# yusanshi/news-recommendation

Measured on NVIDIA H100. Metric: impressions/sec (fwd+bwd), higher is better.
Workload: dtype bf16

## Files before the change

### include/newsrec_b200.h

```cpp
#ifndef NEWSREC_B200_H
#define NEWSREC_B200_H

#include <stdint.h>

#ifdef __cplusplus
extern "C" {
#endif

int nr_version(void);
const char* nr_last_error(void);
int nr_device_error(int out4[4]);
long long nr_launch_count(void);
int nr_num_sms(void);
void nr_debug_set_simt_gemm(int on);
int nr_has_triage_backends(void);
void nr_debug_set_gru_stepwise(int on);
typedef struct {
    const void* A;
    int M, lda;
    const void* W;
    int N, ldw, K, taps, w_tap_rows, tap_origin;
    void* out;
    int ld_out, out_bf16, relu, tanh;
    const void* dtanh_src;
// ... 97 lines not shown
int nr_topk_dot_ranged(const float* users, long long n_users, int ld_users, const float* news, long long n_news, int ld_news, int D,
                       int k, const long long* excl_offsets, const long long* excl_rows, const int* categories, int max_per_category,
                       const long long* row_lo, const long long* row_hi, long long* idx, float* score, int* bad_row_flag,
                       int* bad_score_flag, void* workspace, long long workspace_bytes, void* stream);

int nr_mmr_rerank(const float* news, long long n_news, int ld_news, int D, const long long* shortlist_idx, const float* shortlist_score,
                  long long n_users, int depth, int k, float lambda, long long* idx, float* score, int* bad_row_flag, void* stream);

int nr_list_stats(const float* news, long long n_news, int ld_news, int D, const long long* idx, long long n_rows, int k,
                  const int* categories, const int* ks, int n_ks, double* pair_sum, int* distinct, int* bad_row_flag, void* stream);

long long nr_pool_ranks_workspace(long long n_rows, long long n_news, int D);
int nr_pool_ranks(const float* queries, long long n_rows, int ld_queries, const float* news, long long n_news, int ld_news, int D,
                  const long long* tgt_offsets, const long long* tgt_rows, const long long* excl_offsets, const long long* excl_rows,
                  long long* rank, float* score, int* bad_row_flag, int* bad_score_flag, int* target_flag, void* workspace,
                  long long workspace_bytes, void* stream);

int nr_pool_ranks_ranged(const float* queries, long long n_rows, int ld_queries, const float* news, long long n_news, int ld_news,
                         int D, const long long* tgt_offsets, const long long* tgt_rows, const long long* excl_offsets,
                         const long long* excl_rows, const long long* row_lo, const long long* row_hi, long long* rank, float* score,
                         int* bad_row_flag, int* bad_score_flag, int* target_flag, void* workspace, long long workspace_bytes,
                         void* stream);

long long nr_topk_archive_workspace(long long n_users, int P, long long n_news, int F, int hidden, int k);
int nr_topk_archive(const float* archive, long long n_users, int P, const float* news, long long n_news, int F, const float* W1,
                    const float* b1, int hidden, const float* w2, const float* b2, int k, const long long* excl_offsets,
                    const long long* excl_rows, const int* categories, int max_per_category, long long* idx, float* score,
                    int* bad_row_flag, int* bad_score_flag, void* workspace, long long workspace_bytes, void* stream);

int nr_topk_archive_ranged(const float* archive, long long n_users, int P, const float* news, long long n_news, int F,
                           const float* W1, const float* b1, int hidden, const float* w2, const float* b2, int k,
                           const long long* excl_offsets, const long long* excl_rows, const int* categories, int max_per_category,
                           const long long* row_lo, const long long* row_hi, long long* idx, float* score, int* bad_row_flag,
                           int* bad_score_flag, void* workspace, long long workspace_bytes, void* stream);

long long nr_pool_ranks_archive_workspace(long long n_rows, int P, long long n_news, int F, int hidden);
int nr_pool_ranks_archive(const float* archive, long long n_rows, int P, const float* news, long long n_news, int F, const float* W1,
                          const float* b1, int hidden, const float* w2, const float* b2, const long long* tgt_offsets,
                          const long long* tgt_rows, const long long* excl_offsets, const long long* excl_rows, long long* rank,
                          float* score, int* bad_row_flag, int* bad_score_flag, int* target_flag, void* workspace,
                          long long workspace_bytes, void* stream);

int nr_pool_ranks_archive_ranged(const float* archive, long long n_rows, int P, const float* news, long long n_news, int F,
                                 const float* W1, const float* b1, int hidden, const float* w2, const float* b2,
                                 const long long* tgt_offsets, const long long* tgt_rows, const long long* excl_offsets,
                                 const long long* excl_rows, const long long* row_lo, const long long* row_hi, long long* rank,
                                 float* score, int* bad_row_flag, int* bad_score_flag, int* target_flag, void* workspace,
                                 long long workspace_bytes, void* stream);

int nr_accumulate_ext_grad(float* ext, int rows, int ld, int D, float* dW, float* db, void* stream);

typedef struct {
    long long n_seq;
    int T;
    int d;
    int heads;
    int q;
    int ldx;
    int ld3;
    const long long* ids;
    const void* table_bf16;
    int V;
    const float* dense;
    long long dense_s_seq, dense_s_tok, dense_s_col;
    const void* wqkv_bf16;
    const float* bqkv;
    const void* wa_bf16;
    const float* ba;
    const float* qv;
    float p_drop;
    unsigned long long seed;
    void* X_bf16;
    void* QKV_bf16;
    void* C_bf16;
    float* w;
    float* out;
    int* bad_id_flag;
    void* C_lo_bf16;
    const void* wqkv_kcat_bf16;
    void* X_kcat_bf16;
    float* QKV_f32;
    void* V_lo_bf16;
    const float* dense_pos;
} nr_mhsa_encoder_fwd_args;
int nr_mhsa_accurate_supported(int T, int d, int heads);
int nr_mhsa_encoder_fwd(const nr_mhsa_encoder_fwd_args* a, void* stream);

typedef struct {
    long long n_seq;
    int T, d, heads, q, ldx, ld3, ldq;
    const long long* ids;
    int V;
    const void* wqkvT_bf16;
    const void* wa_bf16;
    const void* waT_bf16;
    const float* ba;
    const float* qv;
    float p_drop;
    unsigned long long seed;
    const void* X_bf16;
    const void* QKV_bf16;
    const void* C_bf16;
    const float* w;
    const float* dout;
    float* dWqkv_ext;
    float* dWa_ext;
    float* dqv;
    float* demb;
    float* ddense;
    void* workspace;
    long long workspace_bytes;
    const void* wqkv_bf16;
    const float* bqkv;
    void* emb_grad_ready_event;
    float* dpos;
    const void* table_bf16;
} nr_mhsa_encoder_bwd_args;
long long nr_mhsa_encoder_bwd_workspace(long long n_seq, int T, int d, int q);
int nr_mhsa_encoder_bwd(const nr_mhsa_encoder_bwd_args* a, void* stream);

typedef struct {
    long long n_seq;
    int T, d, F, q, ldx, ldf;
    const long long* ids;
    const void* table_bf16;
    int V;
    const void* wconv_bf16;
    const float* bconv;
    const void* wa_bf16;
    const float* ba;
    const float* qv;
    float p_drop;
    unsigned long long seed;
    void* Xp_bf16;
    void* Y_bf16;
    float* w;
    float* out;
    int* bad_id_flag;
    void* Y_lo_bf16;
    int window;
} nr_cnn_encoder_fwd_args;
int nr_cnn_encoder_fwd(const nr_cnn_encoder_fwd_args* a, void* stream);

typedef struct {
    long long n_seq;
    int T, d, F, q, ldx, ldf, ldq;
    const long long* ids;
    int V;
    const void* wconvT_bf16;
    const void* wa_bf16;
    const void* waT_bf16;
    const float* ba;
    const float* qv;
    float p_drop;
    unsigned long long seed;
    const void* Xp_bf16;
    const void* Y_bf16;
    const float* w;
    const float* dout;
    float* dWconv_ext;
    float* dWa_ext;
    float* dqv;
    float* demb;
    void* workspace;
    long long workspace_bytes;
    int window;
} nr_cnn_encoder_bwd_args;
long long nr_cnn_encoder_bwd_workspace(long long n_seq, int T, int F, int q);
int nr_cnn_encoder_bwd(const nr_cnn_encoder_bwd_args* a, void* stream);

typedef struct {
    long long n_seq;
    int T, d, de, F, q, n_win;
    int win[4];
    int ldx, lde, ldf, ldo;
    const long long* word_ids;
    const long long* entity_ids;
    const void* word_table_bf16;
    int V;
    const void* entity_table_bf16;
    int Ve;
    const void* mT_bf16;
    const float* mb;
    const void* wconv_bf16;
    const float* bconv;
    const void* wa_bf16;
    const float* ba;
    const float* qv;
    void* X2_bf16;
    void* E_bf16;
    void* Y_bf16;
    float* w;
    float* out;
    int* bad_id_flag;
} nr_kcnn_encoder_fwd_args;
int nr_kcnn_encoder_fwd(const nr_kcnn_encoder_fwd_args* a, void* stream);

typedef struct {
    long long n_seq;
// ... 115 lines not shown
```

### news-recommendation_b200/csrc/abi.cu

```cuda
#include <cstring>
#include <utility>

#include "../../include/newsrec_b200.h"
#include "nr_common.cuh"
#include "nr_ops.h"

namespace nr {
const char* last_error();
int read_device_error(int* out4);
void set_debug_simt_gemm(int on);
int has_triage_backends();
void set_debug_gemm_timing(void* dev_buf, int slots);
void set_comm_reserved_sms(int n);
}

using namespace nr;

extern "C" {

int nr_version(void) { return 1; }
const char* nr_last_error(void) { return last_error(); }
int nr_device_error(int out4[4]) { return read_device_error(out4); }
long long nr_launch_count(void) { return g_launches; }
int nr_num_sms(void) { return num_sms(); }
void nr_debug_set_simt_gemm(int on) { set_debug_simt_gemm(on); }
void nr_debug_set_gru_stepwise(int on) { set_gru_stepwise(on); }
int nr_debug_gemm_store(const nr_gemm_store_args* a, void* stream) {
    NR_REQUIRE(a && a->A && a->W && a->out, "nr_debug_gemm_store: null operand");
    const auto misaligned = [](const void* p, uintptr_t bytes) { return (reinterpret_cast<uintptr_t>(p) & (bytes - 1)) != 0; };
    NR_REQUIRE(!misaligned(a->out, 16) && !misaligned(a->lo_out, 16) && !misaligned(a->dtanh_src, 4),
               "nr_debug_gemm_store: out and lo_out need 16-byte, dtanh_src 4-byte aligned bases");
    return gemm_store({.A = a->A, .M = a->M, .lda = a->lda, .W = a->W, .N = a->N, .ldw = a->ldw, .K = a->K, .taps = a->taps,
                       .w_tap_rows = a->w_tap_rows, .tap_origin = a->tap_origin},
                      {.out = a->out, .ld_out = a->ld_out, .out_bf16 = a->out_bf16, .relu = a->relu, .tanh = a->tanh,
                       .dtanh_src = a->dtanh_src, .dtanh_ld = a->dtanh_ld, .bias = a->bias,
                       .rm = {a->rm_seg_in, a->rm_in_off, a->rm_seg_len, a->rm_seg_out, a->rm_out_off},
                       .drop = {a->p_drop, a->seed}, .ones_col = a->ones_col, .ones_zero_upto = a->ones_zero_upto, .lo_out = a->lo_out,
                       .ld_lo = a->ld_lo, .lo_col0 = a->lo_col0, .accumulate = a->accumulate, .rows_per_tile = a->rows_per_tile},
                      as_stream(stream));
}
int nr_debug_live_tokens(const long long* ids, long long n_seq, int T, int d, const void* table, int V, const void* X, int ldx,
                         const float* bqkv, unsigned* mask, unsigned char* pad, int* offset, int* index, int* tiles, void* Xc,
                         void* dqkv_c, void* stream) {
    NR_REQUIRE(ids && X && bqkv && mask && pad && offset && index && tiles && Xc && dqkv_c && n_seq >= 0 && d >= 2,
               "nr_debug_live_tokens: null operand or n_seq=%lld d=%d", n_seq, d);
    const cudaStream_t st = as_stream(stream);
    const int sec = (d + 7) & ~7, ld3 = (3 * sec + 15) & ~15;
    const long long bytes = live_tokens_bytes(n_seq, T, ld3);
    char* buf = nullptr;
    NR_CHECK_CUDA(cudaMallocAsync(reinterpret_cast<void**>(&buf), bytes, st));
    LiveTokens lt;
    int rc = live_tokens(ids, n_seq, T, d, table, ldx, V, bqkv, sec, ld3, X, ldx, Xc, dqkv_c, buf, bytes, &lt, st);
    const size_t n = static_cast<size_t>(n_seq), M = n * T;
    const std::pair<void*, const void*> copies[] = {{mask, lt.mask}, {pad, lt.pad}, {offset, lt.offset}, {index, lt.index}, {tiles, lt.tiles}};
    const size_t sizes[] = {4 * n, n, 4 * (n + 1), 4 * M, 4 * (1 + (M + 63) / 64)};
    for (int i = 0; i < 5 && rc == 0 && n > 0; ++i)
        if (cudaMemcpyAsync(copies[i].first, copies[i].second, sizes[i], cudaMemcpyDeviceToDevice, st) != cudaSuccess) rc = -1;
    NR_CHECK_CUDA(cudaFreeAsync(buf, st));
    NR_REQUIRE(rc != -1, "nr_debug_live_tokens: copy-out failed");
    return rc;
}
int nr_has_triage_backends(void) { return has_triage_backends(); }
void nr_reserve_sms_for_comm(int n) { set_comm_reserved_sms(n); }
void nr_debug_set_gemm_timing(void* dev_buf, int slots) { set_debug_gemm_timing(dev_buf, slots); }
void nr_profile_enable(int on) { prof_enable(on); }
void nr_profile_context(const char* ctx) { prof_context(ctx ? ctx : ""); }
int nr_profile_report(char* buf, int cap) { return prof_report(buf, cap); }

static Bf16Rows cast_pad_job(const float* src, int R, int C, int lds, void* dst, int ld, int transpose) {
    if (transpose) return {.src = src, .n_rows = C, .D = R, .s_seq = 1, .s_col = lds, .width = ld, .hi = dst, .ld_hi = ld};
    return {.src = src, .n_rows = R, .D = C, .s_seq = lds, .width = ld, .hi = dst, .ld_hi = ld};
}
int nr_cast_pad_bf16_many(int n, const float* const* src, const int* R, const int* C, const int* lds, void* const* dst, const int* ld,
                          const int* transpose, void* stream) {
    NR_REQUIRE(src && R && C && lds && dst && ld && transpose, "nr_cast_pad_bf16_many: null argument array");
    NR_REQUIRE(n >= 0 && n <= kBf16RowsJobs, "nr_cast_pad_bf16_many: %d matrices (at most %d per call)", n, kBf16RowsJobs);
    Bf16Rows jobs[kBf16RowsJobs];
    for (int i = 0; i < n; ++i) {
        NR_REQUIRE(R[i] >= 1 && C[i] >= 1, "nr_cast_pad_bf16_many: bad matrix %d", i);
        jobs[i] = cast_pad_job(src[i], R[i], C[i], lds[i], dst[i], ld[i], transpose[i]);
    }
    return rows_to_bf16(jobs, n, kCastPadMany, as_stream(stream));
}
int nr_cast_pad_bf16(const float* src, int R, int C, int lds, void* dst, int ld, int transpose, void* stream) {
    NR_REQUIRE(src && dst && R >= 0 && C >= 0 && ld % 8 == 0 && ld >= (transpose ? R : C),
               "nr_cast_pad_bf16: R=%d C=%d ld=%d transpose=%d", R, C, ld, transpose);
    return rows_to_bf16(cast_pad_job(src, R, C, lds, dst, ld, transpose), kCastPad, as_stream(stream));
}
int nr_rows_to_bf16(const float* src, long long n, int D, long long s_row, long long s_col, void* dst, int ld,
                    void* stream) {
    NR_REQUIRE(src && dst && n >= 0 && ld % 8 == 0, "nr_rows_to_bf16: n=%lld ld=%d", n, ld);
    return rows_to_bf16({.src = src, .n_rows = n, .D = D, .s_seq = s_row, .s_col = s_col, .width = ld, .hi = dst, .ld_hi = ld, .ones_col = 1},
                        kRowsToBf16, as_stream(stream));
}
int nr_rows_to_bf16_hilo(const float* src, long long n, int D, long long s_row, long long s_col, void* hi, void* lo, int ld,
                         void* stream) {
    NR_REQUIRE(src && hi && lo && n >= 0 && D >= 1 && ld % 8 == 0, "nr_rows_to_bf16_hilo: n=%lld D=%d ld=%d", n, D, ld);
    return rows_to_bf16({.src = src, .n_rows = n, .D = D, .s_seq = s_row, .s_col = s_col, .width = ld, .hi = hi, .ld_hi = ld, .ones_col = 1,
                         .lo = lo, .ld_lo = ld},
                        kRowsToBf16Planes, as_stream(stream));
}
int nr_gather_rows(const long long* ids, long long n_tok, int T, const void* table, int V, int D, int ld, void* X,
                   int padded, float p_drop, unsigned long long seed, int* bad_id_flag, void* stream) {
    NR_REQUIRE(ids && table && X && bad_id_flag && T >= 1 && n_tok % T == 0 && p_drop >= 0.f && p_drop < 1.f,
               "nr_gather_rows: n_tok=%lld T=%d p=%f", n_tok, T, p_drop);
    return gather_rows(ids, n_tok, T, table, V, D, ld, X, ld, padded, DropoutCfg{p_drop, seed}, bad_id_flag, as_stream(stream));
}
int nr_linear(const void* A, int M, int lda, const void* W, int N, int ldw, int K, int taps, int w_tap_rows,
              int rows_per_tile, const float* bias, int relu, void* out, int ld_out, int out_is_bf16, void* stream) {
    NR_REQUIRE(A && W && out && (taps == 1 || taps == 3), "nr_linear: null operand or taps=%d", taps);
    return gemm_store({.A = A, .M = M, .lda = lda, .W = W, .N = N, .ldw = ldw, .K = K, .taps = taps, .w_tap_rows = w_tap_rows},
                      {.out = out, .ld_out = ld_out, .out_bf16 = out_is_bf16, .relu = relu, .bias = bias, .rows_per_tile = rows_per_tile},
                      as_stream(stream));
}
int nr_gemm_tn(const void* A, int Kr, int Ma, int lda, const void* B, int b_rows, int b_cols, int ldb, int b_col0,
               int Nb, int b_row_shift, float* D, int ldd, void* stream) {
    NR_REQUIRE(A && B && D, "nr_gemm_tn: null operand");
    return gemm_tn_accumulate(A, Kr, Ma, lda, B, b_rows, b_cols, ldb, b_col0, Nb, b_row_shift, D, ldd, as_stream(stream));
}
int nr_mhsa_core_fwd(const void* qkv, int ld_qkv, int sec, long long n_seq, int T, int heads, int dk, void* ctx, int ld_ctx,
                     float p_drop, unsigned long long seed, void* stream) {
    NR_REQUIRE(qkv && ctx, "nr_mhsa_core_fwd: null operand");
    return mhsa_core_fwd(qkv, ld_qkv, sec, n_seq, T, heads, dk, ctx, ld_ctx, DropoutCfg{p_drop, seed}, as_stream(stream));
}
int nr_mhsa_core_bwd(const void* qkv, int ld_qkv, int sec, const void* dctx, int ld_dctx, long long n_seq, int T, int heads,
                     int dk, void* dqkv, int ld_dqkv, void* stream) {
    NR_REQUIRE(qkv && dctx && dqkv, "nr_mhsa_core_bwd: null operand");
    return mhsa_core_bwd(qkv, ld_qkv, sec, dctx, ld_dctx, n_seq, T, heads, dk, dqkv, ld_dqkv, as_stream(stream));
}

int nr_additive_attention_fwd(const void* X, long long n_seg, int seg_len, int D, int ldx, const void* Wa, int q, int ldw,
// ... 183 lines not shown
                                 float* score, int* bad_row_flag, int* bad_score_flag, int* target_flag, void* workspace,
                                 long long workspace_bytes, void* stream) {
    NR_REQUIRE(archive && news && W1 && b1 && w2 && b2 && tgt_offsets && tgt_rows && row_lo && row_hi && rank && score &&
                   bad_row_flag && bad_score_flag && target_flag,
               "nr_pool_ranks_archive_ranged: null operand");
    return pool_ranks_archive(archive, n_rows, P, news, n_news, F, W1, b1, hidden, w2, b2, tgt_offsets, tgt_rows, excl_offsets,
                              excl_rows, row_lo, row_hi, rank, score, bad_row_flag, bad_score_flag, target_flag, workspace,
                              workspace_bytes, as_stream(stream));
}
long long nr_prediction_line_offsets_workspace(long long n_seg) {
    NR_REQUIRE(n_seg >= 0, "nr_prediction_line_offsets_workspace: n_seg=%lld", n_seg);
    return prediction_scan_bytes(n_seg);
}
int nr_prediction_line_offsets(const long long* impression_ids, const int* ranks, const long long* seg_offsets, long long n_seg,
                               long long* line_offsets, void* workspace, long long workspace_bytes, void* stream) {
    NR_REQUIRE(impression_ids && ranks && seg_offsets && line_offsets && workspace && n_seg >= 0,
               "nr_prediction_line_offsets: null operand or n_seg=%lld", n_seg);
    return prediction_line_offsets(impression_ids, ranks, seg_offsets, n_seg, line_offsets, workspace, workspace_bytes, as_stream(stream));
}
int nr_prediction_text(const long long* impression_ids, const int* ranks, const long long* seg_offsets, long long n_seg,
                       const long long* line_offsets, char* text, void* stream) {
    NR_REQUIRE(impression_ids && ranks && seg_offsets && line_offsets && text && n_seg >= 0,
               "nr_prediction_text: null operand or n_seg=%lld", n_seg);
    return prediction_text(impression_ids, ranks, seg_offsets, n_seg, line_offsets, text, as_stream(stream));
}

int nr_accumulate_ext_grad(float* ext, int rows, int ld, int D, float* dW, float* db, void* stream) {
    NR_REQUIRE(ext && dW && rows >= 0 && D >= 1, "nr_accumulate_ext_grad: null operand");
    return accumulate_ext_grad(ext, rows, ld, D, dW, db, as_stream(stream));
}

int nr_slots_device_readable(const void* const* slots, int n) {
    if (slots == nullptr || n <= 0) return 0;
    return slots_device_readable(slots, n);
}
int nr_pack_slots(const void* const* slots, int n_clicked, int n_candidates, int B, int L, long long* out, void* stream) {
    NR_REQUIRE(slots && out && n_clicked >= 0 && n_candidates >= 0 && B >= 0 && L >= 1, "nr_pack_slots: bad arguments");
    for (int i = 0; i < n_clicked + n_candidates; ++i) NR_REQUIRE(slots[i] != nullptr, "nr_pack_slots: slot %d is null", i);
    prof_context("feed");
    return pack_slots(slots, n_clicked, n_candidates, B, L, out, as_stream(stream));
}
int nr_feed_gather(const nr_feed_field* fields, int n_fields, const int* behaviors, int H, int C, const int* records,
                   const long long* rows, int B, long long* user_out, long long* length_out, long long* clicked_out, void* stream) {
    NR_REQUIRE(n_fields >= 0 && n_fields <= kFeedFields && (fields || n_fields == 0) && H >= 0 && C >= 1 && B >= 0,
               "nr_feed_gather: bad arguments n_fields=%d H=%d C=%d B=%d", n_fields, H, C, B);
    NR_REQUIRE(behaviors && rows && (records || !(user_out || length_out || clicked_out)), "nr_feed_gather: null operand");
    FeedField f[kFeedFields];
    for (int i = 0; i < n_fields; ++i) {
        NR_REQUIRE(fields[i].table && fields[i].out && fields[i].width >= 1, "nr_feed_gather: bad field %d", i);
        f[i] = {.table = fields[i].table, .width = fields[i].width, .out = fields[i].out};
    }
    prof_context("feed");
    return feed_gather(f, n_fields, behaviors, H, C, {.records = records, .user = user_out, .length = length_out, .clicked = clicked_out},
                       rows, B, as_stream(stream));
}
int nr_sample_negatives(const int* cand_rows, const unsigned char* labels, const long long* imp_offsets, long long n_imp,
                        const long long* row_offsets, int K, unsigned long long seed, long long epoch, int* behaviors, int H, void* stream) {
    NR_REQUIRE(cand_rows && labels && imp_offsets && row_offsets && behaviors, "nr_sample_negatives: null operand");
    NR_REQUIRE(K >= 1 && n_imp >= 0 && H >= 0, "nr_sample_negatives: bad arguments K=%d n_imp=%lld H=%d", K, n_imp, H);
    prof_context("feed");
    return sample_negatives(cand_rows, labels, imp_offsets, n_imp, row_offsets, K, seed, epoch, behaviors, H, as_stream(stream));
}

static int qkv_section(int d) { return (d + 7) & ~7; }
static int check_mhsa_shape(long long n_seq, int T, int d, int heads, int q, int ldx, int ld3) {
    NR_REQUIRE(n_seq >= 0 && T >= 1 && T <= 64 && d >= 8 && heads >= 1 && d % heads == 0 && q >= 1 && q <= 256,
               "mhsa encoder: bad shape n_seq=%lld T=%d d=%d heads=%d q=%d", n_seq, T, d, heads, q);
    NR_REQUIRE(d / heads >= 2 && d / heads <= 32, "mhsa encoder: head size d_k=%d (d=%d, heads=%d) not in [2, 32]", d / heads, d,
               heads);
    NR_REQUIRE(ldx % 8 == 0 && ldx >= d + 1 && ld3 % 8 == 0 && ld3 >= 3 * qkv_section(d), "mhsa encoder: bad pitches ldx=%d ld3=%d",
               ldx, ld3);
    NR_REQUIRE(n_seq * T < (1ll << 31), "mhsa encoder: too many tokens (%lld)", n_seq * T);
    return 0;
}

static bool mhsa_accurate_shape(int T, int d, int heads, int ld3, int ldx) {
    if (heads < 1 || d % heads != 0) return false;
    const int sec = qkv_section(d);
    return mhsa_title_fwd_supported(T, d / heads, heads, sec, ld3, ldx) && gemm_store_lo_supported(3 * sec, d, 2 * sec);
}
int nr_mhsa_accurate_supported(int T, int d, int heads) {
    return mhsa_accurate_shape(T, d, heads, (3 * qkv_section(d) + 15) & ~15, (d + 8) & ~7) ? 1 : 0;
}

struct PaddingScope {
    PaddingTitles pt;
    cudaStream_t st;
    ~PaddingScope() { free_padding_titles(pt, st); }
};


static Bf16Rows dense_rows(const nr_mhsa_encoder_fwd_args* a, void* hi, int ld_hi) {
    return {.src = a->dense, .n_rows = a->n_seq * a->T, .T = a->T, .D = a->d, .s_seq = a->dense_s_seq, .s_tok = a->dense_s_tok,
            .s_col = a->dense_s_col, .pos = a->dense_pos, .width = a->ldx, .hi = hi, .ld_hi = ld_hi, .ones_col = 1};
}

int nr_mhsa_encoder_fwd(const nr_mhsa_encoder_fwd_args* a, void* stream) {
    NR_REQUIRE(a != nullptr, "nr_mhsa_encoder_fwd: null args");
    NR_PROPAGATE(check_mhsa_shape(a->n_seq, a->T, a->d, a->heads, a->q, a->ldx, a->ld3));
    NR_REQUIRE((a->ids != nullptr) != (a->dense != nullptr), "nr_mhsa_encoder_fwd: exactly one of ids / dense");
    NR_REQUIRE(a->wa_bf16 && a->ba && a->qv && a->C_bf16 && a->w && a->out, "nr_mhsa_encoder_fwd: null operand");
    const bool precise_dense = a->dense != nullptr && a->C_lo_bf16 != nullptr;
    NR_REQUIRE(precise_dense || (a->wqkv_bf16 && a->bqkv && a->X_bf16 && a->QKV_bf16), "nr_mhsa_encoder_fwd: null operand");
    NR_REQUIRE(a->p_drop >= 0.f && a->p_drop < 1.f, "nr_mhsa_encoder_fwd: dropout p=%f", a->p_drop);
    NR_REQUIRE(a->dense_pos == nullptr || a->dense != nullptr, "nr_mhsa_encoder_fwd: dense_pos needs the dense (user-level) variant");
    if (a->n_seq == 0) return 0;
    const int M = static_cast<int>(a->n_seq * a->T);
    const cudaStream_t st = as_stream(stream);
    const int sec = qkv_section(a->d);
    prof_context(a->ids != nullptr ? "news.fwd" : "user.fwd");
    if (a->dense != nullptr && a->C_lo_bf16 != nullptr) {
        NR_REQUIRE(a->wqkv_kcat_bf16 && a->X_kcat_bf16 && a->QKV_f32 && a->bqkv && a->X_bf16,
                   "nr_mhsa_encoder_fwd: precise dense variant needs wqkv_kcat_bf16 / X_kcat_bf16 / QKV_f32 / bqkv / X_bf16");
        NR_REQUIRE(a->QKV_bf16 == nullptr, "nr_mhsa_encoder_fwd: the precise dense variant writes no bf16 Q|K|V (pass NULL)");
        NR_PROPAGATE(rows_to_bf16(dense_rows(a, a->X_bf16, a->ldx), kRowsToBf16, st));
        Bf16Rows kcat = dense_rows(a, a->X_kcat_bf16, 2 * a->ldx);
        kcat.lo = static_cast<__nv_bfloat16*>(a->X_kcat_bf16) + a->ldx;
        kcat.ld_lo = 2 * a->ldx;
        NR_PROPAGATE(rows_to_bf16(kcat, kRowsToBf16Hilo, st));
        NR_PROPAGATE(gemm_store({.A = a->X_kcat_bf16, .M = M, .lda = 2 * a->ldx, .W = a->wqkv_kcat_bf16, .N = 3 * sec, .ldw = 2 * a->ldx,
                                 .K = 2 * a->ldx},
                                {.out = a->QKV_f32, .ld_out = 3 * sec, .bias = a->bqkv}, st));
        NR_PROPAGATE(mhsa_f32_fwd(a->QKV_f32, 3 * sec, sec, a->n_seq, a->T, a->heads, a->d / a->heads, a->C_bf16, a->C_lo_bf16, a->ldx, st));
        NR_PROPAGATE(gemm_additive_pool(a->C_bf16, M, a->ldx, a->d, a->wa_bf16, a->q, a->ldx, a->ba, a->qv, a->T, a->out, a->d,
                                        a->w, st, a->C_lo_bf16));
        return 0;
    }
    if (a->ids != nullptr && a->V_lo_bf16 != nullptr) {
        NR_REQUIRE(a->C_lo_bf16 != nullptr && a->table_bf16 && a->bad_id_flag && a->V >= 1,
                   "nr_mhsa_encoder_fwd: the accurate variant needs C_lo_bf16 (+ table / bad_id_flag)");
        NR_REQUIRE(mhsa_accurate_shape(a->T, a->d, a->heads, a->ld3, a->ldx),
                   "nr_mhsa_encoder_fwd: the accurate variant needs the title-level attention kernel (T=20, d_k=20, <=15 heads) and a "
                   "chunk-aligned V section (d=%d); see nr_mhsa_accurate_supported", a->d);
        NR_PROPAGATE(gather_rows(a->ids, M, a->T, a->table_bf16, a->V, a->d, a->ldx, a->X_bf16, a->ldx, 0,
                                 DropoutCfg{a->p_drop, a->seed}, a->bad_id_flag, st));
        PaddingScope pad{.st = st};
        NR_PROPAGATE(padding_titles(a->ids, a->n_seq, a->T, a->d, a->table_bf16, a->ldx, a->bqkv, sec, a->ld3, &pad.pt, st));
        NR_PROPAGATE(gemm_store({.A = a->X_bf16, .M = M, .lda = a->ldx, .W = a->wqkv_bf16, .N = 3 * sec, .ldw = a->ldx, .K = a->d},
                                {.out = a->QKV_bf16, .ld_out = a->ld3, .out_bf16 = 1, .bias = a->bqkv, .lo_out = a->V_lo_bf16, .ld_lo = sec,
                                 .lo_col0 = 2 * sec, .tile_list = pad.pt.live}, st));
        {
            ProfScope ps("mhsa_core_fwd_hilo", static_cast<int>(a->n_seq), a->T, a->d, st);
            NR_PROPAGATE(mhsa_title_fwd(a->QKV_bf16, a->ld3, sec, a->n_seq, a->heads, a->C_bf16, a->ldx, context_dropout(a->p_drop, a->seed), st,
                                        a->V_lo_bf16, sec, a->C_lo_bf16, &pad.pt));
        }
        NR_PROPAGATE(gemm_additive_pool(a->C_bf16, M, a->ldx, a->d, a->wa_bf16, a->q, a->ldx, a->ba, a->qv, a->T, a->out, a->d,
                                        a->w, st, a->C_lo_bf16));
        return 0;
    }
    if (a->ids != nullptr) {
        NR_REQUIRE(a->table_bf16 && a->bad_id_flag && a->V >= 1, "nr_mhsa_encoder_fwd: table / bad_id_flag missing");
        NR_PROPAGATE(gather_rows(a->ids, M, a->T, a->table_bf16, a->V, a->d, a->ldx, a->X_bf16, a->ldx, 0,
                                 DropoutCfg{a->p_drop, a->seed}, a->bad_id_flag, st));
    } else {
        NR_PROPAGATE(rows_to_bf16(dense_rows(a, a->X_bf16, a->ldx), kRowsToBf16, st));
    }
    NR_PROPAGATE(gemm_store({.A = a->X_bf16, .M = M, .lda = a->ldx, .W = a->wqkv_bf16, .N = 3 * sec, .ldw = a->ldx, .K = a->d},
                            {.out = a->QKV_bf16, .ld_out = a->ld3, .out_bf16 = 1, .bias = a->bqkv}, st));
    const DropoutCfg cdrop = context_dropout(a->ids != nullptr ? a->p_drop : 0.f, a->seed);
    NR_PROPAGATE(mhsa_core_fwd(a->QKV_bf16, a->ld3, sec, a->n_seq, a->T, a->heads, a->d / a->heads, a->C_bf16, a->ldx, cdrop, st));
    NR_PROPAGATE(gemm_additive_pool(a->C_bf16, M, a->ldx, a->d, a->wa_bf16, a->q, a->ldx, a->ba, a->qv, a->T, a->out, a->d,
                                    a->w, st));
    return 0;
}

struct MhsaBwdWorkspace : WorkspaceLayout {
    float* dscore;
    __nv_bfloat16 *dpre, *dC, *dQKV, *QKV;
    char* live;
    long long live_bytes;
    MhsaBwdWorkspace(void* base, long long n_seq, int T, int d, int q)
        : WorkspaceLayout{static_cast<char*>(base)}, dscore(take<float>(n_seq * T)), dpre(take<__nv_bfloat16>(n_seq * T * round_up(q, 16))),
          dC(take<__nv_bfloat16>(n_seq * T * round_up(d + 1, 8))), dQKV(take<__nv_bfloat16>(n_seq * T * round_up(3 * qkv_section(d), 16))),
          QKV(take<__nv_bfloat16>(n_seq * T * round_up(3 * qkv_section(d), 16))),
          live_bytes(live_tokens_bytes(n_seq, T, round_up(3 * qkv_section(d), 16))) {
        live = take<char>(live_bytes);
    }
};
long long nr_mhsa_encoder_bwd_workspace(long long n_seq, int T, int d, int q) { return MhsaBwdWorkspace(nullptr, n_seq, T, d, q).bytes(); }

int nr_mhsa_encoder_bwd(const nr_mhsa_encoder_bwd_args* a, void* stream) {
    NR_REQUIRE(a != nullptr, "nr_mhsa_encoder_bwd: null args");
    NR_PROPAGATE(check_mhsa_shape(a->n_seq, a->T, a->d, a->heads, a->q, a->ldx, a->ld3));
    NR_REQUIRE(a->ldq % 8 == 0 && a->ldq >= a->q, "nr_mhsa_encoder_bwd: ldq=%d", a->ldq);
    NR_REQUIRE(a->ldx == ((a->d + 8) & ~7) && a->ld3 == ((3 * qkv_section(a->d) + 15) & ~15) && a->ldq == ((a->q + 15) & ~15),
               "nr_mhsa_encoder_bwd: pitches must be canonical: ldx=round_up(d+1,8), ld3=round_up(3*round_up(d,8),16), ldq=round_up(q,16)");
    NR_REQUIRE(a->wqkvT_bf16 && a->wa_bf16 && a->waT_bf16 && a->ba && a->qv && a->X_bf16 && a->C_bf16 &&
                   a->w && a->dout && a->dWqkv_ext && a->dWa_ext && a->dqv && a->workspace,
               "nr_mhsa_encoder_bwd: null operand");
    NR_REQUIRE(a->QKV_bf16 != nullptr || (a->wqkv_bf16 != nullptr && a->bqkv != nullptr),
               "nr_mhsa_encoder_bwd: Q|K|V was not saved (precise dense forward): pass wqkv_bf16 / bqkv so that it can be recomputed from X");
    NR_REQUIRE((a->ids != nullptr) ? (a->demb != nullptr) : (a->ddense != nullptr),
               "nr_mhsa_encoder_bwd: missing input-gradient buffer");
    NR_REQUIRE(a->dpos == nullptr || a->ids == nullptr, "nr_mhsa_encoder_bwd: dpos needs the dense (user-level) variant");
    NR_REQUIRE(a->ids == nullptr || a->bqkv != nullptr, "nr_mhsa_encoder_bwd: the news variant needs bqkv (Q|K|V of its padding titles)");
    NR_REQUIRE(a->table_bf16 == nullptr || a->ids != nullptr, "nr_mhsa_encoder_bwd: table_bf16 needs the ids (news) variant");
    const MhsaBwdWorkspace ws(a->workspace, a->n_seq, a->T, a->d, a->q);
    NR_REQUIRE(a->workspace_bytes >= ws.bytes(), "nr_mhsa_encoder_bwd: workspace too small (%lld bytes)", a->workspace_bytes);
    if (a->n_seq == 0) return 0;
    const int M = static_cast<int>(a->n_seq * a->T);
    const cudaStream_t st = as_stream(stream);
    const int sec = qkv_section(a->d);

    prof_context(a->ids != nullptr ? "news.bwd" : "user.bwd");
    const void* QKV = a->QKV_bf16;
    if (QKV == nullptr) {
        NR_PROPAGATE(gemm_store({.A = a->X_bf16, .M = M, .lda = a->ldx, .W = a->wqkv_bf16, .N = 3 * sec, .ldw = a->ldx, .K = a->d},
                                {.out = ws.QKV, .ld_out = a->ld3, .out_bf16 = 1, .bias = a->bqkv}, st));
        QKV = ws.QKV;
    }
    NR_PROPAGATE(pool_dscore(a->C_bf16, a->ldx, a->d, a->n_seq, a->T, a->w, a->dout, a->d, ws.dscore, st));
    NR_PROPAGATE(gemm_additive_dpre(a->C_bf16, M, a->ldx, a->d, a->wa_bf16, a->q, a->ldx, a->ba, a->qv, ws.dscore, ws.dpre, a->ldq,
                                    a->dqv, st));
    NR_PROPAGATE(gemm_pool_dinput({.A = ws.dpre, .M = M, .lda = a->ldq, .W = a->waT_bf16, .N = a->d, .ldw = a->ldq, .K = a->q},
                                  {.w = a->w, .dout = a->dout, .ldo = a->d, .seg_len = a->T, .dx = ws.dC, .ld_dx = a->ldx,
                                   .drop = context_dropout(a->ids != nullptr ? a->p_drop : 0.f, a->seed)}, st));
    LiveTokens live;
    const bool compact = a->ids != nullptr && mhsa_title_bwd_supported(a->T, a->d / a->heads, a->heads, sec, a->ld3, a->ldx, a->ld3);
    if (compact) {
        NR_REQUIRE(a->V >= 1, "nr_mhsa_encoder_bwd: V=%d", a->V);
        NR_PROPAGATE(live_tokens(a->ids, a->n_seq, a->T, a->d, a->table_bf16, a->ldx, a->V, a->bqkv, sec, a->ld3, a->X_bf16, a->ldx, ws.QKV,
                                 ws.dQKV, ws.live, ws.live_bytes, &live, st));
    }
    const TitleBwdLive title_live{.tokens = &live, .dbias = a->dWqkv_ext + a->d, .ld_dbias = a->ldx};
    NR_PROPAGATE(mhsa_core_bwd(QKV, a->ld3, sec, ws.dC, a->ldx, a->n_seq, a->T, a->heads, a->d / a->heads, ws.dQKV, a->ld3, st,
                               compact ? &title_live : nullptr));
    if (a->ids != nullptr) {
        NR_REQUIRE(a->V >= 1, "nr_mhsa_encoder_bwd: V=%d", a->V);
        NR_PROPAGATE(gemm_scatter_emb({.A = ws.dQKV, .M = M, .lda = a->ld3, .W = a->wqkvT_bf16, .N = a->d, .ldw = a->ld3, .K = 3 * sec},
                                      {.ids = a->ids, .demb = a->demb, .V = a->V, .drop = {a->p_drop, a->seed}, .drop_ld = a->ldx,
                                       .rows = live.index, .tile_list = live.tiles}, st));
        if (a->emb_grad_ready_event != nullptr) NR_CHECK_CUDA(cudaEventRecord(static_cast<cudaEvent_t>(a->emb_grad_ready_event), st));
    } else {
        NR_PROPAGATE(gemm_store({.A = ws.dQKV, .M = M, .lda = a->ld3, .W = a->wqkvT_bf16, .N = a->d, .ldw = a->ld3, .K = 3 * sec},
                                {.out = a->ddense, .ld_out = a->d}, st));
        if (a->dpos != nullptr) NR_PROPAGATE(sum_over_seq(a->ddense, a->n_seq, static_cast<long long>(a->T) * a->d, a->dpos, st));
    }
    NR_PROPAGATE(gemm_weight_grad(ws.dpre, M, a->q, a->ldq, a->C_bf16, a->d, a->ldx, a->dWa_ext, st));
    NR_PROPAGATE(gemm_weight_grad(ws.dQKV, M, 3 * sec, a->ld3, compact ? ws.QKV : a->X_bf16, a->d, a->ldx, a->dWqkv_ext, st, 0,
                                  live.tiles));
    return 0;
}

}
```

### news-recommendation_b200/csrc/attn_title.cu

```cuda
#include <algorithm>

#define NR_WATCHDOG_SYMBOL g_attn_dev_error
#include "nr_fused.cuh"
#include "nr_mma.cuh"
#include "nr_ops.h"

namespace nr {

int read_topk_device_error(int* out4);
int read_attn_device_error(int* out4) {
    const int rc = static_cast<int>(cudaMemcpyFromSymbol(out4, fused::g_attn_dev_error, sizeof(int) * 4));
    if (rc != 0 || out4[0] != 0) return rc;
    return read_topk_device_error(out4);
}

namespace title {

using namespace fused;
using namespace mma;

constexpr int kT = 20;
constexpr int kDk = 20;
constexpr int kMaxHeads = 15;
constexpr int kIn = 2;
constexpr int kOut = 2;
constexpr int kInHilo = 2;
constexpr int kScrPitch = 48;
constexpr int kScrTile = 24 * kScrPitch;
constexpr int kScrWarp = 2 * kScrTile;

struct Params {
    int n_seq, heads;
    uint32_t sec2;
    uint32_t pq, pc;
    uint32_t qkv_tile;
    uint32_t in_stage;
    uint32_t out_stage;
    uint32_t tx;
    float rs, sc;
    const unsigned char* pad;
    const uint32_t* mask;
    const int* offset;
    char* dqkv;
    uint32_t ld_out, row_bytes;
    float* dbias;
    int ld_dbias;
};

__device__ __forceinline__ uint32_t sel(bool keep, uint32_t v) { return keep ? v : 0u; }

__global__ void __launch_bounds__((kMaxHeads + 1) * 32, 1)
mhsa_title_bwd_kernel(const __grid_constant__ CUtensorMap tm_qkv, const __grid_constant__ CUtensorMap tm_dc,
                      const __grid_constant__ CUtensorMap tm_out, const __grid_constant__ CUtensorMap tm_pad, const Params p) {
    extern __shared__ __align__(16) uint8_t smem_raw[];
    const uint32_t base = (smem_u32(smem_raw) + 127u) & ~127u;
    uint8_t* const base_ptr = smem_raw + (base - smem_u32(smem_raw));
    const int tid = threadIdx.x, warp = tid >> 5, lane = tid & 31, g = lane >> 2, t4 = lane & 3;
    const uint32_t in_base = base, out_base = base + kIn * p.in_stage, scr_base = out_base + kOut * p.out_stage;
    const uint32_t bar_off = kIn * p.in_stage + kOut * p.out_stage + p.heads * kScrWarp;
    uint64_t* const bars = reinterpret_cast<uint64_t*>(base_ptr + bar_off);
    uint64_t* const full = bars;
    uint64_t* const empty = bars + kIn;
    uint64_t* const ofull = bars + 2 * kIn;
    uint64_t* const oempty = bars + 2 * kIn + kOut;

    for (uint32_t i = tid; i < bar_off / 16; i += blockDim.x) reinterpret_cast<uint4*>(base_ptr)[i] = make_uint4(0, 0, 0, 0);
    if (tid == 0) {
        for (int i = 0; i < kIn; ++i) {
            mbar_init(&full[i], 1);
            mbar_init(&empty[i], p.heads);
        }
        for (int i = 0; i < kOut; ++i) {
            mbar_init(&ofull[i], p.heads);
            mbar_init(&oempty[i], 1);
        }
        fence_barrier_init();
    }
    fence_proxy_async();
    __syncthreads();

    const int n_my = (p.n_seq - static_cast<int>(blockIdx.x) + static_cast<int>(gridDim.x) - 1) / static_cast<int>(gridDim.x);

    if (warp == p.heads) {
        if (lane == 0) {
            tma_prefetch_desc(&tm_qkv);
            tma_prefetch_desc(&tm_dc);
            tma_prefetch_desc(&tm_out);
            if (p.pad != nullptr) tma_prefetch_desc(&tm_pad);
            auto load = [&](int it) {
                const int s = it % kIn;
                const int title = static_cast<int>(blockIdx.x) + it * static_cast<int>(gridDim.x), row = title * kT;
                const bool pad = p.pad != nullptr && p.pad[title] != 0;
                mbar_arrive_expect_tx(&full[s], p.tx);
                tma_load_2d(base_ptr + s * p.in_stage, pad ? &tm_pad : &tm_qkv, &full[s], 0, pad ? 0 : row);
                tma_load_2d(base_ptr + s * p.in_stage + p.qkv_tile, &tm_dc, &full[s], 0, row);
            };
            for (int it = 0; it < kIn && it < n_my; ++it) load(it);
            for (int j = 0; j < n_my; ++j) {
                const int o = j % kOut;
                const int title = static_cast<int>(blockIdx.x) + j * static_cast<int>(gridDim.x);
                const uint32_t tile = out_base + o * p.out_stage;
                uint32_t live = 0;
                char* dst = nullptr;
                if (p.mask != nullptr) {
                    live = p.mask[title];
                    dst = p.dqkv + static_cast<size_t>(p.offset[title]) * p.ld_out;
                }
                f_wait(&ofull[o], (j / kOut) & 1, 70);
                if (p.mask == nullptr) {
                    tma_store_2d(&tm_out, tile, 0, title * kT);
                } else {
                    for (; live != 0; live &= live - 1, dst += p.ld_out) bulk_store_1d(dst, tile + (__ffs(live) - 1) * p.pq, p.row_bytes);
                }
                bulk_commit();
                if (j + kIn < n_my) {
                    f_wait(&empty[j % kIn], (j / kIn) & 1, 71);
                    load(j + kIn);
                }
                bulk_wait_read<0>();
                mbar_arrive(&oempty[o]);
            }
            bulk_wait_all();
        }
        return;
    }

    const int h = warp;
    const bool odd = (h & 1) != 0;
    const uint32_t gb = 40u * h - (odd ? 8u : 0u);
    const uint32_t k16b = gb + (odd ? 16u : 0u);
    const uint32_t k8b = gb + (odd ? 0u : 32u);
    const bool v8 = odd ? (t4 >= 2) : (t4 < 2);
    const bool c0ok = !odd || t4 >= 2;
    const bool c2ok = odd || t4 < 2;
    const bool lo2 = t4 < 2;
    const uint32_t pq = p.pq, pc = p.pc;
    const uint32_t r15q = (lane & 15) * pq, r7q = (lane & 7) * pq, r15c = (lane & 15) * pc, r7c = (lane & 7) * pc;
    const uint32_t hi = (lane >> 4) * 16u, mid = ((lane >> 3) & 1) * 16u;
    const uint32_t ps = scr_base + h * kScrWarp, dsb = ps + kScrTile;
    const uint32_t at0 = ((lane & 7) + (lane >> 4) * 8) * kScrPitch + mid;
    const uint32_t at8 = (16 + (lane & 7)) * kScrPitch;
    const uint32_t at1 = (lane & 15) * kScrPitch + 32u;
    const uint32_t st_scr = g * kScrPitch + t4 * 4u;
    const float rs = p.rs, sc = p.sc;
    float dsum[3][3][2] = {};
    const auto add_dead = [](float* acc, uint32_t packed) {
        const float2 v = unpack_bf16x2(packed);
        acc[0] += v.x;
        acc[1] += v.y;
    };

    for (int it = 0; it < n_my; ++it) {
        const int s = it % kIn, o = it % kOut;
        const uint32_t Q = in_base + s * p.in_stage, K = Q + p.sec2, V = K + p.sec2, G = Q + p.qkv_tile;
        const uint32_t ob = out_base + o * p.out_stage;
        const uint32_t dead = p.mask != nullptr ? ~__ldg(p.mask + static_cast<int>(blockIdx.x) + it * static_cast<int>(gridDim.x)) : 0u;
        f_wait(&full[s], (it / kIn) & 1, 72);

        uint32_t kb16[3][2], kb8[3], vb16[3][2], vb8[3], kt16[3][2], kt8[3];
#pragma unroll
        for (int nt = 0; nt < 3; ++nt) {
            lds_x2(kb16[nt], K + k16b + nt * 8 * pq + r7q + mid);
            lds_x2(vb16[nt], V + k16b + nt * 8 * pq + r7q + mid);
            lds_x1(&kb8[nt], K + k8b + nt * 8 * pq + r7q);
            lds_x1(&vb8[nt], V + k8b + nt * 8 * pq + r7q);
            kb8[nt] = sel(v8, kb8[nt]);
            vb8[nt] = sel(v8, vb8[nt]);
            lds_x2_t(kt16[nt], K + gb + 16 * nt + r15q);
            lds_x1_t(&kt8[nt], K + gb + 16 * nt + 16 * pq + r7q);
            kt8[nt] = sel(lo2, kt8[nt]);
        }
#pragma unroll
        for (int mt = 0; mt < 2; ++mt) {
            uint32_t aq[4], ag[4], aq8[2], ag8[2];
            if (mt == 0) {
                lds_x4(aq, Q + k16b + r15q + hi);
                lds_x4(ag, G + k16b + r15c + hi);
                lds_x2(aq8, Q + k8b + r15q);
                lds_x2(ag8, G + k8b + r15c);
            } else {
                uint32_t t[2];
                lds_x2(t, Q + k16b + 16 * pq + r7q + mid);
                aq[0] = t[0], aq[1] = 0u, aq[2] = t[1], aq[3] = 0u;
                lds_x2(t, G + k16b + 16 * pc + r7c + mid);
                ag[0] = t[0], ag[1] = 0u, ag[2] = t[1], ag[3] = 0u;
                lds_x1(&aq8[0], Q + k8b + 16 * pq + r7q);
                lds_x1(&ag8[0], G + k8b + 16 * pc + r7c);
                aq8[1] = ag8[1] = 0u;
            }
            aq8[0] = sel(v8, aq8[0]), aq8[1] = sel(v8, aq8[1]);
            ag8[0] = sel(v8, ag8[0]), ag8[1] = sel(v8, ag8[1]);
            float sm[3][4], dp[3][4];
#pragma unroll
            for (int nt = 0; nt < 3; ++nt) {
                mma_bf16_z(sm[nt], aq, kb16[nt]);
                mma_bf16_k8(sm[nt], aq8, &kb8[nt]);
                mma_bf16_z(dp[nt], ag, vb16[nt]);
                mma_bf16_k8(dp[nt], ag8, &vb8[nt]);
            }
            const bool row0 = mt == 0 || g < 4;
            constexpr float kNegInf = -__builtin_huge_valf();
            float m0 = kNegInf, m1 = kNegInf;
#pragma unroll
            for (int nt = 0; nt < 3; ++nt) {
                const bool ok = nt < 2 || lo2;
#pragma unroll
                for (int e = 0; e < 4; ++e) sm[nt][e] = ok ? sm[nt][e] : kNegInf;
                m0 = fmaxf(m0, fmaxf(sm[nt][0], sm[nt][1]));
                if (mt == 0) m1 = fmaxf(m1, fmaxf(sm[nt][2], sm[nt][3]));
            }
            m0 = quad_max(m0) * sc;
            if (mt == 0) m1 = quad_max(m1) * sc;
            float l0 = 0.f, l1 = 0.f;
#pragma unroll
            for (int nt = 0; nt < 3; ++nt) {
#pragma unroll
                for (int e = 0; e < 2; ++e) {
                    sm[nt][e] = exp2f(fmaf(sm[nt][e], sc, -m0));
                    l0 += sm[nt][e];
                    if (mt == 0) {
                        sm[nt][2 + e] = exp2f(fmaf(sm[nt][2 + e], sc, -m1));
                        l1 += sm[nt][2 + e];
                    }
                }
            }
            l0 = quad_sum(l0);
            const float i0 = 1.f / (l0 + 1e-8f * exp2f(-m0));
            float i1 = 0.f;
            if (mt == 0) {
                l1 = quad_sum(l1);
                i1 = 1.f / (l1 + 1e-8f * exp2f(-m1));
            }
            float del0 = 0.f, del1 = 0.f;
#pragma unroll
            for (int nt = 0; nt < 3; ++nt) {
                const bool ok = nt < 2 || lo2;
#pragma unroll
                for (int e = 0; e < 2; ++e) {
                    sm[nt][e] = (ok && row0) ? sm[nt][e] * i0 : 0.f;
                    del0 += ok ? sm[nt][e] * dp[nt][e] : 0.f;
                    if (mt == 0) {
                        sm[nt][2 + e] = ok ? sm[nt][2 + e] * i1 : 0.f;
                        del1 += ok ? sm[nt][2 + e] * dp[nt][2 + e] : 0.f;
                    } else {
                        sm[nt][2 + e] = 0.f;
                    }
                }
            }
            del0 = quad_sum(del0);
            if (mt == 0) del1 = quad_sum(del1);
            uint32_t a16[4], a8[2];
#pragma unroll
            for (int nt = 0; nt < 3; ++nt) {
                const bool ok = nt < 2 || lo2;
#pragma unroll
                for (int e = 0; e < 2; ++e) {
                    dp[nt][e] = (ok && row0) ? sm[nt][e] * (dp[nt][e] - del0) * rs : 0.f;
                    dp[nt][2 + e] = (mt == 0 && ok) ? sm[nt][2 + e] * (dp[nt][2 + e] - del1) * rs : 0.f;
                }
                const uint32_t p01 = pack_bf16x2(sm[nt][0], sm[nt][1]), d01 = pack_bf16x2(dp[nt][0], dp[nt][1]);
                const uint32_t p23 = pack_bf16x2(sm[nt][2], sm[nt][3]), d23 = pack_bf16x2(dp[nt][2], dp[nt][3]);
                const uint32_t so = st_scr + mt * 16 * kScrPitch + nt * 16;
                sts32(ps + so, p01);
                sts32(dsb + so, d01);
                if (mt == 0) {
                    sts32(ps + so + 8 * kScrPitch, p23);
                    sts32(dsb + so + 8 * kScrPitch, d23);
                }
                if (nt == 0) a16[0] = d01, a16[1] = d23;
                if (nt == 1) a16[2] = d01, a16[3] = d23;
                if (nt == 2) a8[0] = d01, a8[1] = d23;
            }
            if (mt == 0 && it >= kOut) f_wait(&oempty[o], ((it / kOut) - 1) & 1, 73);
#pragma unroll
            for (int nd = 0; nd < 3; ++nd) {
                float dq[4];
                mma_bf16_z(dq, a16, kt16[nd]);
                mma_bf16_k8(dq, a8, &kt8[nd]);
                const bool cok = nd == 1 || (nd == 0 ? c0ok : c2ok);
                const uint32_t oa = ob + (mt * 16 + g) * pq + gb + 16 * nd + 4 * t4;
                if (cok && row0) {
                    const uint32_t v = pack_bf16x2(dq[0], dq[1]);
                    sts32(oa, v);
                    if ((dead >> (mt * 16 + g)) & 1u) add_dead(dsum[0][nd], v);
                }
                if (mt == 0 && cok) {
                    const uint32_t v = pack_bf16x2(dq[2], dq[3]);
                    sts32(oa + 8 * pq, v);
                    if ((dead >> (8 + g)) & 1u) add_dead(dsum[0][nd], v);
                }
            }
        }
        __syncwarp();
        uint32_t qt16[3][2], qt8[3], gt16[3][2], gt8[3];
#pragma unroll
        for (int nd = 0; nd < 3; ++nd) {
            lds_x2_t(qt16[nd], Q + gb + 16 * nd + r15q);
            lds_x2_t(gt16[nd], G + gb + 16 * nd + r15c);
            lds_x1_t(&qt8[nd], Q + gb + 16 * nd + 16 * pq + r7q);
            lds_x1_t(&gt8[nd], G + gb + 16 * nd + 16 * pc + r7c);
            qt8[nd] = sel(lo2, qt8[nd]);
            gt8[nd] = sel(lo2, gt8[nd]);
        }
#pragma unroll
        for (int mt = 0; mt < 2; ++mt) {
            uint32_t ad[4], ap[4], ad8[2], ap8[2];
            if (mt == 0) {
                lds_x4_t(ad, dsb + at0);
                lds_x4_t(ap, ps + at0);
                lds_x2_t(ad8, dsb + at8 + mid);
                lds_x2_t(ap8, ps + at8 + mid);
            } else {
                uint32_t t[2];
                lds_x2_t(t, dsb + at1);
                ad[0] = t[0], ad[1] = 0u, ad[2] = t[1], ad[3] = 0u;
                lds_x2_t(t, ps + at1);
                ap[0] = t[0], ap[1] = 0u, ap[2] = t[1], ap[3] = 0u;
                lds_x1_t(&ad8[0], dsb + at8 + 32u);
                lds_x1_t(&ap8[0], ps + at8 + 32u);
                ad8[1] = ap8[1] = 0u;
            }
            const bool row0 = mt == 0 || g < 4;
#pragma unroll
            for (int nd = 0; nd < 3; ++nd) {
                float dk[4], dv[4];
                mma_bf16_z(dk, ad, qt16[nd]);
                mma_bf16_k8(dk, ad8, &qt8[nd]);
                mma_bf16_z(dv, ap, gt16[nd]);
                mma_bf16_k8(dv, ap8, &gt8[nd]);
                const bool cok = nd == 1 || (nd == 0 ? c0ok : c2ok);
                const uint32_t oa = ob + p.sec2 + (mt * 16 + g) * pq + gb + 16 * nd + 4 * t4;
                if (cok && row0) {
                    const uint32_t k = pack_bf16x2(dk[0], dk[1]), v = pack_bf16x2(dv[0], dv[1]);
                    sts32(oa, k);
                    sts32(oa + p.sec2, v);
                    if ((dead >> (mt * 16 + g)) & 1u) add_dead(dsum[1][nd], k), add_dead(dsum[2][nd], v);
                }
                if (mt == 0 && cok) {
                    const uint32_t k = pack_bf16x2(dk[2], dk[3]), v = pack_bf16x2(dv[2], dv[3]);
                    sts32(oa + 8 * pq, k);
                    sts32(oa + p.sec2 + 8 * pq, v);
                    if ((dead >> (8 + g)) & 1u) add_dead(dsum[1][nd], k), add_dead(dsum[2][nd], v);
                }
            }
        }
        fence_proxy_async();
        __syncwarp();
        if (lane == 0) {
            mbar_arrive(&empty[s]);
            mbar_arrive(&ofull[o]);
        }
    }
    if (p.mask != nullptr) {
        const int sec = static_cast<int>(p.sec2 / 2u);
#pragma unroll
        for (int nd = 0; nd < 3; ++nd) {
            const bool cok = nd == 1 || (nd == 0 ? c0ok : c2ok);
            const int col = static_cast<int>(gb / 2u) + 8 * nd + 2 * t4;
#pragma unroll
            for (int sct = 0; sct < 3; ++sct) {
#pragma unroll
                for (int e = 0; e < 2; ++e) {
                    float v = dsum[sct][nd][e];
                    v += __shfl_xor_sync(0xffffffffu, v, 4);
                    v += __shfl_xor_sync(0xffffffffu, v, 8);
                    v += __shfl_xor_sync(0xffffffffu, v, 16);
                    if (g == 0 && cok) red_add_f32(p.dbias + static_cast<size_t>(sct * sec + col + e) * p.ld_dbias, v);
                }
            }
        }
    }
}


struct FwdParams {
    int n_seq, heads, ld_ctx;
    uint32_t sec2, pq, pc, pv, qkv_tile, in_stage, out_tile, out_stage, tx;
    float sc;
    Dropout drop;
    const unsigned char* pad;
};

template <bool HILO>
__global__ void __launch_bounds__((kMaxHeads + 1) * 32, HILO ? 1 : 2)
mhsa_title_fwd_kernel(const __grid_constant__ CUtensorMap tm_qkv, const __grid_constant__ CUtensorMap tm_vlo,
                      const __grid_constant__ CUtensorMap tm_ctx, const __grid_constant__ CUtensorMap tm_clo,
                      const __grid_constant__ CUtensorMap tm_pad, const __grid_constant__ CUtensorMap tm_padlo, const FwdParams p) {
    constexpr int kIn = HILO ? kInHilo : title::kIn;
    extern __shared__ __align__(16) uint8_t smem_raw[];
    const uint32_t base = (smem_u32(smem_raw) + 127u) & ~127u;
    uint8_t* const base_ptr = smem_raw + (base - smem_u32(smem_raw));
    const int tid = threadIdx.x, warp = tid >> 5, lane = tid & 31, g = lane >> 2, t4 = lane & 3;
    const uint32_t in_base = base, out_base = base + kIn * p.in_stage;
    const uint32_t bar_off = kIn * p.in_stage + kOut * p.out_stage;
    uint64_t* const bars = reinterpret_cast<uint64_t*>(base_ptr + bar_off);
    uint64_t* const full = bars;
    uint64_t* const empty = bars + kIn;
    uint64_t* const ofull = bars + 2 * kIn;
    uint64_t* const oempty = bars + 2 * kIn + kOut;
    for (uint32_t i = tid; i < bar_off / 16; i += blockDim.x) reinterpret_cast<uint4*>(base_ptr)[i] = make_uint4(0, 0, 0, 0);
    __syncthreads();
    if (tid < kOut * kT)
        *reinterpret_cast<__nv_bfloat16*>(base_ptr + kIn * p.in_stage + (tid / kT) * p.out_stage + (tid % kT) * p.pc + p.heads * kDk * 2) =
            __float2bfloat16_rn(1.0f);
    if (tid == 0) {
        for (int i = 0; i < kIn; ++i) {
            mbar_init(&full[i], 1);
            mbar_init(&empty[i], p.heads);
        }
        for (int i = 0; i < kOut; ++i) {
            mbar_init(&ofull[i], p.heads);
            mbar_init(&oempty[i], 1);
        }
        fence_barrier_init();
    }
    fence_proxy_async();
    __syncthreads();
    const int n_my = (p.n_seq - static_cast<int>(blockIdx.x) + static_cast<int>(gridDim.x) - 1) / static_cast<int>(gridDim.x);

    if (warp == p.heads) {
        if (lane == 0) {
            tma_prefetch_desc(&tm_qkv);
            tma_prefetch_desc(&tm_ctx);
            if (HILO) {
                tma_prefetch_desc(&tm_vlo);
                tma_prefetch_desc(&tm_clo);
            }
            if (p.pad != nullptr) {
                tma_prefetch_desc(&tm_pad);
                if (HILO) tma_prefetch_desc(&tm_padlo);
            }
            auto load = [&](int it) {
                const int s = it % kIn;
                const int title = static_cast<int>(blockIdx.x) + it * static_cast<int>(gridDim.x);
                const bool pad = p.pad != nullptr && p.pad[title] != 0;
                const int row = pad ? 0 : title * kT;
                mbar_arrive_expect_tx(&full[s], p.tx);
                tma_load_2d(base_ptr + s * p.in_stage, pad ? &tm_pad : &tm_qkv, &full[s], 0, row);
                if (HILO) tma_load_2d(base_ptr + s * p.in_stage + p.qkv_tile, pad ? &tm_padlo : &tm_vlo, &full[s], 0, row);
            };
            for (int it = 0; it < kIn && it < n_my; ++it) load(it);
            for (int j = 0; j < n_my; ++j) {
                const int o = j % kOut;
                const int row = (static_cast<int>(blockIdx.x) + j * static_cast<int>(gridDim.x)) * kT;
                f_wait(&ofull[o], (j / kOut) & 1, 80);
                tma_store_2d(&tm_ctx, base_ptr + kIn * p.in_stage + o * p.out_stage, 0, row);
                if (HILO) tma_store_2d(&tm_clo, base_ptr + kIn * p.in_stage + o * p.out_stage + p.out_tile, 0, row);
                bulk_commit();
                if (j + kIn < n_my) {
                    f_wait(&empty[j % kIn], (j / kIn) & 1, 81);
                    load(j + kIn);
                }
                bulk_wait_read<0>();
                mbar_arrive(&oempty[o]);
            }
            bulk_wait_all();
        }
        return;
    }

    const int h = warp;
    const bool odd = (h & 1) != 0;
    const uint32_t gb = 40u * h - (odd ? 8u : 0u);
    const uint32_t k16b = gb + (odd ? 16u : 0u), k8b = gb + (odd ? 0u : 32u);
    const bool v8 = odd ? (t4 >= 2) : (t4 < 2);
    const bool c0ok = !odd || t4 >= 2, c2ok = odd || t4 < 2, lo2 = t4 < 2;
    const uint32_t pq = p.pq, pc = p.pc, pv = p.pv;
    const uint32_t r15q = (lane & 15) * pq, r7q = (lane & 7) * pq;
    const uint32_t hi = (lane >> 4) * 16u, mid = ((lane >> 3) & 1) * 16u;
    const float sc = p.sc;

    for (int it = 0; it < n_my; ++it) {
        const int s = it % kIn, o = it % kOut;
        const uint32_t Q = in_base + s * p.in_stage, K = Q + p.sec2, V = K + p.sec2, VL = Q + p.qkv_tile;
        const uint32_t ob = out_base + o * p.out_stage;
        const long long row_base = static_cast<long long>(static_cast<int>(blockIdx.x) + it * static_cast<int>(gridDim.x)) * kT;
        f_wait(&full[s], (it / kIn) & 1, 82);
        uint32_t kb16[3][2], kb8[3], vt16[3][2], vt8[3], vl16[HILO ? 3 : 1][2], vl8[HILO ? 3 : 1];
#pragma unroll
        for (int nt = 0; nt < 3; ++nt) {
            lds_x2(kb16[nt], K + k16b + nt * 8 * pq + r7q + mid);
            lds_x1(&kb8[nt], K + k8b + nt * 8 * pq + r7q);
            kb8[nt] = sel(v8, kb8[nt]);
            lds_x2_t(vt16[nt], V + gb + 16 * nt + r15q);
            lds_x1_t(&vt8[nt], V + gb + 16 * nt + 16 * pq + r7q);
            vt8[nt] = sel(lo2, vt8[nt]);
            if (HILO) {
                lds_x2_t(vl16[nt], VL + gb + 16 * nt + (lane & 15) * pv);
                lds_x1_t(&vl8[nt], VL + gb + 16 * nt + 16 * pv + (lane & 7) * pv);
                vl8[nt] = sel(lo2, vl8[nt]);
            }
        }
#pragma unroll
        for (int mt = 0; mt < 2; ++mt) {
            uint32_t aq[4], aq8[2];
            if (mt == 0) {
                lds_x4(aq, Q + k16b + r15q + hi);
                lds_x2(aq8, Q + k8b + r15q);
            } else {
                uint32_t t[2];
                lds_x2(t, Q + k16b + 16 * pq + r7q + mid);
                aq[0] = t[0], aq[1] = 0u, aq[2] = t[1], aq[3] = 0u;
                lds_x1(&aq8[0], Q + k8b + 16 * pq + r7q);
                aq8[1] = 0u;
            }
            aq8[0] = sel(v8, aq8[0]), aq8[1] = sel(v8, aq8[1]);
            float sm[3][4];
#pragma unroll
            for (int nt = 0; nt < 3; ++nt) {
                mma_bf16_z(sm[nt], aq, kb16[nt]);
                mma_bf16_k8(sm[nt], aq8, &kb8[nt]);
            }
            const bool row0 = mt == 0 || g < 4;
            constexpr float kNegInf = -__builtin_huge_valf();
            float m0 = kNegInf, m1 = kNegInf;
#pragma unroll
            for (int nt = 0; nt < 3; ++nt) {
                const bool ok = nt < 2 || lo2;
#pragma unroll
                for (int e = 0; e < 4; ++e) sm[nt][e] = ok ? sm[nt][e] : kNegInf;
                m0 = fmaxf(m0, fmaxf(sm[nt][0], sm[nt][1]));
                if (mt == 0) m1 = fmaxf(m1, fmaxf(sm[nt][2], sm[nt][3]));
            }
            m0 = quad_max(m0) * sc;
            if (mt == 0) m1 = quad_max(m1) * sc;
            float l0 = 0.f, l1 = 0.f;
#pragma unroll
            for (int nt = 0; nt < 3; ++nt) {
#pragma unroll
                for (int e = 0; e < 2; ++e) {
                    sm[nt][e] = exp2f(fmaf(sm[nt][e], sc, -m0));
                    l0 += sm[nt][e];
                    if (mt == 0) {
                        sm[nt][2 + e] = exp2f(fmaf(sm[nt][2 + e], sc, -m1));
                        l1 += sm[nt][2 + e];
                    }
                }
            }
            l0 = quad_sum(l0);
            const float i0 = 1.f / (l0 + 1e-8f * exp2f(-m0));
            float i1 = 0.f;
            if (mt == 0) {
                l1 = quad_sum(l1);
                i1 = 1.f / (l1 + 1e-8f * exp2f(-m1));
            }
            uint32_t a16[4], a8[2], b16[HILO ? 4 : 1], b8[HILO ? 2 : 1];
#pragma unroll
            for (int nt = 0; nt < 3; ++nt) {
                const bool ok = nt < 2 || lo2;
                const float q0 = (ok && row0) ? sm[nt][0] * i0 : 0.f, q1 = (ok && row0) ? sm[nt][1] * i0 : 0.f;
                const float q2 = (mt == 0 && ok) ? sm[nt][2] * i1 : 0.f, q3 = (mt == 0 && ok) ? sm[nt][3] * i1 : 0.f;
                const uint32_t p01 = pack_bf16x2(q0, q1), p23 = pack_bf16x2(q2, q3);
                if (nt == 0) a16[0] = p01, a16[1] = p23;
                if (nt == 1) a16[2] = p01, a16[3] = p23;
                if (nt == 2) a8[0] = p01, a8[1] = p23;
                if (HILO) {
                    const float2 h01 = unpack_bf16x2(p01), h23 = unpack_bf16x2(p23);
                    const uint32_t l01 = pack_bf16x2(q0 - h01.x, q1 - h01.y), l23 = pack_bf16x2(q2 - h23.x, q3 - h23.y);
                    if (nt == 0) b16[0] = l01, b16[1] = l23;
                    if (nt == 1) b16[2] = l01, b16[3] = l23;
                    if (nt == 2) b8[0] = l01, b8[1] = l23;
                }
            }
            if (mt == 0 && it >= kOut) f_wait(&oempty[o], ((it / kOut) - 1) & 1, 83);
#pragma unroll
            for (int nd = 0; nd < 3; ++nd) {
                float c[4];
                if (HILO) {
                    mma_bf16_z(c, b16, vt16[nd]);
                    mma_bf16_k8(c, b8, &vt8[nd]);
                    mma_bf16(c, a16, vl16[nd]);
                    mma_bf16_k8(c, a8, &vl8[nd]);
                    mma_bf16(c, a16, vt16[nd]);
                } else {
                    mma_bf16_z(c, a16, vt16[nd]);
                }
                mma_bf16_k8(c, a8, &vt8[nd]);
                const bool cok = nd == 1 || (nd == 0 ? c0ok : c2ok);
                const uint32_t oa = ob + (mt * 16 + g) * pc + gb + 16 * nd + 4 * t4;
#pragma unroll
                for (int hf = 0; hf < 2; ++hf) {
                    if (hf == 1 && mt == 1) continue;
                    if (cok && (hf == 1 || row0)) {
                        const uint32_t hv = pack_bf16x2(c[2 * hf], c[2 * hf + 1]);
                        sts32(oa + hf * 8 * pc, hv);
                        if (HILO) {
// ... 13 lines not shown
                if (i < kT * 5) {
                    const uint32_t r = (i * 205u) >> 10, c4 = i - 5u * r;
                    const uint32_t a = ob + r * pc + 40u * h + 8u * c4;
                    uint32_t u0, u1;
                    asm volatile("ld.shared.v2.b32 {%0,%1}, [%2];" : "=r"(u0), "=r"(u1) : "r"(a));
                    float m[4];
                    p.drop.mask4_group(gbase + r * (static_cast<uint32_t>(p.ld_ctx) >> 2) + c4, m);
                    float2 x = unpack_bf16x2(u0), y = unpack_bf16x2(u1);
                    if (HILO) {
                        uint32_t w0, w1;
                        asm volatile("ld.shared.v2.b32 {%0,%1}, [%2];" : "=r"(w0), "=r"(w1) : "r"(a + p.out_tile));
                        const float2 xl = unpack_bf16x2(w0), yl = unpack_bf16x2(w1);
                        x.x = (x.x + xl.x) * m[0], x.y = (x.y + xl.y) * m[1], y.x = (y.x + yl.x) * m[2], y.y = (y.y + yl.y) * m[3];
                        const uint32_t h0 = pack_bf16x2(x.x, x.y), h1 = pack_bf16x2(y.x, y.y);
                        const float2 hx = unpack_bf16x2(h0), hy = unpack_bf16x2(h1);
                        asm volatile("st.shared.v2.b32 [%0], {%1,%2};" ::"r"(a), "r"(h0), "r"(h1) : "memory");
                        asm volatile("st.shared.v2.b32 [%0], {%1,%2};" ::"r"(a + p.out_tile), "r"(pack_bf16x2(x.x - hx.x, x.y - hx.y)),
                                     "r"(pack_bf16x2(y.x - hy.x, y.y - hy.y)) : "memory");
                    } else {
                        x.x *= m[0], x.y *= m[1], y.x *= m[2], y.y *= m[3];
                        asm volatile("st.shared.v2.b32 [%0], {%1,%2};" ::"r"(a), "r"(pack_bf16x2(x.x, x.y)), "r"(pack_bf16x2(y.x, y.y)) : "memory");
                    }
                }
            }
        }
        fence_proxy_async();
        __syncwarp();
        if (lane == 0) {
            mbar_arrive(&empty[s]);
            mbar_arrive(&ofull[o]);
        }
    }
}

static uint32_t odd16_pitch(uint32_t row_bytes) {
    uint32_t q = (row_bytes + 15u) / 16u;
    if ((q & 1u) == 0) ++q;
    return q * 16u;
}

}

bool mhsa_title_bwd_supported(int T, int dk, int heads, int sec, int ld_qkv, int ld_dctx, int ld_dqkv) {
    using namespace title;
    if (T != kT || dk != kDk || heads < 1 || heads > kMaxHeads) return false;
    if (sec % 8 != 0 || sec < heads * dk || ld_qkv % 8 != 0 || ld_dctx % 8 != 0 || ld_dqkv != ld_qkv) return false;
    if (ld_qkv < 3 * sec || ld_dctx < heads * dk) return false;
    return odd16_pitch(static_cast<uint32_t>(3 * sec) * 2u) <= 2048u && odd16_pitch(static_cast<uint32_t>(ld_dctx) * 2u) <= 2048u;
}

int mhsa_title_bwd(const void* qkv, int ld_qkv, int sec, const void* dctx, int ld_dctx, long long n_seq, int heads, void* dqkv,
                   int ld_dqkv, cudaStream_t stream, const TitleBwdLive* live) {
    using namespace title;
    NR_REQUIRE(mhsa_title_bwd_supported(kT, kDk, heads, sec, ld_qkv, ld_dctx, ld_dqkv), "mhsa_title_bwd: unsupported layout");
    NR_REQUIRE(n_seq * kT < (1ll << 31), "mhsa_title_bwd: too many rows");
    if (n_seq == 0) return 0;
    Params p;
    p.n_seq = static_cast<int>(n_seq);
    p.heads = heads;
    p.sec2 = static_cast<uint32_t>(sec) * 2u;
    const uint32_t qkv_row = 3u * p.sec2;
    const uint32_t dc_row = static_cast<uint32_t>(ld_dctx) * 2u;
    p.pq = odd16_pitch(qkv_row);
    p.pc = odd16_pitch(dc_row);
    p.qkv_tile = (kT * p.pq + 127u) & ~127u;
    const uint32_t dc_tile = (kT * p.pc + 127u) & ~127u;
    p.in_stage = p.qkv_tile + dc_tile;
    p.out_stage = p.qkv_tile;
    p.tx = kT * p.pq + kT * p.pc;
    p.rs = 1.0f / sqrtf(static_cast<float>(kDk));
    p.sc = p.rs * 1.4426950408889634f;
    const LiveTokens* lt = live != nullptr ? live->tokens : nullptr;
    NR_REQUIRE(live == nullptr || (lt != nullptr && lt->pad && lt->mask && lt->offset && lt->qkv && live->dbias),
               "mhsa_title_bwd: live tokens without their flags, offsets, padding Q|K|V tile or bias column");
    NR_REQUIRE(live == nullptr || (reinterpret_cast<uintptr_t>(dqkv) & 15) == 0, "mhsa_title_bwd: compact rows not 16-byte aligned");
    p.pad = lt != nullptr ? lt->pad : nullptr;
    p.mask = lt != nullptr ? lt->mask : nullptr;
    p.offset = lt != nullptr ? lt->offset : nullptr;
    p.dqkv = static_cast<char*>(dqkv);
    p.ld_out = static_cast<uint32_t>(ld_dqkv) * 2u;
    p.row_bytes = qkv_row;
    p.dbias = live != nullptr ? live->dbias : nullptr;
    p.ld_dbias = live != nullptr ? live->ld_dbias : 0;
    const size_t smem = 128 + static_cast<size_t>(kIn) * p.in_stage + static_cast<size_t>(kOut) * p.out_stage +
                       static_cast<size_t>(heads) * kScrWarp + (2 * kIn + 2 * kOut) * sizeof(uint64_t) + 64;
    NR_REQUIRE(smem <= 227 * 1024, "mhsa_title_bwd: %zu bytes of shared memory", smem);
    const long long rows = n_seq * kT;
    CUtensorMap tq, tc, to, tp;
    NR_PROPAGATE(make_tmap_bytes_2d(&tq, qkv, rows, qkv_row, static_cast<int64_t>(ld_qkv) * 2, static_cast<int>(p.pq), kT));
    NR_PROPAGATE(make_tmap_bytes_2d(&tc, dctx, rows, dc_row, static_cast<int64_t>(ld_dctx) * 2, static_cast<int>(p.pc), kT));
    NR_PROPAGATE(make_tmap_bytes_2d(&to, dqkv, rows, qkv_row, static_cast<int64_t>(ld_dqkv) * 2, static_cast<int>(p.pq), kT));
    if (lt != nullptr)
        NR_PROPAGATE(make_tmap_bytes_2d(&tp, lt->qkv, kT, qkv_row, static_cast<int64_t>(ld_qkv) * 2, static_cast<int>(p.pq), kT));
    else
        tp = tq;
    static bool attr_set = false;
    if (!attr_set) {
        NR_CHECK_CUDA(cudaFuncSetAttribute(mhsa_title_bwd_kernel, cudaFuncAttributeMaxDynamicSharedMemorySize, 227 * 1024));
        attr_set = true;
    }
    const int grid = static_cast<int>(std::min<long long>(n_seq, num_sms()));
    mhsa_title_bwd_kernel<<<grid, (heads + 1) * 32, smem, stream>>>(tq, tc, to, tp, p);
    ++g_launches;
    NR_CHECK_CUDA(cudaGetLastError());
    return 0;
}

bool mhsa_title_fwd_supported(int T, int dk, int heads, int sec, int ld_qkv, int ld_ctx) {
    using namespace title;
    if (T != kT || dk != kDk || heads < 1 || heads > kMaxHeads) return false;
    if (sec % 8 != 0 || sec < heads * dk || ld_qkv % 8 != 0 || ld_ctx % 8 != 0 || ld_qkv < 3 * sec || ld_ctx < heads * dk + 1) return false;
    return odd16_pitch(static_cast<uint32_t>(3 * sec) * 2u) <= 2048u && odd16_pitch(static_cast<uint32_t>(ld_ctx) * 2u) <= 2048u;
}

int mhsa_title_fwd(const void* qkv, int ld_qkv, int sec, long long n_seq, int heads, void* ctx, int ld_ctx, DropoutCfg drop,
                   cudaStream_t stream, const void* v_lo, int ld_vlo, void* ctx_lo, const PaddingTitles* pad) {
    using namespace title;
    NR_REQUIRE(mhsa_title_fwd_supported(kT, kDk, heads, sec, ld_qkv, ld_ctx), "mhsa_title_fwd: unsupported layout");
    NR_REQUIRE(n_seq * kT < (1ll << 31), "mhsa_title_fwd: too many rows");
    const bool hilo = v_lo != nullptr || ctx_lo != nullptr;
    NR_REQUIRE(!hilo || (v_lo != nullptr && ctx_lo != nullptr && ld_vlo % 8 == 0 && ld_vlo >= heads * kDk),
               "mhsa_title_fwd: the hi/lo variant needs both low planes (ld_vlo=%d)", ld_vlo);
    if (n_seq == 0) return 0;
    FwdParams p;
    p.n_seq = static_cast<int>(n_seq);
    p.heads = heads;
    p.ld_ctx = ld_ctx;
    p.sec2 = static_cast<uint32_t>(sec) * 2u;
    const uint32_t qkv_row = 3u * p.sec2, ctx_row = static_cast<uint32_t>(ld_ctx) * 2u, vlo_row = static_cast<uint32_t>(ld_vlo) * 2u;
    p.pq = odd16_pitch(qkv_row);
    p.pc = odd16_pitch(ctx_row);
    p.pv = hilo ? odd16_pitch(vlo_row) : 0u;
    p.qkv_tile = (kT * p.pq + 127u) & ~127u;
    p.in_stage = p.qkv_tile + (hilo ? ((kT * p.pv + 127u) & ~127u) : 0u);
    p.out_tile = (kT * p.pc + 127u) & ~127u;
    p.out_stage = (hilo ? 2u : 1u) * p.out_tile;
    p.tx = kT * p.pq + (hilo ? kT * p.pv : 0u);
    p.sc = 1.4426950408889634f / sqrtf(static_cast<float>(kDk));
    p.drop = Dropout::make(drop.p, drop.seed);
    NR_REQUIRE(pad == nullptr || (pad->pad != nullptr && pad->qkv != nullptr && (!hilo || (pad->v_lo != nullptr && ld_vlo == sec))),
               "mhsa_title_fwd: padding titles without their Q|K|V tile (or its V low plane at pitch sec)");
    p.pad = pad != nullptr ? pad->pad : nullptr;
    const int n_in = hilo ? kInHilo : kIn;
    const size_t smem = 128 + static_cast<size_t>(n_in) * p.in_stage + static_cast<size_t>(kOut) * p.out_stage +
                       (2 * n_in + 2 * kOut) * sizeof(uint64_t) + 64;
    const size_t cap = hilo ? 227 * 1024 : 113 * 1024;
    NR_REQUIRE(smem <= cap, "mhsa_title_fwd: %zu bytes of shared memory", smem);
    const long long rows = n_seq * kT;
    CUtensorMap tq, tc, tv, tl, tp, tpl;
    NR_PROPAGATE(make_tmap_bytes_2d(&tq, qkv, rows, qkv_row, static_cast<int64_t>(ld_qkv) * 2, static_cast<int>(p.pq), kT));
    NR_PROPAGATE(make_tmap_bytes_2d(&tc, ctx, rows, ctx_row, static_cast<int64_t>(ld_ctx) * 2, static_cast<int>(p.pc), kT));
    if (hilo) {
        NR_PROPAGATE(make_tmap_bytes_2d(&tv, v_lo, rows, vlo_row, static_cast<int64_t>(ld_vlo) * 2, static_cast<int>(p.pv), kT));
        NR_PROPAGATE(make_tmap_bytes_2d(&tl, ctx_lo, rows, ctx_row, static_cast<int64_t>(ld_ctx) * 2, static_cast<int>(p.pc), kT));
    } else {
        tv = tq;
        tl = tc;
    }
    tp = tq;
    tpl = tv;
    if (pad != nullptr) {
        NR_PROPAGATE(make_tmap_bytes_2d(&tp, pad->qkv, kT, qkv_row, static_cast<int64_t>(ld_qkv) * 2, static_cast<int>(p.pq), kT));
        if (hilo) NR_PROPAGATE(make_tmap_bytes_2d(&tpl, pad->v_lo, kT, vlo_row, static_cast<int64_t>(ld_vlo) * 2, static_cast<int>(p.pv), kT));
    }
    static bool attr_set = false;
    if (!attr_set) {
        NR_CHECK_CUDA(cudaFuncSetAttribute(mhsa_title_fwd_kernel<false>, cudaFuncAttributeMaxDynamicSharedMemorySize, 113 * 1024));
        NR_CHECK_CUDA(cudaFuncSetAttribute(mhsa_title_fwd_kernel<true>, cudaFuncAttributeMaxDynamicSharedMemorySize, 227 * 1024));
        attr_set = true;
    }
    const int grid = static_cast<int>(std::min<long long>(n_seq, (hilo ? 1ll : 2ll) * num_sms()));
    if (hilo)
        mhsa_title_fwd_kernel<true><<<grid, (heads + 1) * 32, smem, stream>>>(tq, tv, tc, tl, tp, tpl, p);
    else
        mhsa_title_fwd_kernel<false><<<grid, (heads + 1) * 32, smem, stream>>>(tq, tv, tc, tl, tp, tpl, p);
    ++g_launches;
    NR_CHECK_CUDA(cudaGetLastError());
    return 0;
}

}
```

### news-recommendation_b200/csrc/aux.cu

```cuda
#include <algorithm>

#include <cub/device/device_scan.cuh>

#include "nr_common.cuh"
#include "nr_ops.h"

namespace nr {

template <int N>
struct Bf16Jobs {
    Bf16Rows job[N];
};
__device__ __forceinline__ uint4 pack_bf16x8(const float (&v)[8]) {
    return make_uint4(pack_bf16x2(v[0], v[1]), pack_bf16x2(v[2], v[3]), pack_bf16x2(v[4], v[5]), pack_bf16x2(v[6], v[7]));
}
template <int N, int kThreads>
__global__ void __launch_bounds__(kThreads) rows_to_bf16_kernel(const __grid_constant__ Bf16Jobs<N> jobs) {
    const Bf16Rows& j = jobs.job[N == 1 ? 0 : blockIdx.y];
    const int D = j.D, T = j.T, chunks = j.width >> 3, n_rows = static_cast<int>(j.n_rows);
    const bool by_col = j.s_col != 1;
    __nv_bfloat16* const hi = static_cast<__nv_bfloat16*>(j.hi);
    __nv_bfloat16* const lo = static_cast<__nv_bfloat16*>(j.lo);
    for (int i = blockIdx.x * kThreads + threadIdx.x; i < n_rows * chunks; i += gridDim.x * kThreads) {
        const int c = by_col ? i / n_rows : i % chunks;
        const int r = by_col ? i - c * n_rows : i / chunks;
        const int col = c * 8;
        const int seq = T == 1 ? r : r / T;
        const int tok = r - seq * T;
        const float* sp = j.src + seq * j.s_seq + tok * j.s_tok;
        float x[8];
        if (j.s_col == 1 && col + 8 <= D && (reinterpret_cast<uintptr_t>(sp + col) & 15) == 0) {
            const float4 a = __ldg(reinterpret_cast<const float4*>(sp + col)), b = __ldg(reinterpret_cast<const float4*>(sp + col) + 1);
            x[0] = a.x; x[1] = a.y; x[2] = a.z; x[3] = a.w; x[4] = b.x; x[5] = b.y; x[6] = b.z; x[7] = b.w;
        } else {
#pragma unroll
            for (int e = 0; e < 8; ++e) x[e] = col + e < D ? __ldg(sp + (col + e) * j.s_col) : 0.f;
        }
        if (j.pos != nullptr) {
            const float* pp = j.pos + tok * D;
#pragma unroll
            for (int e = 0; e < 8; ++e)
                if (col + e < D) x[e] += __ldg(pp + col + e);
        }
        if (hi != nullptr) {
            float h[8];
#pragma unroll
            for (int e = 0; e < 8; ++e) h[e] = j.ones_col && col + e == D ? 1.0f : x[e];
            *reinterpret_cast<uint4*>(hi + static_cast<long long>(r) * j.ld_hi + col) = pack_bf16x8(h);
        }
        if (lo != nullptr) {
            float l[8];
#pragma unroll
            for (int e = 0; e < 8; ++e) l[e] = x[e] - bf16_round(x[e]);
            *reinterpret_cast<uint4*>(lo + static_cast<long long>(r) * j.ld_lo + col) = pack_bf16x8(l);
        }
    }
}
static bool plane_ok(const void* p, int ld, int width) {
    return p == nullptr || ((reinterpret_cast<uintptr_t>(p) & 15) == 0 && ld % 8 == 0 && ld >= width);
}
int rows_to_bf16(const Bf16Rows* jobs, int n_jobs, Bf16Op op, cudaStream_t stream) {
    NR_REQUIRE(n_jobs >= 0 && n_jobs <= kBf16RowsJobs, "%s: %d jobs (at most %d per launch)", op.name, n_jobs, kBf16RowsJobs);
    Bf16Jobs<kBf16RowsJobs> a;
    int n = 0;
    long long chunks = 0, biggest = 0;
    for (int i = 0; i < n_jobs; ++i) {
        const Bf16Rows& j = jobs[i];
        NR_REQUIRE(j.src && (j.hi || j.lo) && j.n_rows >= 0 && j.T >= 1 && j.D >= 0 && j.width % 8 == 0 &&
                       j.width >= j.D + (j.hi && j.ones_col ? 1 : 0) && plane_ok(j.hi, j.ld_hi, j.width) && plane_ok(j.lo, j.ld_lo, j.width),
                   "%s: job %d: n_rows=%lld T=%d D=%d width=%d ld_hi=%d ld_lo=%d (null or misaligned operand?)", op.name, i, j.n_rows, j.T,
                   j.D, j.width, j.ld_hi, j.ld_lo);
        NR_REQUIRE(j.n_rows * (j.width / 8) < (1ll << 30), "%s: job %d: %lld rows of %d columns", op.name, i, j.n_rows, j.width);
        if (j.n_rows == 0 || j.width == 0) continue;
        chunks = std::max(chunks, j.n_rows * (j.width / 8));
        biggest = std::max(biggest, j.n_rows * j.width);
        a.job[n++] = j;
    }
    if (n == 0) return 0;
    ProfScope ps(op.name, n_jobs == 1 ? static_cast<int>(a.job[0].n_rows) : n_jobs,
                 n_jobs == 1 ? a.job[0].D : static_cast<int>(std::min<long long>(biggest, 1 << 30)), n_jobs == 1 ? a.job[0].width : 0,
                 stream);
    const int threads = n == 1 ? 512 : 128;
    const dim3 grid(static_cast<unsigned>(std::min<long long>((chunks + threads - 1) / threads, 148ll * op.blocks_per_sm)),
                    static_cast<unsigned>(n));
    if (n == 1) rows_to_bf16_kernel<1, 512><<<grid, 512, 0, stream>>>(Bf16Jobs<1>{a.job[0]});
    else rows_to_bf16_kernel<kBf16RowsJobs, 128><<<grid, 128, 0, stream>>>(a);
    ++g_launches;
    NR_CHECK_CUDA(cudaGetLastError());
    return 0;
}

constexpr int kGatherThreads = 320;
__global__ void __launch_bounds__(kGatherThreads) gather_rows_kernel(const long long* __restrict__ ids, long long n_tok, int T,
                                                                   const uint4* __restrict__ table, int V, int D, int ld,
                                                                   uint4* __restrict__ X, int ld_x, int padded, Dropout drop,
                                                                   int* bad_flag) {
    const int chunks = ld >> 3;
    const int x_chunks = ld_x >> 3;
    const int rows_per_it = kGatherThreads / chunks;
    const int rl = threadIdx.x / chunks, c = threadIdx.x - rl * chunks;
    if (rl >= rows_per_it) return;
    const long long stride = static_cast<long long>(gridDim.x) * rows_per_it;
    long long tok = static_cast<long long>(blockIdx.x) * rows_per_it + rl;
    long long n_id = tok < n_tok ? __ldg(ids + tok) : 0;
    if (tok < n_tok && (n_id < 0 || n_id >= V)) { atomicExch(bad_flag, 1); n_id = 0; }
    uint4 n_u = tok < n_tok ? __ldg(table + n_id * chunks + c) : make_uint4(0, 0, 0, 0);
    const int col = c * 8;
    for (; tok < n_tok; tok += stride) {
        uint4 u = n_u;
        const long long tok2 = tok + stride;
        if (tok2 < n_tok) {
            n_id = __ldg(ids + tok2);
            if (n_id < 0 || n_id >= V) { atomicExch(bad_flag, 1); n_id = 0; }
            n_u = __ldg(table + n_id * chunks + c);
        }
        long long xr = tok;
        int t = 0;
        if (padded) {
            const long long seg = tok / T;
            t = static_cast<int>(tok - seg * T);
            xr = seg * (T + 2) + 1 + t;
        }
        uint32_t w[4] = {u.x, u.y, u.z, u.w};
        if (drop.active()) {
#pragma unroll
            for (int h = 0; h < 2; ++h) {
                float m[4];
                drop.mask4_group(static_cast<uint64_t>(xr) * (ld_x >> 2) + (col >> 2) + h, m);
                const float2 f0 = unpack_bf16x2(w[2 * h]), f1 = unpack_bf16x2(w[2 * h + 1]);
                w[2 * h] = pack_bf16x2(f0.x * m[0], f0.y * m[1]);
                w[2 * h + 1] = pack_bf16x2(f1.x * m[2], f1.y * m[3]);
            }
        }
        if (D >= col && D < col + 8) {
            __nv_bfloat16* e = reinterpret_cast<__nv_bfloat16*>(w);
            for (int j = D - col; j < 8; ++j) e[j] = __float2bfloat16_rn(j == D - col ? 1.0f : 0.f);
        }
        X[xr * x_chunks + c] = make_uint4(w[0], w[1], w[2], w[3]);
        if (padded) {
            if (t == 0) X[(xr - 1) * x_chunks + c] = make_uint4(0, 0, 0, 0);
            if (t == T - 1) X[(xr + 1) * x_chunks + c] = make_uint4(0, 0, 0, 0);
        }
    }
}
int gather_rows(const long long* ids, long long n_tok, int T, const void* table, int V, int D, int ld_table, void* X,
                int ld_x, int padded, DropoutCfg drop, int* bad_id_flag, cudaStream_t stream) {
    if (n_tok == 0) return 0;
    NR_REQUIRE(ld_table % 8 == 0 && ld_x % 8 == 0 && ld_x >= ld_table && ld_table >= D + 1 && ld_table / 8 <= kGatherThreads,
               "gather_rows: pitch %d/%d for D=%d", ld_table, ld_x, D);
    const int rows_per_it = kGatherThreads / (ld_table / 8);
    const int blocks = static_cast<int>(std::min<long long>((n_tok + rows_per_it - 1) / rows_per_it, 148 * 6));
    ProfScope ps("gather_rows", static_cast<int>(n_tok), D, ld_x, stream);
    gather_rows_kernel<<<blocks, kGatherThreads, 0, stream>>>(ids, n_tok, T, static_cast<const uint4*>(table), V, D, ld_table,
                                                   static_cast<uint4*>(X), ld_x, padded, Dropout::make(drop.p, drop.seed),
                                                   bad_id_flag);
    ++g_launches;
    NR_CHECK_CUDA(cudaGetLastError());
    return 0;
}

constexpr int kDsSegs = 6;
__global__ void __launch_bounds__(256) pool_dscore_kernel(const __nv_bfloat16* __restrict__ X, int lda, int D,
                                                          long long n_seg, int seg_len, const float* __restrict__ w,
                                                          const float* __restrict__ dout, int ldo,
                                                          float* __restrict__ dscore) {
    extern __shared__ float s_dw[];
    const int warp = threadIdx.x >> 5, lane = threadIdx.x & 31;
    const int chunks = D >> 3;
    const long long n_groups = (n_seg + kDsSegs - 1) / kDsSegs;
    for (long long grp = blockIdx.x; grp < n_groups; grp += gridDim.x) {
        const long long seg0 = grp * kDsSegs;
        const int nsg = static_cast<int>(min(static_cast<long long>(kDsSegs), n_seg - seg0));
        const int nrows = nsg * seg_len;
        for (int r0 = warp * 4; r0 < nrows; r0 += 8 * 4) {
            uint4 u[4][2];
            float acc[4] = {0.f, 0.f, 0.f, 0.f};
#pragma unroll
            for (int k = 0; k < 4; ++k) {
                const int r = r0 + k;
                const uint4* xr = reinterpret_cast<const uint4*>(X + (seg0 * seg_len + r) * static_cast<long long>(lda));
#pragma unroll
                for (int h = 0; h < 2; ++h) {
                    const int c = lane + 32 * h;
                    u[k][h] = (r < nrows && c < chunks) ? __ldg(xr + c) : make_uint4(0, 0, 0, 0);
                }
            }
#pragma unroll
            for (int k = 0; k < 4; ++k) {
                const int r = r0 + k;
                if (r >= nrows) break;
                const float* dob = dout + (seg0 + r / seg_len) * ldo;
#pragma unroll
                for (int h = 0; h < 2; ++h) {
                    const int c = lane + 32 * h;
                    if (c < chunks) {
                        const float4 d0 = *reinterpret_cast<const float4*>(dob + c * 8);
                        const float4 d1 = *reinterpret_cast<const float4*>(dob + c * 8 + 4);
                        const uint4 v = u[k][h];
                        const float2 f0 = unpack_bf16x2(v.x), f1 = unpack_bf16x2(v.y), f2 = unpack_bf16x2(v.z), f3 = unpack_bf16x2(v.w);
                        float a = acc[k];
                        a = fmaf(f0.x, d0.x, a); a = fmaf(f0.y, d0.y, a); a = fmaf(f1.x, d0.z, a); a = fmaf(f1.y, d0.w, a);
                        a = fmaf(f2.x, d1.x, a); a = fmaf(f2.y, d1.y, a); a = fmaf(f3.x, d1.z, a); a = fmaf(f3.y, d1.w, a);
                        acc[k] = a;
                    }
                }
                const __nv_bfloat16* xe = X + (seg0 * seg_len + r) * static_cast<long long>(lda);
                for (int c = 64 + lane; c < chunks; c += 32) {
                    const uint4 v = __ldg(reinterpret_cast<const uint4*>(xe) + c);
                    const uint32_t vw[4] = {v.x, v.y, v.z, v.w};
                    for (int j = 0; j < 4; ++j) {
                        const float2 f = unpack_bf16x2(vw[j]);
                        acc[k] = fmaf(f.x, dob[c * 8 + 2 * j], acc[k]);
                        acc[k] = fmaf(f.y, dob[c * 8 + 2 * j + 1], acc[k]);
                    }
                }
                for (int c = chunks * 8 + lane; c < D; c += 32) acc[k] = fmaf(__bfloat162float(xe[c]), dob[c], acc[k]);
                const float tot = warp_sum(acc[k]);
                if (lane == 0) s_dw[r] = tot;
            }
        }
        __syncthreads();
        for (int r = threadIdx.x; r < nrows; r += blockDim.x) {
            const int sgi = r / seg_len;
            const float* wr = w + (seg0 + sgi) * seg_len;
            const float* dwr = s_dw + sgi * seg_len;
            float dot = 0.f;
            for (int t = 0; t < seg_len; ++t) dot = fmaf(wr[t], dwr[t], dot);
            dscore[seg0 * seg_len + r] = wr[r - sgi * seg_len] * (s_dw[r] - dot);
        }
        __syncthreads();
    }
}
__global__ void __launch_bounds__(256) pool_dscore_warp_kernel(const __nv_bfloat16* __restrict__ X, int lda, int D,
                                                               long long n_seg, int seg_len, const float* __restrict__ w,
                                                               const float* __restrict__ dout, int ldo,
                                                               float* __restrict__ dscore) {
    const int lane = threadIdx.x & 31;
    const int chunks = (D + 7) >> 3;
// ... 932 lines not shown
```

### news-recommendation_b200/csrc/gemm.cu

```cuda
#include <algorithm>
#include <cstdarg>
#include <cstdio>
#include <cstdlib>
#include <cstring>
#include <map>
#include <mutex>
#include <string>
#include <tuple>
#include <vector>

#define NR_OWNS_WATCHDOG 1
#include "nr_epilogues.cuh"
#include "nr_ops.h"

namespace nr {

static_assert(kGemmTileRows == kTileM, "nr_ops.h and nr_gemm.cuh disagree on the gemm_nt tile height");
int read_gru_device_error(int* out4);
int g_launches = 0;

static thread_local char t_err[1024] = "";
void set_error(const char* fmt, ...) {
    va_list ap;
    va_start(ap, fmt);
// ... 771 lines not shown
    bool nz = false;
    for (int i = threadIdx.x; i < d / 2; i += blockDim.x) nz = nz || (row[i] & 0x7fff7fffu) != 0;
    return __syncthreads_or(nz) != 0;
}

__device__ __forceinline__ void write_padding_qkv(const float* bqkv, int T, int sec, int ld3, void* qkv_out, void* vlo_out) {
    const int n3 = 3 * sec;
    auto* qkv = static_cast<__nv_bfloat16*>(qkv_out);
    auto* vlo = static_cast<__nv_bfloat16*>(vlo_out);
    for (int i = blockIdx.x * blockDim.x + threadIdx.x; i < T * ld3; i += gridDim.x * blockDim.x) {
        const int c = i % ld3, r = i / ld3;
        const float y = c < n3 ? bqkv[c] : 0.f;
        const __nv_bfloat16 h = __float2bfloat16_rn(y);
        qkv[i] = h;
        if (vlo != nullptr && c >= 2 * sec && c < n3) vlo[r * sec + c - 2 * sec] = __float2bfloat16_rn(y - __bfloat162float(h));
    }
}

__global__ void __launch_bounds__(kLiveTilesThreads) padding_titles_kernel(const PaddingJob j) {
    const int lane = threadIdx.x & 31, warp = threadIdx.x >> 5, warps = kLiveTilesThreads / 32;
    const bool row0_nonzero = block_row_nonzero(j.row0, j.d);
    if (j.bqkv != nullptr) write_padding_qkv(j.bqkv, j.T, j.sec, j.ld3, j.out.qkv, j.out.v_lo);
    for (int t = blockIdx.x * warps + warp; t < j.num_tiles; t += gridDim.x * warps) {
        const int r0 = t * kTileM, r1 = min(j.M, r0 + kTileM);
        bool live = false;
        for (int s = r0 / j.T; s * j.T < r1; ++s) {
            const long long id = lane < j.T ? j.ids[static_cast<long long>(s) * j.T + lane] : 0;
            const bool pad = __all_sync(0xffffffffu, id == 0) && !row0_nonzero;
            live = live || !pad;
            if (lane == 0 && s * j.T >= r0) j.out.pad[s] = pad ? 1 : 0;
        }
        if (lane == 0) j.out.tile_flags[t] = live ? 1 : 0;
    }
    compact_live_tiles(j.out.tile_flags, j.num_tiles, j.ticket, j.out.live);
}

int padding_titles(const long long* ids, long long n_seq, int T, int d, const void* table, int ld_table, const float* bqkv, int sec,
                   int ld3, PaddingTitles* out, cudaStream_t stream) {
    NR_REQUIRE(T >= 1 && T <= 32 && d % 2 == 0 && ld_table % 8 == 0 && n_seq * T < (1ll << 31), "padding_titles: T=%d d=%d ld=%d", T,
               d, ld_table);
    const int M = static_cast<int>(n_seq * T), num_tiles = ceil_div(M, kTileM);
    const size_t pad_b = round_up(static_cast<int>(n_seq), 16), head_b = round_up(static_cast<int>(pad_b) + 4 * (2 * num_tiles + 2), 128);
    const size_t qkv_b = bqkv ? round_up(T * ld3 * 2, 128) : 0, vlo_b = bqkv ? static_cast<size_t>(T) * sec * 2 : 0;
    char* buf = nullptr;
    NR_CHECK_CUDA(cudaMallocAsync(reinterpret_cast<void**>(&buf), head_b + qkv_b + vlo_b, stream));
    out->base = buf;
    out->pad = reinterpret_cast<unsigned char*>(buf);
    out->tile_flags = reinterpret_cast<int*>(buf + pad_b);
    unsigned* ticket = reinterpret_cast<unsigned*>(out->tile_flags + num_tiles);
    out->live = out->tile_flags + num_tiles + 1;
    out->qkv = bqkv ? buf + head_b : nullptr;
    out->v_lo = bqkv ? static_cast<char*>(out->qkv) + qkv_b : nullptr;
    if (n_seq == 0) return 0;
    NR_CHECK_CUDA(cudaMemsetAsync(ticket, 0, sizeof(unsigned), stream));
    const PaddingJob j{.ids = ids, .n_seq = static_cast<int>(n_seq), .T = T, .d = d, .M = M, .num_tiles = num_tiles,
                       .row0 = static_cast<const uint32_t*>(table), .bqkv = bqkv, .sec = sec, .ld3 = ld3, .out = *out, .ticket = ticket};
    ProfScope ps("padding_titles", M, num_tiles, 0, stream);
    const int blocks = std::max(1, std::min(4 * num_sms(), ceil_div(num_tiles, kLiveTilesThreads / 32)));
    padding_titles_kernel<<<blocks, kLiveTilesThreads, 0, stream>>>(j);
    ++g_launches;
    NR_CHECK_CUDA(cudaGetLastError());
    return 0;
}

void free_padding_titles(PaddingTitles& pt, cudaStream_t stream) {
    if (pt.base != nullptr) cudaFreeAsync(pt.base, stream);
    pt = PaddingTitles{};
}

constexpr int kLiveTitlesPerBlock = 32;

struct LiveJob {
    const long long* ids;
    int n_seq, T, d, M, V, n_blocks;
    const uint32_t* row0;
    const float* bqkv;
    int sec, ld3, ldx;
    const uint4* X;
    uint4* Xc;
    uint4* dqkv_c;
    int* counts;
    int* block_base;
    unsigned* ticket;
    LiveTokens out;
};

__global__ void __launch_bounds__(kLiveTilesThreads) live_classify_kernel(const LiveJob j) {
    const int lane = threadIdx.x & 31, warp = threadIdx.x >> 5, warps = kLiveTilesThreads / 32;
    const bool all_live = j.row0 != nullptr && block_row_nonzero(j.row0, j.d);
    write_padding_qkv(j.bqkv, j.T, j.sec, j.ld3, j.out.qkv, nullptr);
    const int gtid = blockIdx.x * blockDim.x + threadIdx.x, nthreads = gridDim.x * blockDim.x;
    for (int i = gtid; i < (j.M + kTileM - 1) / kTileM; i += nthreads) j.out.tiles[1 + i] = i;
    const int px = j.ldx / 8;
    const int s0 = blockIdx.x * kLiveTitlesPerBlock, s1 = min(j.n_seq, s0 + kLiveTitlesPerBlock);
    int total = 0;
    for (int s = s0 + warp; s < s1; s += warps) {
        const long long id = lane < j.T ? j.ids[static_cast<long long>(s) * j.T + lane] : 0;
        uint32_t mask = __ballot_sync(0xffffffffu, lane < j.T && (all_live || (id >= 1 && id < j.V)));
        if (j.row0 == nullptr) {
            for (uint32_t cand = ((j.T == 32 ? 0u : 1u << j.T) - 1u) & ~mask; cand != 0; cand &= cand - 1) {
                const int r = __ffs(cand) - 1;
                const uint4* x = j.X + (static_cast<long long>(s) * j.T + r) * px;
                uint32_t nz = 0;
                for (int c = lane; c < px; c += 32) {
                    const uint4 v = __ldg(x + c);
                    const int n = min(8, max(0, j.d - 8 * c));
                    const uint32_t w[4] = {v.x, v.y, v.z, v.w};
#pragma unroll
                    for (int k = 0; k < 4; ++k) nz |= w[k] & (2 * k + 1 < n ? 0x7fff7fffu : 2 * k < n ? 0x00007fffu : 0u);
                }
                if (__any_sync(0xffffffffu, nz != 0)) mask |= 1u << r;
            }
        }
        if (lane == 0) {
            j.out.mask[s] = mask;
            j.out.pad[s] = mask == 0 ? 1 : 0;
            j.counts[s] = __popc(mask);
            total += __popc(mask);
        }
    }
    __shared__ int warp_tot[kLiveTilesThreads / 32];
    __shared__ bool last;
    if (lane == 0) warp_tot[warp] = total;
    __syncthreads();
    if (threadIdx.x == 0) {
        int t = 0;
        for (int w = 0; w < warps; ++w) t += warp_tot[w];
        j.block_base[blockIdx.x] = t;
        __threadfence();
        last = atomicAdd(j.ticket, 1u) == gridDim.x - 1;
    }
    __syncthreads();
    if (!last) return;
    __threadfence();
    __shared__ int carry;
    if (threadIdx.x == 0) carry = 0;
    __syncthreads();
    for (int b0 = 0; b0 < j.n_blocks; b0 += kLiveTilesThreads) {
        const int b = b0 + threadIdx.x;
        const int v = b < j.n_blocks ? __ldcg(j.block_base + b) : 0;
        int incl = v;
#pragma unroll
        for (int o = 1; o < 32; o <<= 1) {
            const int y = __shfl_up_sync(0xffffffffu, incl, o);
            if (lane >= o) incl += y;
        }
        if (lane == 31) warp_tot[warp] = incl;
        __syncthreads();
        int base = carry;
        for (int w = 0; w < warp; ++w) base += warp_tot[w];
        if (b < j.n_blocks) j.block_base[b] = base + incl - v;
        __syncthreads();
        if (threadIdx.x == kLiveTilesThreads - 1) carry = base + incl;
        __syncthreads();
    }
    if (threadIdx.x == 0) {
        j.out.offset[j.n_seq] = carry;
        j.out.tiles[0] = (carry + kTileM - 1) / kTileM;
    }
}

__global__ void __launch_bounds__(kLiveTilesThreads) live_compact_kernel(const LiveJob j) {
    const int lane = threadIdx.x & 31, warp = threadIdx.x >> 5, warps = kLiveTilesThreads / 32;
    const int s0 = blockIdx.x * kLiveTitlesPerBlock, s1 = min(j.n_seq, s0 + kLiveTitlesPerBlock);
    static_assert(kLiveTitlesPerBlock == 32, "one warp scans the block's titles");
    __shared__ int off[kLiveTitlesPerBlock];
    if (warp == 0) {
        const int v = s0 + lane < s1 ? j.counts[s0 + lane] : 0;
        int incl = v;
#pragma unroll
        for (int o = 1; o < 32; o <<= 1) {
            const int y = __shfl_up_sync(0xffffffffu, incl, o);
            if (lane >= o) incl += y;
        }
        off[lane] = j.block_base[blockIdx.x] + incl - v;
        if (s0 + lane < s1) j.out.offset[s0 + lane] = off[lane];
    }
    __syncthreads();
    const int px = j.ldx / 8, p3 = j.ld3 / 8;
    if (blockIdx.x == gridDim.x - 1) {
        const int m_live = j.out.offset[j.n_seq];
        const int tail_end = min(j.M, (m_live + kTileM - 1) / kTileM * kTileM);
        for (int r = m_live + threadIdx.x; r < tail_end; r += blockDim.x) j.out.index[r] = -1;
        for (int i = threadIdx.x; i < (tail_end - m_live) * px; i += blockDim.x)
            j.Xc[static_cast<long long>(m_live) * px + i] = make_uint4(0, 0, 0, 0);
        for (int i = threadIdx.x; i < (tail_end - m_live) * p3; i += blockDim.x)
            j.dqkv_c[static_cast<long long>(m_live) * p3 + i] = make_uint4(0, 0, 0, 0);
    }
    __shared__ int src_row[kLiveTilesThreads / 32][32];
    for (int s = s0 + warp; s < s1; s += warps) {
        const uint32_t mask = j.out.mask[s];
        const int dst = off[s - s0], n_live = __popc(mask);
        const int rank = __popc(mask & ((1u << lane) - 1u));
        if (lane < j.T && ((mask >> lane) & 1u)) {
            j.out.index[dst + rank] = s * j.T + lane;
            src_row[warp][rank] = s * j.T + lane;
        }
        __syncwarp();
        const uint4* X = j.X;
        uint4* Xc = j.Xc + static_cast<long long>(dst) * px;
#pragma unroll 4
        for (int i = lane; i < n_live * px; i += 32) {
            const int k = i / px, c = i - k * px;
            Xc[i] = __ldg(X + static_cast<long long>(src_row[warp][k]) * px + c);
        }
        __syncwarp();
    }
}

long long live_tokens_bytes(long long n_seq, int T, int ld3) {
    const long long n = n_seq, M = n_seq * T, nb = (n + kLiveTitlesPerBlock - 1) / kLiveTitlesPerBlock;
    WorkspaceLayout l{nullptr};
    l.take<unsigned char>(n);
    l.take<uint32_t>(n);
    l.take<int>(n);
    l.take<int>(n + 1);
    l.take<int>(M);
    l.take<int>(M / kTileM + 2);
    l.take<int>(nb + 1);
    l.take<__nv_bfloat16>(static_cast<long long>(T) * ld3);
    return l.bytes();
}

int live_tokens(const long long* ids, long long n_seq, int T, int d, const void* table, int ld_table, int V, const float* bqkv,
                int sec, int ld3, const void* X, int ldx, void* Xc, void* dqkv_c, void* buf, long long buf_bytes, LiveTokens* out,
                cudaStream_t stream) {
    NR_REQUIRE(ids && bqkv && X && Xc && dqkv_c && buf, "live_tokens: null operand");
    NR_REQUIRE(T >= 1 && T <= 32 && d % 2 == 0 && ld_table % 8 == 0 && ldx % 8 == 0 && ld3 % 8 == 0 && V >= 1 && n_seq * T < (1ll << 31),
               "live_tokens: T=%d d=%d ld_table=%d ldx=%d ld3=%d V=%d", T, d, ld_table, ldx, ld3, V);
    const auto a16 = [](const void* p) { return (reinterpret_cast<uintptr_t>(p) & 15) == 0; };
    NR_REQUIRE(a16(X) && a16(Xc) && a16(dqkv_c) && a16(buf), "live_tokens: rows not 16-byte aligned");
    NR_REQUIRE(buf_bytes >= live_tokens_bytes(n_seq, T, ld3), "live_tokens: buffer too small (%lld bytes)", buf_bytes);
    const int n = static_cast<int>(n_seq), M = n * T, nb = ceil_div(n, kLiveTitlesPerBlock);
    WorkspaceLayout l{static_cast<char*>(buf)};
    out->pad = l.take<unsigned char>(n);
    out->mask = l.take<uint32_t>(n);
    int* counts = l.take<int>(n);
    out->offset = l.take<int>(n + 1);
    out->index = l.take<int>(M);
    out->tiles = l.take<int>(M / kTileM + 2);
    int* block_base = l.take<int>(nb + 1);
    out->qkv = l.take<__nv_bfloat16>(static_cast<long long>(T) * ld3);
    if (n == 0) return 0;
    unsigned* ticket = reinterpret_cast<unsigned*>(block_base + nb);
    NR_CHECK_CUDA(cudaMemsetAsync(ticket, 0, sizeof(unsigned), stream));
    const LiveJob j{.ids = ids, .n_seq = n, .T = T, .d = d, .M = M, .V = V, .n_blocks = nb, .row0 = static_cast<const uint32_t*>(table),
                    .bqkv = bqkv, .sec = sec, .ld3 = ld3, .ldx = ldx, .X = static_cast<const uint4*>(X), .Xc = static_cast<uint4*>(Xc),
                    .dqkv_c = static_cast<uint4*>(dqkv_c), .counts = counts, .block_base = block_base, .ticket = ticket, .out = *out};
    ProfScope ps("live_tokens", M, n, 0, stream);
    live_classify_kernel<<<nb, kLiveTilesThreads, 0, stream>>>(j);
    ++g_launches;
    NR_CHECK_CUDA(cudaGetLastError());
    live_compact_kernel<<<nb, kLiveTilesThreads, 0, stream>>>(j);
    ++g_launches;
    NR_CHECK_CUDA(cudaGetLastError());
    return 0;
}

int gemm_scatter_emb(const GemmOperands& g, const ScatterEmbCfg& c, cudaStream_t stream) {
    if (g.M == 0) return 0;
    NR_REQUIRE(g.N % 4 == 0 && c.V >= 1, "scatter_emb: N=%d V=%d", g.N, c.V);
    GemmNTPlan plan;
    NR_PROPAGATE(plan_gemm_nt(&plan, g.A, g.M, g.lda, g.W, g.N, g.ldw, g.K, g.taps, g.w_tap_rows, kTileM, num_sms(), 0,
                              kEpiSmemBytes<EpiScatter>, 0));
    NR_PROPAGATE(apply_tap_origin(plan, g));
    const EpiScatter e{.ids = c.ids, .demb = c.demb, .V = c.V, .D = g.N, .rm = to_rm(c.rm), .drop = Dropout::make(c.drop.p, c.drop.seed),
                       .drop_ld = c.drop_ld, .rows = c.rows};
    NR_REQUIRE(c.rows == nullptr || c.rm.seg_in == 0, "scatter_emb: compact rows need the identity row map");
    if (c.tile_list != nullptr) {
        plan.p.tile_list = c.tile_list;
        g_launches += debug_simt_gemm() ? 2 : 1;
        ProfScope ps("gemm_scatter_emb", g.M, g.N, g.K * g.taps, stream);
        return launch_gemm_nt(plan, e, g.A, g.lda, g.W, g.ldw, stream);
    }
    const int num_tiles = plan.p.num_m_tiles;
    int* buf = nullptr;
    NR_CHECK_CUDA(cudaMallocAsync(&buf, sizeof(int) * (2 * static_cast<size_t>(num_tiles) + 2), stream));
    unsigned* ticket = reinterpret_cast<unsigned*>(buf + num_tiles);
    int* list = buf + num_tiles + 1;
    NR_CHECK_CUDA(cudaMemsetAsync(ticket, 0, sizeof(unsigned), stream));
    {
        ProfScope ps("scatter_live_tiles", g.M, num_tiles, 0, stream);
        const int blocks = std::max(1, std::min(4 * num_sms(), ceil_div(num_tiles, kLiveTilesThreads / 32)));
        scatter_live_tiles_kernel<<<blocks, kLiveTilesThreads, 0, stream>>>(c.ids, c.V, e.rm, g.M, num_tiles, buf, ticket, list);
        NR_CHECK_CUDA(cudaGetLastError());
        ++g_launches;
    }
    plan.p.tile_list = list;
    g_launches += debug_simt_gemm() ? 2 : 1;
    int rc;
    {
        ProfScope ps("gemm_scatter_emb", g.M, g.N, g.K * g.taps, stream);
        rc = launch_gemm_nt(plan, e, g.A, g.lda, g.W, g.ldw, stream);
    }
    NR_CHECK_CUDA(cudaFreeAsync(buf, stream));
    return rc;
}

}
```

### news-recommendation_b200/csrc/nr_ops.h

```cpp
#pragma once
#include <cuda_runtime.h>
#include <stdint.h>

namespace nr {

struct DropoutCfg {
    float p;
    uint64_t seed;
};

struct RowMapCfg {
    int seg_in, in_off, seg_len, seg_out, out_off;
};

constexpr int kGemmTileRows = 64;
struct GemmOperands {
    const void* A;
    int M, lda;
    const void* W;
    int N, ldw, K, taps = 1, w_tap_rows = 0, tap_origin = -1;
};

struct StoreCfg {
    void* out;
    int ld_out, out_bf16 = 0, relu = 0;
    int tanh = 0;
    const void* dtanh_src = nullptr;
    int dtanh_ld = 0;
    const float* bias = nullptr;
    RowMapCfg rm = {};
    DropoutCfg drop = {};
    int ones_col = -1, ones_zero_upto = 0;
    void* lo_out = nullptr;
    int ld_lo = 0, lo_col0 = 0;
    int accumulate = 0;
    int rows_per_tile = kGemmTileRows;
    const int* tile_list = nullptr;
};
int gemm_store(const GemmOperands& g, const StoreCfg& c, cudaStream_t stream);
bool gemm_store_lo_supported(int N, int K, int lo_col0);

int gemm_additive_pool(const void* X, int M, int lda, int D, const void* Wa, int q, int ldw, const float* ba,
                       const float* qv, int seg_len, float* out, int ldo, float* w_out, cudaStream_t stream,
                       const void* X_lo = nullptr);

int gemm_additive_dpre(const void* X, int M, int lda, int D, const void* Wa, int q, int ldw, const float* ba,
                       const float* qv, const float* dscore, void* dpre, int ld_dpre, float* dqv,
                       cudaStream_t stream);
int additive_dpre_check(int q, int D, int ld_dpre);

struct PoolDInputCfg {
    const float *w, *dout;
    int ldo, seg_len;
    void* dx;
    int ld_dx;
    RowMapCfg rm = {};
    int zero_pad_rows = 0;
    DropoutCfg drop = {};
    const void* relu_src = nullptr;
    int relu_ld = 0;
};
int gemm_pool_dinput(const GemmOperands& g, const PoolDInputCfg& c, cudaStream_t stream);
int pool_dinput_check(const GemmOperands& g, const PoolDInputCfg& c);

struct ScatterEmbCfg {
    const long long* ids;
    float* demb;
    int V;
    RowMapCfg rm = {};
    DropoutCfg drop = {};
    int drop_ld = 0;
    const int* rows = nullptr;
    const int* tile_list = nullptr;
};
int gemm_scatter_emb(const GemmOperands& g, const ScatterEmbCfg& c, cudaStream_t stream);

int gemm_tn_accumulate(const void* A, int Kr, int Ma, int lda, const void* B, int b_rows, int b_cols, int ldb,
                       int b_col0, int Nb, int b_row_shift, float* D, int ldd, cudaStream_t stream, const int* k_list = nullptr);
int gemm_weight_grad(const void* dY, int M, int N, int ld_dy, const void* X, int K, int ldx, float* dW_ext, cudaStream_t stream,
                     int x_row_shift = 0, const int* k_list = nullptr);

struct PaddingTitles {
    unsigned char* pad = nullptr;
    int* tile_flags = nullptr;
    int* live = nullptr;
    void* qkv = nullptr;
    void* v_lo = nullptr;
    void* base = nullptr;
};
int padding_titles(const long long* ids, long long n_seq, int T, int d, const void* table, int ld_table, const float* bqkv, int sec,
                   int ld3, PaddingTitles* out, cudaStream_t stream);
void free_padding_titles(PaddingTitles& pt, cudaStream_t stream);

struct LiveTokens {
    unsigned char* pad = nullptr;
    uint32_t* mask = nullptr;
    int* offset = nullptr;
    int* index = nullptr;
    int* tiles = nullptr;
    void* qkv = nullptr;
};
long long live_tokens_bytes(long long n_seq, int T, int ld3);
int live_tokens(const long long* ids, long long n_seq, int T, int d, const void* table, int ld_table, int V, const float* bqkv,
                int sec, int ld3, const void* X, int ldx, void* Xc, void* dqkv_c, void* buf, long long buf_bytes, LiveTokens* out,
                cudaStream_t stream);

struct Bf16Rows {
    const float* src;
    long long n_rows;
    int T = 1, D;
    long long s_seq, s_tok = 0, s_col = 1;
    const float* pos = nullptr;
    int width;
    void* hi = nullptr;
    int ld_hi = 0, ones_col = 0;
    void* lo = nullptr;
    int ld_lo = 0;
};
struct Bf16Op {
    const char* name;
    int blocks_per_sm;
};
inline constexpr Bf16Op kCastPad{"cast_pad", 16}, kCastPadMany{"cast_pad_many", 4}, kRowsToBf16{"rows_to_bf16", 6},
    kRowsToBf16Hilo{"rows_to_bf16_hilo", 8}, kRowsToBf16Planes{"rows_to_bf16_planes", 8}, kRowsToBf16Lo{"rows_to_bf16_lo", 8};
constexpr int kBf16RowsJobs = 8;
int rows_to_bf16(const Bf16Rows* jobs, int n_jobs, Bf16Op op, cudaStream_t stream);
inline int rows_to_bf16(const Bf16Rows& job, Bf16Op op, cudaStream_t stream) { return rows_to_bf16(&job, 1, op, stream); }
int sum_over_seq(const float* src, long long n_seq, long long L, float* dst, cudaStream_t stream);
int gather_rows(const long long* ids, long long n_tok, int T, const void* table, int V, int D, int ld_table, void* X,
                int ld_x, int padded, DropoutCfg drop, int* bad_id_flag, cudaStream_t stream);
struct TitleBwdLive {
    const LiveTokens* tokens;
    float* dbias;
    int ld_dbias;
};
int mhsa_core_fwd(const void* qkv, int ld_qkv, int sec, long long n_seq, int T, int heads, int dk, void* ctx, int ld_ctx,
                  DropoutCfg drop, cudaStream_t stream);
int mhsa_core_bwd(const void* qkv, int ld_qkv, int sec, const void* dctx, int ld_dctx, long long n_seq, int T, int heads, int dk,
                  void* dqkv, int ld_dqkv, cudaStream_t stream, const TitleBwdLive* live = nullptr);
bool mhsa_title_fwd_supported(int T, int dk, int heads, int sec, int ld_qkv, int ld_ctx);
int mhsa_title_fwd(const void* qkv, int ld_qkv, int sec, long long n_seq, int heads, void* ctx, int ld_ctx, DropoutCfg drop,
                   cudaStream_t stream, const void* v_lo = nullptr, int ld_vlo = 0, void* ctx_lo = nullptr,
                   const PaddingTitles* pad = nullptr);
bool mhsa_title_bwd_supported(int T, int dk, int heads, int sec, int ld_qkv, int ld_dctx, int ld_dqkv);
int mhsa_title_bwd(const void* qkv, int ld_qkv, int sec, const void* dctx, int ld_dctx, long long n_seq, int heads, void* dqkv,
                   int ld_dqkv, cudaStream_t stream, const TitleBwdLive* live = nullptr);
int pool_dscore(const void* X, int lda, int D, long long n_seg, int seg_len, const float* w, const float* dout, int ldo,
                float* dscore, cudaStream_t stream);
int pool_dscore_check(int lda, int D, int seg_len, int ldo);
int dot_score_fwd(const float* cand, const float* user, int B, int C, int D, float* logits, cudaStream_t stream);
int dot_score_bwd(const float* cand, const float* user, const float* dlogits, int B, int C, int D, float* dcand,
                  float* duser, cudaStream_t stream);

int accumulate_ext_grad(float* ext, int rows, int ld, int D, float* dW, float* db, cudaStream_t stream);
int relu_bwd_to_bf16(const float* dy, const float* relu_out, long long n, int N, int ld_dy, void* dst, int ldn, cudaStream_t stream);
int embedding_f32_fwd(const long long* ids, long long n, const float* table, int V, int D, float* out, int* bad_id_flag,
                      cudaStream_t stream);
int embedding_f32_bwd(const long long* ids, long long n, const float* dout, int V, int D, float* dtable, cudaStream_t stream);


int gru_persistent_supported(int B, int Hd);
int gru_fwd_persistent(int B, int S, int Hd, int ldh, int ldg, const float* gi, const void* whh, const float* bhh, const float* h0,
                       const long long* len, float* gh, float* hs, void* hb, float* out, cudaStream_t stream);
void set_gru_stepwise(int on);

int mhsa_f32_fwd(const float* qkv, int ld, int sec, long long n_seq, int T, int heads, int dk, void* c_hi, void* c_lo, int ldc,
                 cudaStream_t stream);
int segment_dot(const float* news, long long n_news, int D, const long long* cand, long long n_cand, const long long* seg_offsets,
                long long n_seg, const float* user, float* scores, int* bad_flag, cudaStream_t stream);
int impression_metrics(const float* scores, const unsigned char* labels, const long long* seg_offsets, long long n_seg, double* metrics,
                       int* bad_label_flag, cudaStream_t stream);
int impression_ranks(const float* scores, const long long* seg_offsets, long long n_seg, int* ranks, int* bad_score_flag,
                     cudaStream_t stream);
long long prediction_scan_bytes(long long n_seg);
int prediction_line_offsets(const long long* ids, const int* ranks, const long long* seg_offsets, long long n_seg, long long* line_offsets,
                            void* workspace, long long workspace_bytes, cudaStream_t stream);
int prediction_text(const long long* ids, const int* ranks, const long long* seg_offsets, long long n_seg, const long long* line_offsets,
                    char* text, cudaStream_t stream);

int slots_device_readable(const void* const* slots, int n);
int pack_slots(const void* const* slots, int H, int C, int B, int L, long long* out, cudaStream_t stream);
constexpr int kFeedFields = 8;
struct FeedField {
    const int* table;
    int width;
    long long* out;
};
struct FeedRecords {
    const int* records;
    long long *user, *length, *clicked;
};
int feed_gather(const FeedField* fields, int n_fields, const int* behaviors, int H, int C, FeedRecords rec, const long long* rows, int B,
                cudaStream_t stream);
int sample_negatives(const int* cand_rows, const unsigned char* labels, const long long* imp_offsets, long long n_imp, const long long* row_offsets,
                     int K, unsigned long long seed, long long epoch, int* behaviors, int H, cudaStream_t stream);
long long topk_dot_workspace(long long n_users, long long n_news, int D, int k);
int topk_dot(const float* users, long long n_users, int ld_users, const float* news, long long n_news, int ld_news, int D, int k,
             const long long* excl_offsets, const long long* excl_rows, const int* categories, int max_per_category,
             const long long* row_lo, const long long* row_hi, long long* idx, float* score, int* bad_row_flag, int* bad_score_flag, void* workspace, long long workspace_bytes, cudaStream_t stream);
long long pool_ranks_workspace(long long n_rows, long long n_news, int D);
int pool_ranks(const float* queries, long long n_rows, int ld_queries, const float* news, long long n_news, int ld_news, int D,
               const long long* tgt_offsets, const long long* tgt_rows, const long long* excl_offsets, const long long* excl_rows,
               const long long* row_lo, const long long* row_hi, long long* rank, float* score, int* bad_row_flag, int* bad_score_flag, int* target_flag, void* workspace,
               long long workspace_bytes, cudaStream_t stream);
long long topk_archive_workspace(long long n_users, int P, long long n_news, int F, int hidden, int k);
int topk_archive(const float* archive, long long n_users, int P, const float* news, long long n_news, int F, const float* W1,
                 const float* b1, int hidden, const float* w2, const float* b2, int k, const long long* excl_offsets,
                 const long long* excl_rows, const int* categories, int max_per_category, const long long* row_lo,
                 const long long* row_hi, long long* idx, float* score,
                 int* bad_row_flag, int* bad_score_flag, void* workspace, long long workspace_bytes, cudaStream_t stream);
long long pool_ranks_archive_workspace(long long n_rows, int P, long long n_news, int F, int hidden);
int pool_ranks_archive(const float* archive, long long n_rows, int P, const float* news, long long n_news, int F, const float* W1,
                       const float* b1, int hidden, const float* w2, const float* b2, const long long* tgt_offsets,
                       const long long* tgt_rows, const long long* excl_offsets, const long long* excl_rows,
                       const long long* row_lo, const long long* row_hi, long long* rank,
                       float* score, int* bad_row_flag, int* bad_score_flag, int* target_flag, void* workspace,
                       long long workspace_bytes, cudaStream_t stream);
int mmr_rerank(const float* news, long long n_news, int ld_news, int D, const long long* sl_idx, const float* sl_score,
               long long n_users, int depth, int k, float lambda, long long* idx, float* score, int* bad_row_flag,
               cudaStream_t stream);
int list_stats(const float* news, long long n_news, int ld_news, int D, const long long* idx, long long n_rows, int k,
               const int* categories, const int* ks, int n_ks, double* pair_sum, int* distinct, int* bad_row_flag,
               cudaStream_t stream);
int num_sms();
extern int g_launches;

// ... 26 lines not shown
```

### news-recommendation_b200/src/newsrec_b200/__init__.py

```python
from __future__ import annotations

import ctypes as C
import os

_HERE = os.path.dirname(os.path.abspath(__file__))
LIB_PATH = os.path.join(_HERE, "libnewsrec_b200.so")

_vp, _i, _ll, _f, _ull = C.c_void_p, C.c_int, C.c_longlong, C.c_float, C.c_ulonglong


class MhsaEncoderFwdArgs(C.Structure):
    _fields_ = [
        ("n_seq", _ll), ("T", _i), ("d", _i), ("heads", _i), ("q", _i), ("ldx", _i), ("ld3", _i),
        ("ids", _vp), ("table_bf16", _vp), ("V", _i),
        ("dense", _vp), ("dense_s_seq", _ll), ("dense_s_tok", _ll), ("dense_s_col", _ll),
        ("wqkv_bf16", _vp), ("bqkv", _vp), ("wa_bf16", _vp), ("ba", _vp), ("qv", _vp),
        ("p_drop", _f), ("seed", _ull),
        ("X_bf16", _vp), ("QKV_bf16", _vp), ("C_bf16", _vp), ("w", _vp), ("out", _vp), ("bad_id_flag", _vp),
        ("C_lo_bf16", _vp),
        ("wqkv_kcat_bf16", _vp), ("X_kcat_bf16", _vp), ("QKV_f32", _vp),
        ("V_lo_bf16", _vp),
        ("dense_pos", _vp),
    ]


class MhsaEncoderBwdArgs(C.Structure):
    _fields_ = [
        ("n_seq", _ll), ("T", _i), ("d", _i), ("heads", _i), ("q", _i), ("ldx", _i), ("ld3", _i), ("ldq", _i),
        ("ids", _vp), ("V", _i),
        ("wqkvT_bf16", _vp), ("wa_bf16", _vp), ("waT_bf16", _vp), ("ba", _vp), ("qv", _vp),
        ("p_drop", _f), ("seed", _ull),
        ("X_bf16", _vp), ("QKV_bf16", _vp), ("C_bf16", _vp), ("w", _vp), ("dout", _vp),
        ("dWqkv_ext", _vp), ("dWa_ext", _vp), ("dqv", _vp), ("demb", _vp), ("ddense", _vp),
        ("workspace", _vp), ("workspace_bytes", _ll),
        ("wqkv_bf16", _vp), ("bqkv", _vp), ("emb_grad_ready_event", _vp),
        ("dpos", _vp), ("table_bf16", _vp),
    ]


class CnnEncoderFwdArgs(C.Structure):
    _fields_ = [
        ("n_seq", _ll), ("T", _i), ("d", _i), ("F", _i), ("q", _i), ("ldx", _i), ("ldf", _i),
        ("ids", _vp), ("table_bf16", _vp), ("V", _i),
        ("wconv_bf16", _vp), ("bconv", _vp), ("wa_bf16", _vp), ("ba", _vp), ("qv", _vp),
        ("p_drop", _f), ("seed", _ull),
        ("Xp_bf16", _vp), ("Y_bf16", _vp), ("w", _vp), ("out", _vp), ("bad_id_flag", _vp),
        ("Y_lo_bf16", _vp), ("window", _i),
    ]


class CnnEncoderBwdArgs(C.Structure):
    _fields_ = [
        ("n_seq", _ll), ("T", _i), ("d", _i), ("F", _i), ("q", _i), ("ldx", _i), ("ldf", _i), ("ldq", _i),
        ("ids", _vp), ("V", _i),
        ("wconvT_bf16", _vp), ("wa_bf16", _vp), ("waT_bf16", _vp), ("ba", _vp), ("qv", _vp),
        ("p_drop", _f), ("seed", _ull),
        ("Xp_bf16", _vp), ("Y_bf16", _vp), ("w", _vp), ("dout", _vp),
        ("dWconv_ext", _vp), ("dWa_ext", _vp), ("dqv", _vp), ("demb", _vp),
        ("workspace", _vp), ("workspace_bytes", _ll), ("window", _i),
    ]


class KcnnEncoderFwdArgs(C.Structure):
    _fields_ = [
        ("n_seq", _ll), ("T", _i), ("d", _i), ("de", _i), ("F", _i), ("q", _i), ("n_win", _i), ("win", _i * 4),
        ("ldx", _i), ("lde", _i), ("ldf", _i), ("ldo", _i),
        ("word_ids", _vp), ("entity_ids", _vp), ("word_table_bf16", _vp), ("V", _i), ("entity_table_bf16", _vp), ("Ve", _i),
        ("mT_bf16", _vp), ("mb", _vp), ("wconv_bf16", _vp), ("bconv", _vp), ("wa_bf16", _vp), ("ba", _vp), ("qv", _vp),
        ("X2_bf16", _vp), ("E_bf16", _vp), ("Y_bf16", _vp), ("w", _vp), ("out", _vp), ("bad_id_flag", _vp),
    ]


class KcnnEncoderBwdArgs(C.Structure):
    _fields_ = [
        ("n_seq", _ll), ("T", _i), ("d", _i), ("de", _i), ("F", _i), ("q", _i), ("n_win", _i), ("win", _i * 4),
        ("ldx", _i), ("lde", _i), ("ldf", _i), ("ldo", _i), ("ldq", _i),
        ("word_ids", _vp), ("entity_ids", _vp), ("V", _i), ("Ve", _i),
        ("wT_word_bf16", _vp), ("wT_entity_bf16", _vp), ("m_bf16", _vp), ("wa_bf16", _vp), ("waT_bf16", _vp), ("ba", _vp),
        ("qv", _vp), ("X2_bf16", _vp), ("E_bf16", _vp), ("Y_bf16", _vp), ("w", _vp), ("dout", _vp),
        ("dWconv_ext", _vp), ("dM_ext", _vp), ("dWa_ext", _vp), ("dqv", _vp), ("dword", _vp), ("dentity", _vp),
        ("workspace", _vp), ("workspace_bytes", _ll),
    ]


class GruFwdArgs(C.Structure):
    _fields_ = [
        ("B", _i), ("S", _i), ("D", _i), ("Hd", _i),
        ("x", _vp), ("x_s_b", _ll), ("x_s_t", _ll), ("x_s_c", _ll),
        ("len", _vp), ("h0", _vp), ("wih_bf16", _vp), ("whh_bf16", _vp), ("bih", _vp), ("bhh", _vp),
        ("xb", _vp), ("gi", _vp), ("gh", _vp), ("hs", _vp), ("hb", _vp), ("out", _vp),
        ("x_lo_bf16", _vp),
    ]


class GruBwdArgs(C.Structure):
    _fields_ = [
        ("B", _i), ("S", _i), ("D", _i), ("Hd", _i),
        ("len", _vp), ("wihT_bf16", _vp), ("whhT_bf16", _vp),
        ("xb", _vp), ("gi", _vp), ("gh", _vp), ("hs", _vp), ("hb", _vp),
        ("dout", _vp), ("dWih_ext", _vp), ("dWhh_ext", _vp), ("dx", _vp), ("dh0", _vp),
        ("workspace", _vp), ("workspace_bytes", _ll),
    ]


class GemmStoreArgs(C.Structure):
    _fields_ = [
        ("A", _vp), ("M", _i), ("lda", _i), ("W", _vp), ("N", _i), ("ldw", _i), ("K", _i), ("taps", _i), ("w_tap_rows", _i),
        ("tap_origin", _i),
        ("out", _vp), ("ld_out", _i), ("out_bf16", _i), ("relu", _i), ("tanh", _i), ("dtanh_src", _vp), ("dtanh_ld", _i),
        ("bias", _vp),
        ("rm_seg_in", _i), ("rm_in_off", _i), ("rm_seg_len", _i), ("rm_seg_out", _i), ("rm_out_off", _i),
        ("p_drop", _f), ("seed", _ull),
        ("ones_col", _i), ("ones_zero_upto", _i), ("lo_out", _vp), ("ld_lo", _i), ("lo_col0", _i), ("accumulate", _i),
        ("rows_per_tile", _i),
    ]


class FeedField(C.Structure):
    _fields_ = [("table", _vp), ("width", _i), ("out", _vp)]


SIGNATURES = {
    "nr_version": (_i, []),
    "nr_last_error": (C.c_char_p, []),
    "nr_device_error": (_i, [C.POINTER(_i * 4)]),
    "nr_launch_count": (_ll, []),
    "nr_num_sms": (_i, []),
    "nr_debug_set_simt_gemm": (None, [_i]),
    "nr_debug_set_gru_stepwise": (None, [_i]),
    "nr_debug_gemm_store": (_i, [C.POINTER(GemmStoreArgs), _vp]),
    "nr_has_triage_backends": (_i, []),
    "nr_reserve_sms_for_comm": (None, [_i]),
    "nr_debug_set_gemm_timing": (None, [_vp, _i]),
    "nr_debug_live_tokens": (_i, [_vp, _ll, _i, _i, _vp, _i, _vp, _i, _vp, _vp, _vp, _vp, _vp, _vp, _vp, _vp, _vp]),
    "nr_profile_enable": (None, [_i]),
    "nr_profile_context": (None, [C.c_char_p]),
    "nr_profile_report": (_i, [C.c_char_p, _i]),
    "nr_cast_pad_bf16": (_i, [_vp, _i, _i, _i, _vp, _i, _i, _vp]),
    "nr_cast_pad_bf16_many": (_i, [_i, _vp, _vp, _vp, _vp, _vp, _vp, _vp, _vp]),
    "nr_rows_to_bf16": (_i, [_vp, _ll, _i, _ll, _ll, _vp, _i, _vp]),
    "nr_rows_to_bf16_hilo": (_i, [_vp, _ll, _i, _ll, _ll, _vp, _vp, _i, _vp]),
    "nr_gather_rows": (_i, [_vp, _ll, _i, _vp, _i, _i, _i, _vp, _i, _f, _ull, _vp, _vp]),
    "nr_linear": (_i, [_vp, _i, _i, _vp, _i, _i, _i, _i, _i, _i, _vp, _i, _vp, _i, _i, _vp]),
    "nr_gemm_tn": (_i, [_vp, _i, _i, _i, _vp, _i, _i, _i, _i, _i, _i, _vp, _i, _vp]),
    "nr_mhsa_core_fwd": (_i, [_vp, _i, _i, _ll, _i, _i, _i, _vp, _i, _f, _ull, _vp]),
    "nr_mhsa_core_bwd": (_i, [_vp, _i, _i, _vp, _i, _ll, _i, _i, _i, _vp, _i, _vp]),
    "nr_additive_attention_fwd": (_i, [_vp, _ll, _i, _i, _i, _vp, _i, _i, _vp, _vp, _vp, _i, _vp, _vp]),
    "nr_additive_attention_fwd_hilo": (_i, [_vp, _vp, _ll, _i, _i, _i, _vp, _i, _i, _vp, _vp, _vp, _i, _vp, _vp]),
    "nr_additive_attention_bwd_workspace": (_ll, [_ll, _i, _i]),
    "nr_additive_attention_bwd": (_i, [_vp, _ll, _i, _i, _i, _vp, _vp, _i, _i, _i, _vp, _vp, _vp, _vp, _i, _vp, _i,
                                        _vp, _vp, _vp, _ll, _vp]),
    "nr_dot_score_fwd": (_i, [_vp, _vp, _i, _i, _i, _vp, _vp]),
    "nr_slots_device_readable": (_i, [_vp, _i]),
    "nr_pack_slots": (_i, [_vp, _i, _i, _i, _i, _vp, _vp]),
    "nr_feed_gather": (_i, [C.POINTER(FeedField), _i, _vp, _i, _i, _vp, _vp, _i, _vp, _vp, _vp, _vp]),
    "nr_sample_negatives": (_i, [_vp, _vp, _vp, _ll, _vp, _i, _ull, _ll, _vp, _i, _vp]),
    "nr_segment_dot": (_i, [_vp, _ll, _i, _vp, _ll, _vp, _ll, _vp, _vp, _vp, _vp]),
    "nr_impression_metrics": (_i, [_vp, _vp, _vp, _ll, _vp, _vp, _vp]),
    "nr_impression_ranks": (_i, [_vp, _vp, _ll, _vp, _vp, _vp]),
    "nr_topk_dot_workspace": (_ll, [_ll, _ll, _i, _i]),
    "nr_topk_dot": (_i, [_vp, _ll, _i, _vp, _ll, _i, _i, _i, _vp, _vp, _vp, _vp, _vp, _vp, _vp, _ll, _vp]),
    "nr_topk_dot_capped": (_i, [_vp, _ll, _i, _vp, _ll, _i, _i, _i, _vp, _vp, _vp, _i, _vp, _vp, _vp, _vp, _vp, _ll, _vp]),
    "nr_topk_dot_ranged": (_i, [_vp, _ll, _i, _vp, _ll, _i, _i, _i, _vp, _vp, _vp, _i, _vp, _vp, _vp, _vp, _vp, _vp, _vp, _ll,
                                _vp]),
    "nr_mmr_rerank": (_i, [_vp, _ll, _i, _i, _vp, _vp, _ll, _i, _i, _f, _vp, _vp, _vp, _vp]),
    "nr_list_stats": (_i, [_vp, _ll, _i, _i, _vp, _ll, _i, _vp, _vp, _i, _vp, _vp, _vp, _vp]),
    "nr_pool_ranks_workspace": (_ll, [_ll, _ll, _i]),
    "nr_pool_ranks": (_i, [_vp, _ll, _i, _vp, _ll, _i, _i, _vp, _vp, _vp, _vp, _vp, _vp, _vp, _vp, _vp, _vp, _ll, _vp]),
    "nr_pool_ranks_ranged": (_i, [_vp, _ll, _i, _vp, _ll, _i, _i, _vp, _vp, _vp, _vp, _vp, _vp, _vp, _vp, _vp, _vp, _vp, _vp,
                                  _ll, _vp]),
    "nr_topk_archive_workspace": (_ll, [_ll, _i, _ll, _i, _i, _i]),
    "nr_topk_archive": (_i, [_vp, _ll, _i, _vp, _ll, _i, _vp, _vp, _i, _vp, _vp, _i, _vp, _vp, _vp, _i, _vp, _vp, _vp, _vp,
                             _vp, _ll, _vp]),
    "nr_topk_archive_ranged": (_i, [_vp, _ll, _i, _vp, _ll, _i, _vp, _vp, _i, _vp, _vp, _i, _vp, _vp, _vp, _i, _vp, _vp, _vp,
                                    _vp, _vp, _vp, _vp, _ll, _vp]),
    "nr_pool_ranks_archive_workspace": (_ll, [_ll, _i, _ll, _i, _i]),
    "nr_pool_ranks_archive": (_i, [_vp, _ll, _i, _vp, _ll, _i, _vp, _vp, _i, _vp, _vp, _vp, _vp, _vp, _vp, _vp, _vp, _vp, _vp,
                                   _vp, _vp, _ll, _vp]),
    "nr_pool_ranks_archive_ranged": (_i, [_vp, _ll, _i, _vp, _ll, _i, _vp, _vp, _i, _vp, _vp, _vp, _vp, _vp, _vp, _vp, _vp,
                                          _vp, _vp, _vp, _vp, _vp, _vp, _ll, _vp]),
    "nr_prediction_line_offsets_workspace": (_ll, [_ll]),
    "nr_prediction_line_offsets": (_i, [_vp, _vp, _vp, _ll, _vp, _vp, _ll, _vp]),
    "nr_prediction_text": (_i, [_vp, _vp, _vp, _ll, _vp, _vp, _vp]),
    "nr_accumulate_ext_grad": (_i, [_vp, _i, _i, _i, _vp, _vp, _vp]),
    "nr_dot_score_bwd": (_i, [_vp, _vp, _vp, _i, _i, _i, _vp, _vp, _vp]),
    "nr_mhsa_accurate_supported": (_i, [_i, _i, _i]),
    "nr_mhsa_encoder_fwd": (_i, [C.POINTER(MhsaEncoderFwdArgs), _vp]),
    "nr_mhsa_encoder_bwd_workspace": (_ll, [_ll, _i, _i, _i]),
    "nr_mhsa_encoder_bwd": (_i, [C.POINTER(MhsaEncoderBwdArgs), _vp]),
    "nr_cnn_encoder_fwd": (_i, [C.POINTER(CnnEncoderFwdArgs), _vp]),
    "nr_cnn_encoder_bwd_workspace": (_ll, [_ll, _i, _i, _i]),
    "nr_cnn_encoder_bwd": (_i, [C.POINTER(CnnEncoderBwdArgs), _vp]),
    "nr_kcnn_encoder_fwd": (_i, [C.POINTER(KcnnEncoderFwdArgs), _vp]),
    "nr_kcnn_encoder_bwd_workspace": (_ll, [_ll, _i, _i, _i, _i, _i]),
    "nr_kcnn_encoder_bwd": (_i, [C.POINTER(KcnnEncoderBwdArgs), _vp]),
    "nr_linear_rows_fwd": (_i, [_vp, _ll, _i, _ll, _ll, _vp, _i, _vp, _i, _i, _vp, _i, _vp, _i, _vp]),
    "nr_linear_rows_bwd": (_i, [_vp, _vp, _ll, _i, _i, _vp, _i, _vp, _i, _i, _vp, _i, _vp, _vp, _i, _vp]),
    "nr_embedding_f32_fwd": (_i, [_vp, _ll, _vp, _i, _i, _vp, _vp, _vp]),
    "nr_embedding_f32_bwd": (_i, [_vp, _ll, _vp, _i, _i, _vp, _vp]),
    "nr_element_encoder_fwd": (_i, [_vp, _ll, _vp, _i, _i, _i, _vp, _vp, _i, _vp, _vp, _vp, _vp]),
    "nr_element_encoder_bwd": (_i, [_vp, _ll, _vp, _vp, _i, _vp, _i, _vp, _i, _i, _vp, _vp, _vp, _i, _vp]),
    "nr_gru_fwd": (_i, [C.POINTER(GruFwdArgs), _vp]),
    "nr_gru_persistent_supported": (_i, [_i, _i]),
    "nr_gru_bwd_workspace": (_ll, [_i, _i, _i, _i]),
    "nr_gru_bwd": (_i, [C.POINTER(GruBwdArgs), _vp]),
    "nr_archive_user_fwd": (_i, [_vp, _ll, _i, _i, _i, _vp, _vp, _vp, _vp]),
    "nr_archive_user_bwd_workspace": (_ll, [_ll, _i, _i]),
    "nr_archive_user_bwd": (_i, [_vp, _ll, _i, _i, _i, _vp, _vp, _vp, _vp, _vp, _vp, _ll, _vp]),
    "nr_archive_score_fwd": (_i, [_vp, _ll, _i, _vp, _ll, _vp, _ll, _vp, _i, _vp, _vp, _i, _vp, _vp, _vp, _vp, _vp]),
    "nr_archive_score_bwd_workspace": (_ll, [_ll, _i, _i]),
    "nr_archive_score_bwd": (_i, [_vp, _ll, _i, _vp, _ll, _vp, _ll, _vp, _i, _vp, _vp, _i, _vp, _vp, _vp, _vp, _vp,
                                   _vp, _vp, _vp, _vp, _vp, _ll, _vp]),
    "nr_dkn_user_fwd": (_i, [_vp, _ll, _i, _i, _vp, _i, _vp, _vp, _vp]),
    "nr_dkn_user_bwd_workspace": (_ll, [_ll, _i]),
    "nr_dkn_user_bwd": (_i, [_vp, _ll, _i, _i, _vp, _i, _vp, _vp, _vp, _vp, _vp, _vp, _ll, _vp]),
}

_lib = None


class NewsrecError(RuntimeError):
    pass


def load_library(path: str | None = None):
    global _lib
    if _lib is not None and path is None:
        return _lib
    p = path or LIB_PATH
    if not os.path.exists(p):
        raise NewsrecError(
            f"{p} not found: build it with `python __graft_entry__.py build` (or `make -C news-recommendation_b200/csrc`). "
            "There is no CPU / PyTorch fallback for the hot path.")
    lib = C.CDLL(p)
    for name, (res, args) in SIGNATURES.items():
        fn = getattr(lib, name)
        fn.restype = res
        fn.argtypes = args
    if path is None:
        _lib = lib
    return lib


def check(rc: int, what: str = ""):
    if rc != 0:
        lib = load_library()
        msg = lib.nr_last_error().decode(errors="replace")
        raise NewsrecError(f"{what} failed (code {rc}): {msg}")


def require_cuda():
    import torch
    if not torch.cuda.is_available():
        raise NewsrecError("newsrec_b200 needs a CUDA (sm_90a) device: the hot path has no CPU fallback")
    return torch.device("cuda", torch.cuda.current_device())


def profile_report() -> dict:
    import json
    buf = C.create_string_buffer(1 << 16)
    n = load_library().nr_profile_report(buf, len(buf))
    if n < 0:
        raise NewsrecError("profile report does not fit the buffer")
    return {k: tuple(v) for k, v in json.loads(buf.value.decode()).items()}


def launch_count() -> int:
    return int(load_library().nr_launch_count())
```

### news-recommendation_b200/src/newsrec_b200/ops.py

```python
from __future__ import annotations

import ctypes as C
import numbers
import os

import torch

from . import (MhsaEncoderBwdArgs, MhsaEncoderFwdArgs, NewsrecError, check, load_library, require_cuda)


def ru8(x: int) -> int:
    return (x + 7) // 8 * 8


def ru16(x: int) -> int:
    return (x + 15) // 16 * 16


def _p(t):
    return C.c_void_p(t.data_ptr()) if t is not None else C.c_void_p(0)


def _stream():
    return C.c_void_p(torch.cuda.current_stream().cuda_stream)
# ... 107 lines not shown


def mhsa_operands(cache: OperandCache, prefix, Wq, bq, Wk, bk, Wv, bv, Wa, ba, qv):
    d, q = Wq.shape[0], Wa.shape[0]
    ldx, ldq = ru8(d + 1), ru16(q)
    ld3 = qkv_pitches(d)[1]

    def build(Wq, bq, Wk, bk, Wv, bv, Wa, ba, qv):
        wqkv = stack_qkv(Wq, Wk, Wv)
        w, wT, wa, waT = cast_pad_many([(wqkv, ldx, False), (wqkv, ld3, True), (Wa, ldx, False), (Wa, ldq, True)])
        return dict(wqkv=w, wqkvT=wT, bqkv=stack_qkv(bq, bk, bv).contiguous(), wa=wa, waT=waT,
                    ba=ba.float().contiguous(), qv=qv.float().contiguous())

    return cache.get(prefix, (Wq, bq, Wk, bk, Wv, bv, Wa, ba, qv), build)


def table_operand(cache: OperandCache, name, weight):
    ldx = ru8(weight.shape[1] + 1)
    return cache.get(name, (weight,), lambda w: cast_pad(w, ldx))


class MhsaPoolEncoderFn(torch.autograd.Function):

    @staticmethod
    def forward(ctx, ids, dense, emb_w, Wq, bq, Wk, bk, Wv, bv, Wa, ba, qv, heads, p_drop, cache, prefix, bad_flag, precise=False,
                pos=None):
        lib = load_library()
        dev = require_cuda()
        d, q = Wq.shape[0], Wa.shape[0]
        ldx = ru8(d + 1)
        sec, ld3 = qkv_pitches(d)
        ops = mhsa_operands(cache, prefix, Wq, bq, Wk, bk, Wv, bv, Wa, ba, qv)
        a = MhsaEncoderFwdArgs()
        if ids is not None:
            n_seq, T = ids.shape
            ids = ids.contiguous()
            table = table_operand(cache, prefix + ".table", emb_w)
            a.ids, a.table_bf16, a.V = _p(ids), _p(table), emb_w.shape[0]
            a.dense = None
        else:
            n_seq, T, dd = dense.shape
            if dd != d:
                raise NewsrecError(f"user encoder input width {dd} != model width {d}")
            dense = dense.float()
            a.ids, a.table_bf16, a.V = None, None, 0
            a.dense = _p(dense)
            a.dense_s_seq, a.dense_s_tok, a.dense_s_col = dense.stride()
            table = None
        if pos is not None:
            if ids is not None:
                raise NewsrecError("a positional addend applies to the dense (user-level) input only")
            if tuple(pos.shape) != (T, d):
                raise NewsrecError(f"positional addend of shape {tuple(pos.shape)} for inputs of {T} positions x {d}")
            a.dense_pos = _p(pos.detach().float().contiguous())
        n_tok = n_seq * T
        need_bwd = any(ctx.needs_input_grad)
        mode = precise if isinstance(precise, str) else ("accurate" if precise else "fast")
        accurate = ids is not None and mode == "accurate" and bool(lib.nr_mhsa_accurate_supported(T, d, heads))
        precise_dense = ids is None and mode == "accurate"
        X = QKV = C_lo = V_lo = None
        X = torch.empty((n_tok, ldx), dtype=torch.bfloat16, device=dev)
        if not precise_dense:
            QKV = torch.empty((n_tok, ld3), dtype=torch.bfloat16, device=dev)
        Cx = torch.empty((n_tok, ldx), dtype=torch.bfloat16, device=dev)
        w = torch.empty((n_tok,), dtype=torch.float32, device=dev)
        out = torch.empty((n_seq, d), dtype=torch.float32, device=dev)
        seed = next_seed() if p_drop > 0 else 0
        a.n_seq, a.T, a.d, a.heads, a.q, a.ldx, a.ld3 = n_seq, T, d, heads, q, ldx, ld3
        a.wqkv_bf16, a.bqkv, a.wa_bf16, a.ba, a.qv = _p(ops["wqkv"]), _p(ops["bqkv"]), _p(ops["wa"]), _p(ops["ba"]), _p(ops["qv"])
        a.p_drop, a.seed = float(p_drop), seed
        if accurate:
            C_lo = torch.empty((n_tok, ldx), dtype=torch.bfloat16, device=dev)
            V_lo = torch.empty((n_tok, sec), dtype=torch.bfloat16, device=dev)
            a.C_lo_bf16, a.V_lo_bf16 = _p(C_lo), _p(V_lo)
        keep = None
        if precise_dense:
            kcat = cache.get(prefix + ".kcat", (Wq, Wk, Wv), lambda Wq, Wk, Wv: cast_pad(
                torch.cat((torch.nn.functional.pad(stack_qkv(Wq, Wk, Wv), (0, ldx - d)),) * 2, dim=1), 2 * ldx))
            C_lo = torch.empty((n_tok, ldx), dtype=torch.bfloat16, device=dev)
            keep = (torch.empty((n_tok, 2 * ldx), dtype=torch.bfloat16, device=dev), torch.empty((n_tok, 3 * sec), dtype=torch.float32, device=dev))
            a.wqkv_kcat_bf16, a.X_kcat_bf16, a.QKV_f32, a.C_lo_bf16 = _p(kcat), _p(keep[0]), _p(keep[1]), _p(C_lo)
        a.X_bf16, a.QKV_bf16, a.C_bf16, a.w, a.out = _p(X), _p(QKV), _p(Cx), _p(w), _p(out)
        a.bad_id_flag = _p(bad_flag)
        check(lib.nr_mhsa_encoder_fwd(C.byref(a), _stream()), "nr_mhsa_encoder_fwd")
        if need_bwd:
            ctx.save_for_backward(X, QKV if QKV is not None else torch.empty(0, device=dev), Cx, w,
                                  ids if ids is not None else torch.empty(0, device=dev))
        ctx.meta = dict(n_seq=n_seq, T=T, d=d, q=q, heads=heads, p_drop=float(p_drop), seed=seed, ops=ops,
                        has_ids=ids is not None, V=emb_w.shape[0] if ids is not None else 0,
                        dense_shape=None if dense is None else tuple(dense.shape),
                        params=(emb_w, Wq, bq, Wk, bk, Wv, bv, Wa, ba, qv), cache=cache, prefix=prefix,
                        pos=pos, table=table)
        return out

    @staticmethod
    def backward(ctx, dout):
        lib = load_library()
        X, QKV, Cx, w, ids = ctx.saved_tensors
        m = ctx.meta
        dev = X.device
        d, q, T, n_seq = m["d"], m["q"], m["T"], m["n_seq"]
        ldx, ldq = ru8(d + 1), ru16(q)
        sec, ld3 = qkv_pitches(d)
        ops = m["ops"]
        dout = dout.contiguous().float()
        emb_w, Wq, bq, Wk, bk, Wv, bv, Wa, ba, qv = m["params"]
        sinks = [grad_sink(t) for t in (Wq, bq, Wk, bk, Wv, bv, Wa, ba, qv)]
        direct = all(g is not None for g in sinks)
        if direct:
            ws_grads = m["cache"].get(m["prefix"] + ".grad_ws", (), lambda: dict(
                dWqkv=torch.zeros((3 * sec, ldx), dtype=torch.float32, device=dev),
                dWa=torch.zeros((q, ldx), dtype=torch.float32, device=dev)))
            dWqkv, dWa, dqv = ws_grads["dWqkv"], ws_grads["dWa"], sinks[8]
        else:
            dWqkv = torch.zeros((3 * sec, ldx), dtype=torch.float32, device=dev)
            dWa = torch.zeros((q, ldx), dtype=torch.float32, device=dev)
            dqv = torch.zeros((q,), dtype=torch.float32, device=dev)
        demb = ddense = None
        emb_direct = False
        if m["has_ids"]:
            demb = grad_sink(emb_w)
            emb_direct = demb is not None
            if not emb_direct:
                demb = torch.zeros((m["V"], d), dtype=torch.float32, device=dev)
        else:
            ddense = torch.empty((n_seq * T, d), dtype=torch.float32, device=dev)
        dpos, pos_direct = None, False
        if m["pos"] is not None:
            dpos = grad_sink(m["pos"])
            pos_direct = dpos is not None
            if not pos_direct:
                dpos = torch.zeros((T, d), dtype=torch.float32, device=dev)
        ws_bytes = int(lib.nr_mhsa_encoder_bwd_workspace(n_seq, T, d, q))
        ws = torch.empty((ws_bytes,), dtype=torch.uint8, device=dev)
        a = MhsaEncoderBwdArgs()
        a.n_seq, a.T, a.d, a.heads, a.q, a.ldx, a.ld3, a.ldq = n_seq, T, d, m["heads"], q, ldx, ld3, ldq
        a.ids = _p(ids) if m["has_ids"] else None
        a.V = m["V"]
        a.table_bf16 = _p(m["table"]) if m["has_ids"] else None
        a.wqkvT_bf16, a.wa_bf16, a.waT_bf16, a.ba, a.qv = _p(ops["wqkvT"]), _p(ops["wa"]), _p(ops["waT"]), _p(ops["ba"]), _p(ops["qv"])
        a.p_drop, a.seed = m["p_drop"], m["seed"]
        a.X_bf16, a.QKV_bf16, a.C_bf16, a.w, a.dout = _p(X), (_p(QKV) if QKV.numel() else None), _p(Cx), _p(w), _p(dout)
        a.wqkv_bf16, a.bqkv = _p(ops["wqkv"]), _p(ops["bqkv"])
        hook = getattr(demb, GRAD_READY_ATTR, None) if (m["has_ids"] and emb_direct) else None
        if hook is not None:
            a.emb_grad_ready_event = C.c_void_p(hook["event"].cuda_event)
            hook["recorded"] = True
        a.dWqkv_ext, a.dWa_ext, a.dqv = _p(dWqkv), _p(dWa), _p(dqv)
        a.demb, a.ddense, a.dpos = _p(demb), _p(ddense), _p(dpos)
        a.workspace, a.workspace_bytes = _p(ws), ws_bytes
        check(lib.nr_mhsa_encoder_bwd(C.byref(a), _stream()), "nr_mhsa_encoder_bwd")
        g_dense = ddense.view(m["dense_shape"]) if ddense is not None else None
        g_emb = None if emb_direct else demb
        g_pos = None if pos_direct else dpos
        if direct:
            for i in range(3):
                check(lib.nr_accumulate_ext_grad(_p(dWqkv[i * sec:i * sec + d]), d, ldx, d, _p(sinks[2 * i]), _p(sinks[2 * i + 1]),
                                                 _stream()), "nr_accumulate_ext_grad")
            check(lib.nr_accumulate_ext_grad(_p(dWa), q, ldx, d, _p(sinks[6]), _p(sinks[7]), _stream()), "nr_accumulate_ext_grad")
            return (None, g_dense, g_emb) + (None,) * 15 + (g_pos,)
        gW = [dWqkv[i * sec:i * sec + d, :d].contiguous() for i in range(3)]
        gb = [dWqkv[i * sec:i * sec + d, d].contiguous() for i in range(3)]
        return (None, g_dense, g_emb, gW[0], gb[0], gW[1], gb[1], gW[2], gb[2],
                dWa[:, :d].contiguous(), dWa[:, d].contiguous(), dqv, None, None, None, None, None, None, g_pos)


class AdditiveAttentionFn(torch.autograd.Function):

    @staticmethod
    def forward(ctx, x, Wa, ba, qv, cache, prefix, precision="fast"):
        lib = load_library()
        dev = require_cuda()
        if precision not in ("fast", "accurate"):
            raise NewsrecError(f"additive attention precision must be 'fast' or 'accurate' (got {precision!r})")
        N, S, D = x.shape
        q = Wa.shape[0]
        ldx, ldq = ru8(D + 1), ru16(q)
        ops = cache.get(prefix, (Wa, ba, qv), lambda Wa, ba, qv: dict(
            wa=cast_pad(Wa, ldx), waT=cast_pad(Wa, ldq, transpose=True), ba=ba.float().contiguous(),
            qv=qv.float().contiguous()))
        xf = x.float()
        X = torch.empty((N * S, ldx), dtype=torch.bfloat16, device=dev)
        xs = xf.reshape(N * S, D) if xf.is_contiguous() else xf.contiguous().view(N * S, D)
        out = torch.empty((N, D), dtype=torch.float32, device=dev)
        w = torch.empty((N * S,), dtype=torch.float32, device=dev)
        if precision == "accurate":
            X_lo = torch.empty((N * S, ldx), dtype=torch.bfloat16, device=dev)
            check(lib.nr_rows_to_bf16_hilo(_p(xs), N * S, D, xs.stride(0), xs.stride(1), _p(X), _p(X_lo), ldx, _stream()),
                  "nr_rows_to_bf16_hilo")
            check(lib.nr_additive_attention_fwd_hilo(_p(X), _p(X_lo), N, S, D, ldx, _p(ops["wa"]), q, ldx, _p(ops["ba"]),
                                                     _p(ops["qv"]), _p(out), D, _p(w), _stream()), "nr_additive_attention_fwd_hilo")
        else:
            check(lib.nr_rows_to_bf16(_p(xs), N * S, D, xs.stride(0), xs.stride(1), _p(X), ldx, _stream()), "nr_rows_to_bf16")
            check(lib.nr_additive_attention_fwd(_p(X), N, S, D, ldx, _p(ops["wa"]), q, ldx, _p(ops["ba"]), _p(ops["qv"]),
                                                _p(out), D, _p(w), _stream()), "nr_additive_attention_fwd")
        ctx.save_for_backward(X, w)
        ctx.meta = dict(N=N, S=S, D=D, q=q, ops=ops)
        return out

    @staticmethod
    def backward(ctx, dout):
        lib = load_library()
        X, w = ctx.saved_tensors
        m = ctx.meta
        N, S, D, q, ops = m["N"], m["S"], m["D"], m["q"], m["ops"]
        dev = X.device
        ldx, ldq = ru8(D + 1), ru16(q)
        dout = dout.contiguous().float()
        dX = torch.empty((N * S, ldx), dtype=torch.bfloat16, device=dev)
        dWa = torch.zeros((q, ldx), dtype=torch.float32, device=dev)
        dqv = torch.zeros((q,), dtype=torch.float32, device=dev)
        ws_bytes = int(lib.nr_additive_attention_bwd_workspace(N, S, q))
        ws = torch.empty((ws_bytes,), dtype=torch.uint8, device=dev)
        check(lib.nr_additive_attention_bwd(_p(X), N, S, D, ldx, _p(ops["wa"]), _p(ops["waT"]), q, ldx, ldq, _p(ops["ba"]),
                                            _p(ops["qv"]), _p(w), _p(dout), D, _p(dX), ldx, _p(dWa), _p(dqv), _p(ws),
                                            ws_bytes, _stream()), "nr_additive_attention_bwd")
        gx = dX[:, :D].float().view(N, S, D)
        return gx, dWa[:, :D].contiguous(), dWa[:, D].contiguous(), dqv, None, None, None


class DotScoreFn(torch.autograd.Function):

    @staticmethod
    def forward(ctx, cand, user):
        lib = load_library()
        dev = require_cuda()
        cand = cand.contiguous().float()
        user = user.contiguous().float()
        B, Cn, D = cand.shape
        logits = torch.empty((B, Cn), dtype=torch.float32, device=dev)
        check(lib.nr_dot_score_fwd(_p(cand), _p(user), B, Cn, D, _p(logits), _stream()), "nr_dot_score_fwd")
        ctx.save_for_backward(cand, user)
        return logits
# ... 459 lines not shown
```

Before: 88800.

## Compute live-token compaction in forward and reuse it in backward

```diff
diff --git a/include/newsrec_b200.h b/include/newsrec_b200.h
--- a/include/newsrec_b200.h
+++ b/include/newsrec_b200.h
@@ -203,8 +203,11 @@
     float* QKV_f32;
     void* V_lo_bf16;
     const float* dense_pos;
+    void* live;
+    long long live_bytes;
 } nr_mhsa_encoder_fwd_args;
 int nr_mhsa_accurate_supported(int T, int d, int heads);
+long long nr_mhsa_encoder_live_bytes(long long n_seq, int T, int d);
 int nr_mhsa_encoder_fwd(const nr_mhsa_encoder_fwd_args* a, void* stream);
 
 typedef struct {
@@ -236,6 +239,8 @@
     void* emb_grad_ready_event;
     float* dpos;
     const void* table_bf16;
+    void* live;
+    long long live_bytes;
 } nr_mhsa_encoder_bwd_args;
 long long nr_mhsa_encoder_bwd_workspace(long long n_seq, int T, int d, int q);
 int nr_mhsa_encoder_bwd(const nr_mhsa_encoder_bwd_args* a, void* stream);
diff --git a/news-recommendation_b200/csrc/abi.cu b/news-recommendation_b200/csrc/abi.cu
--- a/news-recommendation_b200/csrc/abi.cu
+++ b/news-recommendation_b200/csrc/abi.cu
@@ -46,7 +46,7 @@
                "nr_debug_live_tokens: null operand or n_seq=%lld d=%d", n_seq, d);
     const cudaStream_t st = as_stream(stream);
     const int sec = (d + 7) & ~7, ld3 = (3 * sec + 15) & ~15;
-    const long long bytes = live_tokens_bytes(n_seq, T, ld3);
+    const long long bytes = live_tokens_bytes(n_seq, T, sec, ld3);
     char* buf = nullptr;
     NR_CHECK_CUDA(cudaMallocAsync(reinterpret_cast<void**>(&buf), bytes, st));
     LiveTokens lt;
@@ -396,6 +396,10 @@
 int nr_mhsa_accurate_supported(int T, int d, int heads) {
     return mhsa_accurate_shape(T, d, heads, (3 * qkv_section(d) + 15) & ~15, (d + 8) & ~7) ? 1 : 0;
 }
+long long nr_mhsa_encoder_live_bytes(long long n_seq, int T, int d) {
+    NR_REQUIRE(n_seq >= 0 && T >= 1 && d >= 1, "nr_mhsa_encoder_live_bytes: n_seq=%lld T=%d d=%d", n_seq, T, d);
+    return live_tokens_bytes(n_seq, T, qkv_section(d), (3 * qkv_section(d) + 15) & ~15);
+}
 
 struct PaddingScope {
     PaddingTitles pt;
@@ -418,11 +422,39 @@
     NR_REQUIRE(precise_dense || (a->wqkv_bf16 && a->bqkv && a->X_bf16 && a->QKV_bf16), "nr_mhsa_encoder_fwd: null operand");
     NR_REQUIRE(a->p_drop >= 0.f && a->p_drop < 1.f, "nr_mhsa_encoder_fwd: dropout p=%f", a->p_drop);
     NR_REQUIRE(a->dense_pos == nullptr || a->dense != nullptr, "nr_mhsa_encoder_fwd: dense_pos needs the dense (user-level) variant");
+    const int sec = qkv_section(a->d);
+    if (a->live != nullptr) {
+        NR_REQUIRE(a->ids != nullptr && mhsa_title_fwd_supported(a->T, a->d / a->heads, a->heads, sec, a->ld3, a->ldx) &&
+                       (a->V_lo_bf16 == nullptr || mhsa_accurate_shape(a->T, a->d, a->heads, a->ld3, a->ldx)),
+                   "nr_mhsa_encoder_fwd: live tokens need the ids variant at the title-level attention kernel's shape");
+        NR_REQUIRE(a->live_bytes >= live_tokens_bytes(a->n_seq, a->T, sec, a->ld3), "nr_mhsa_encoder_fwd: live buffer too small (%lld bytes)",
+                   a->live_bytes);
+    }
     if (a->n_seq == 0) return 0;
     const int M = static_cast<int>(a->n_seq * a->T);
     const cudaStream_t st = as_stream(stream);
-    const int sec = qkv_section(a->d);
     prof_context(a->ids != nullptr ? "news.fwd" : "user.fwd");
+    if (a->live != nullptr) {
+        NR_REQUIRE(a->table_bf16 && a->bad_id_flag && a->V >= 1 && (a->V_lo_bf16 == nullptr || a->C_lo_bf16 != nullptr),
+                   "nr_mhsa_encoder_fwd: table / bad_id_flag missing (or V_lo_bf16 without C_lo_bf16)");
+        LiveTokens live;
+        NR_PROPAGATE(live_tokens(a->ids, a->n_seq, a->T, a->d, a->table_bf16, a->ldx, a->V, a->bqkv, sec, a->ld3, nullptr, a->ldx, nullptr,
+                                 nullptr, a->live, a->live_bytes, &live, st, a->bad_id_flag));
+        NR_PROPAGATE(gather_rows(a->ids, M, a->T, a->table_bf16, a->V, a->d, a->ldx, a->X_bf16, a->ldx, 0, DropoutCfg{a->p_drop, a->seed},
+                                 a->bad_id_flag, st, &live));
+        const bool hilo = a->V_lo_bf16 != nullptr;
+        NR_PROPAGATE(gemm_store({.A = a->X_bf16, .M = M, .lda = a->ldx, .W = a->wqkv_bf16, .N = 3 * sec, .ldw = a->ldx, .K = a->d},
+                                {.out = a->QKV_bf16, .ld_out = a->ld3, .out_bf16 = 1, .bias = a->bqkv, .lo_out = a->V_lo_bf16,
+                                 .ld_lo = hilo ? sec : 0, .lo_col0 = hilo ? 2 * sec : 0, .tile_list = live.tiles}, st));
+        {
+            ProfScope ps(hilo ? "mhsa_core_fwd_hilo" : "mhsa_core_fwd", static_cast<int>(a->n_seq), a->T, a->d, st);
+            NR_PROPAGATE(mhsa_title_fwd(a->QKV_bf16, a->ld3, sec, a->n_seq, a->heads, a->C_bf16, a->ldx, context_dropout(a->p_drop, a->seed),
+                                        st, a->V_lo_bf16, hilo ? sec : 0, hilo ? a->C_lo_bf16 : nullptr, nullptr, &live));
+        }
+        NR_PROPAGATE(gemm_additive_pool(a->C_bf16, M, a->ldx, a->d, a->wa_bf16, a->q, a->ldx, a->ba, a->qv, a->T, a->out, a->d,
+                                        a->w, st, hilo ? a->C_lo_bf16 : nullptr));
+        return 0;
+    }
     if (a->dense != nullptr && a->C_lo_bf16 != nullptr) {
         NR_REQUIRE(a->wqkv_kcat_bf16 && a->X_kcat_bf16 && a->QKV_f32 && a->bqkv && a->X_bf16,
                    "nr_mhsa_encoder_fwd: precise dense variant needs wqkv_kcat_bf16 / X_kcat_bf16 / QKV_f32 / bqkv / X_bf16");
@@ -487,7 +519,7 @@
         : WorkspaceLayout{static_cast<char*>(base)}, dscore(take<float>(n_seq * T)), dpre(take<__nv_bfloat16>(n_seq * T * round_up(q, 16))),
           dC(take<__nv_bfloat16>(n_seq * T * round_up(d + 1, 8))), dQKV(take<__nv_bfloat16>(n_seq * T * round_up(3 * qkv_section(d), 16))),
           QKV(take<__nv_bfloat16>(n_seq * T * round_up(3 * qkv_section(d), 16))),
-          live_bytes(live_tokens_bytes(n_seq, T, round_up(3 * qkv_section(d), 16))) {
+          live_bytes(live_tokens_bytes(n_seq, T, qkv_section(d), round_up(3 * qkv_section(d), 16))) {
         live = take<char>(live_bytes);
     }
 };
@@ -511,10 +543,17 @@
     NR_REQUIRE(a->table_bf16 == nullptr || a->ids != nullptr, "nr_mhsa_encoder_bwd: table_bf16 needs the ids (news) variant");
     const MhsaBwdWorkspace ws(a->workspace, a->n_seq, a->T, a->d, a->q);
     NR_REQUIRE(a->workspace_bytes >= ws.bytes(), "nr_mhsa_encoder_bwd: workspace too small (%lld bytes)", a->workspace_bytes);
+    const int sec = qkv_section(a->d);
+    const bool title_shape = mhsa_title_bwd_supported(a->T, a->d / a->heads, a->heads, sec, a->ld3, a->ldx, a->ld3);
+    if (a->live != nullptr) {
+        NR_REQUIRE(a->ids != nullptr && title_shape && a->QKV_bf16 != nullptr,
+                   "nr_mhsa_encoder_bwd: live tokens need the ids variant at the title-level attention kernel's shape");
+        NR_REQUIRE(a->live_bytes >= live_tokens_bytes(a->n_seq, a->T, sec, a->ld3), "nr_mhsa_encoder_bwd: live buffer too small (%lld bytes)",
+                   a->live_bytes);
+    }
     if (a->n_seq == 0) return 0;
     const int M = static_cast<int>(a->n_seq * a->T);
     const cudaStream_t st = as_stream(stream);
-    const int sec = qkv_section(a->d);
 
     prof_context(a->ids != nullptr ? "news.bwd" : "user.bwd");
     const void* QKV = a->QKV_bf16;
@@ -530,13 +569,17 @@
                                   {.w = a->w, .dout = a->dout, .ldo = a->d, .seg_len = a->T, .dx = ws.dC, .ld_dx = a->ldx,
                                    .drop = context_dropout(a->ids != nullptr ? a->p_drop : 0.f, a->seed)}, st));
     LiveTokens live;
-    const bool compact = a->ids != nullptr && mhsa_title_bwd_supported(a->T, a->d / a->heads, a->heads, sec, a->ld3, a->ldx, a->ld3);
-    if (compact) {
+    const bool compact = a->ids != nullptr && title_shape;
+    const bool from_fwd = a->live != nullptr;
+    if (from_fwd) {
+        live = live_tokens_view(a->live, a->n_seq, a->T, sec, a->ld3);
+        NR_PROPAGATE(live_zero_tail(live, a->n_seq, a->T, ws.dQKV, a->ld3, st));
+    } else if (compact) {
         NR_REQUIRE(a->V >= 1, "nr_mhsa_encoder_bwd: V=%d", a->V);
         NR_PROPAGATE(live_tokens(a->ids, a->n_seq, a->T, a->d, a->table_bf16, a->ldx, a->V, a->bqkv, sec, a->ld3, a->X_bf16, a->ldx, ws.QKV,
                                  ws.dQKV, ws.live, ws.live_bytes, &live, st));
     }
-    const TitleBwdLive title_live{.tokens = &live, .dbias = a->dWqkv_ext + a->d, .ld_dbias = a->ldx};
+    const TitleBwdLive title_live{.tokens = &live, .dbias = a->dWqkv_ext + a->d, .ld_dbias = a->ldx, .compact_qkv = from_fwd ? 1 : 0};
     NR_PROPAGATE(mhsa_core_bwd(QKV, a->ld3, sec, ws.dC, a->ldx, a->n_seq, a->T, a->heads, a->d / a->heads, ws.dQKV, a->ld3, st,
                                compact ? &title_live : nullptr));
     if (a->ids != nullptr) {
@@ -551,8 +594,8 @@
         if (a->dpos != nullptr) NR_PROPAGATE(sum_over_seq(a->ddense, a->n_seq, static_cast<long long>(a->T) * a->d, a->dpos, st));
     }
     NR_PROPAGATE(gemm_weight_grad(ws.dpre, M, a->q, a->ldq, a->C_bf16, a->d, a->ldx, a->dWa_ext, st));
-    NR_PROPAGATE(gemm_weight_grad(ws.dQKV, M, 3 * sec, a->ld3, compact ? ws.QKV : a->X_bf16, a->d, a->ldx, a->dWqkv_ext, st, 0,
-                                  live.tiles));
+    NR_PROPAGATE(gemm_weight_grad(ws.dQKV, M, 3 * sec, a->ld3, compact && !from_fwd ? ws.QKV : a->X_bf16, a->d, a->ldx, a->dWqkv_ext, st,
+                                  0, live.tiles));
     return 0;
 }
 
diff --git a/news-recommendation_b200/csrc/attn_title.cu b/news-recommendation_b200/csrc/attn_title.cu
--- a/news-recommendation_b200/csrc/attn_title.cu
+++ b/news-recommendation_b200/csrc/attn_title.cu
@@ -28,6 +28,20 @@
 constexpr int kScrPitch = 48;
 constexpr int kScrTile = 24 * kScrPitch;
 constexpr int kScrWarp = 2 * kScrTile;
+
+__device__ __forceinline__ void row_offsets(const uint32_t* mask, int title, uint32_t pitch, uint32_t to_bias, int lane, uint32_t ro[3]) {
+    const uint32_t m = mask != nullptr ? __ldg(mask + title) : 0u;
+#pragma unroll
+    for (int j = 0; j < 3; ++j) {
+        const uint32_t r = 8u * j + static_cast<uint32_t>(lane & 7);
+        const bool live = r < kT && ((m >> r) & 1u);
+        ro[j] = mask == nullptr ? r * pitch : live ? static_cast<uint32_t>(__popc(m & ((1u << r) - 1u))) * pitch : to_bias;
+    }
+}
+__device__ __forceinline__ void copy_bias_row(uint8_t* dst, const void* src, uint32_t row_bytes, uint32_t pitch) {
+    for (uint32_t i = threadIdx.x; i < pitch / 16u; i += blockDim.x)
+        reinterpret_cast<uint4*>(dst)[i] = i < row_bytes / 16u ? __ldg(static_cast<const uint4*>(src) + i) : make_uint4(0, 0, 0, 0);
+}
 
 struct Params {
     int n_seq, heads;
@@ -45,6 +59,8 @@
     uint32_t ld_out, row_bytes;
     float* dbias;
     int ld_dbias;
+    int compact;
+    const void* bias;
 };
 
 __device__ __forceinline__ uint32_t sel(bool keep, uint32_t v) { return keep ? v : 0u; }
@@ -65,6 +81,8 @@
     uint64_t* const oempty = bars + 2 * kIn + kOut;
 
     for (uint32_t i = tid; i < bar_off / 16; i += blockDim.x) reinterpret_cast<uint4*>(base_ptr)[i] = make_uint4(0, 0, 0, 0);
+    const uint32_t bias_off = bar_off + 128u;
+    if (p.compact) copy_bias_row(base_ptr + bias_off, p.bias, 3u * p.sec2, p.pq);
     if (tid == 0) {
         for (int i = 0; i < kIn; ++i) {
             mbar_init(&full[i], 1);
@@ -91,8 +109,9 @@
                 const int s = it % kIn;
                 const int title = static_cast<int>(blockIdx.x) + it * static_cast<int>(gridDim.x), row = title * kT;
                 const bool pad = p.pad != nullptr && p.pad[title] != 0;
-                mbar_arrive_expect_tx(&full[s], p.tx);
-                tma_load_2d(base_ptr + s * p.in_stage, pad ? &tm_pad : &tm_qkv, &full[s], 0, pad ? 0 : row);
+                const bool none = pad && p.compact;
+                mbar_arrive_expect_tx(&full[s], none ? p.tx - kT * p.pq : p.tx);
+                if (!none) tma_load_2d(base_ptr + s * p.in_stage, pad ? &tm_pad : &tm_qkv, &full[s], 0, pad ? 0 : p.compact ? p.offset[title] : row);
                 tma_load_2d(base_ptr + s * p.in_stage + p.qkv_tile, &tm_dc, &full[s], 0, row);
             };
             for (int it = 0; it < kIn && it < n_my; ++it) load(it);
@@ -135,7 +154,7 @@
     const bool c2ok = odd || t4 < 2;
     const bool lo2 = t4 < 2;
     const uint32_t pq = p.pq, pc = p.pc;
-    const uint32_t r15q = (lane & 15) * pq, r7q = (lane & 7) * pq, r15c = (lane & 15) * pc, r7c = (lane & 7) * pc;
+    const uint32_t r15c = (lane & 15) * pc, r7c = (lane & 7) * pc;
     const uint32_t hi = (lane >> 4) * 16u, mid = ((lane >> 3) & 1) * 16u;
     const uint32_t ps = scr_base + h * kScrWarp, dsb = ps + kScrTile;
     const uint32_t at0 = ((lane & 7) + (lane >> 4) * 8) * kScrPitch + mid;
@@ -154,37 +173,41 @@
         const int s = it % kIn, o = it % kOut;
         const uint32_t Q = in_base + s * p.in_stage, K = Q + p.sec2, V = K + p.sec2, G = Q + p.qkv_tile;
         const uint32_t ob = out_base + o * p.out_stage;
-        const uint32_t dead = p.mask != nullptr ? ~__ldg(p.mask + static_cast<int>(blockIdx.x) + it * static_cast<int>(gridDim.x)) : 0u;
+        const int title = static_cast<int>(blockIdx.x) + it * static_cast<int>(gridDim.x);
+        const uint32_t dead = p.mask != nullptr ? ~__ldg(p.mask + title) : 0u;
+        uint32_t ro[3];
+        row_offsets(p.compact ? p.mask : nullptr, title, pq, base + bias_off - Q, lane, ro);
+        const uint32_t r15 = (lane & 8) ? ro[1] : ro[0];
         f_wait(&full[s], (it / kIn) & 1, 72);
 
         uint32_t kb16[3][2], kb8[3], vb16[3][2], vb8[3], kt16[3][2], kt8[3];
 #pragma unroll
         for (int nt = 0; nt < 3; ++nt) {
-            lds_x2(kb16[nt], K + k16b + nt * 8 * pq + r7q + mid);
-            lds_x2(vb16[nt], V + k16b + nt * 8 * pq + r7q + mid);
-            lds_x1(&kb8[nt], K + k8b + nt * 8 * pq + r7q);
-            lds_x1(&vb8[nt], V + k8b + nt * 8 * pq + r7q);
+            lds_x2(kb16[nt], K + k16b + ro[nt] + mid);
+            lds_x2(vb16[nt], V + k16b + ro[nt] + mid);
+            lds_x1(&kb8[nt], K + k8b + ro[nt]);
+            lds_x1(&vb8[nt], V + k8b + ro[nt]);
             kb8[nt] = sel(v8, kb8[nt]);
             vb8[nt] = sel(v8, vb8[nt]);
-            lds_x2_t(kt16[nt], K + gb + 16 * nt + r15q);
-            lds_x1_t(&kt8[nt], K + gb + 16 * nt + 16 * pq + r7q);
+            lds_x2_t(kt16[nt], K + gb + 16 * nt + r15);
+            lds_x1_t(&kt8[nt], K + gb + 16 * nt + ro[2]);
             kt8[nt] = sel(lo2, kt8[nt]);
         }
 #pragma unroll
         for (int mt = 0; mt < 2; ++mt) {
             uint32_t aq[4], ag[4], aq8[2], ag8[2];
             if (mt == 0) {
-                lds_x4(aq, Q + k16b + r15q + hi);
+                lds_x4(aq, Q + k16b + r15 + hi);
                 lds_x4(ag, G + k16b + r15c + hi);
-                lds_x2(aq8, Q + k8b + r15q);
+                lds_x2(aq8, Q + k8b + r15);
                 lds_x2(ag8, G + k8b + r15c);
             } else {
                 uint32_t t[2];
-                lds_x2(t, Q + k16b + 16 * pq + r7q + mid);
+                lds_x2(t, Q + k16b + ro[2] + mid);
                 aq[0] = t[0], aq[1] = 0u, aq[2] = t[1], aq[3] = 0u;
                 lds_x2(t, G + k16b + 16 * pc + r7c + mid);
                 ag[0] = t[0], ag[1] = 0u, ag[2] = t[1], ag[3] = 0u;
-                lds_x1(&aq8[0], Q + k8b + 16 * pq + r7q);
+                lds_x1(&aq8[0], Q + k8b + ro[2]);
                 lds_x1(&ag8[0], G + k8b + 16 * pc + r7c);
                 aq8[1] = ag8[1] = 0u;
             }
@@ -295,9 +318,9 @@
         uint32_t qt16[3][2], qt8[3], gt16[3][2], gt8[3];
 #pragma unroll
         for (int nd = 0; nd < 3; ++nd) {
-            lds_x2_t(qt16[nd], Q + gb + 16 * nd + r15q);
+            lds_x2_t(qt16[nd], Q + gb + 16 * nd + r15);
             lds_x2_t(gt16[nd], G + gb + 16 * nd + r15c);
-            lds_x1_t(&qt8[nd], Q + gb + 16 * nd + 16 * pq + r7q);
+            lds_x1_t(&qt8[nd], Q + gb + 16 * nd + ro[2]);
             lds_x1_t(&gt8[nd], G + gb + 16 * nd + 16 * pc + r7c);
             qt8[nd] = sel(lo2, qt8[nd]);
             gt8[nd] = sel(lo2, gt8[nd]);
@@ -379,6 +402,9 @@
     float sc;
     Dropout drop;
     const unsigned char* pad;
+    const uint32_t* mask;
+    const int* offset;
+    const void *bias_q, *bias_v;
 };
 
 template <bool HILO>
@@ -399,6 +425,11 @@
     uint64_t* const ofull = bars + 2 * kIn;
     uint64_t* const oempty = bars + 2 * kIn + kOut;
     for (uint32_t i = tid; i < bar_off / 16; i += blockDim.x) reinterpret_cast<uint4*>(base_ptr)[i] = make_uint4(0, 0, 0, 0);
+    const uint32_t bias_q = bar_off + 128u, bias_v = bias_q + p.pq;
+    if (p.mask != nullptr) {
+        copy_bias_row(base_ptr + bias_q, p.bias_q, 3u * p.sec2, p.pq);
+        if (HILO) copy_bias_row(base_ptr + bias_v, p.bias_v, p.sec2, p.pv);
+    }
     __syncthreads();
     if (tid < kOut * kT)
         *reinterpret_cast<__nv_bfloat16*>(base_ptr + kIn * p.in_stage + (tid / kT) * p.out_stage + (tid % kT) * p.pc + p.heads * kDk * 2) =
@@ -434,7 +465,11 @@
                 const int s = it % kIn;
                 const int title = static_cast<int>(blockIdx.x) + it * static_cast<int>(gridDim.x);
                 const bool pad = p.pad != nullptr && p.pad[title] != 0;
-                const int row = pad ? 0 : title * kT;
+                if (p.mask != nullptr && p.mask[title] == 0) {
+                    mbar_arrive(&full[s]);
+                    return;
+                }
+                const int row = pad ? 0 : p.mask != nullptr ? p.offset[title] : title * kT;
                 mbar_arrive_expect_tx(&full[s], p.tx);
                 tma_load_2d(base_ptr + s * p.in_stage, pad ? &tm_pad : &tm_qkv, &full[s], 0, row);
                 if (HILO) tma_load_2d(base_ptr + s * p.in_stage + p.qkv_tile, pad ? &tm_padlo : &tm_vlo, &full[s], 0, row);
@@ -466,7 +501,6 @@
     const bool v8 = odd ? (t4 >= 2) : (t4 < 2);
     const bool c0ok = !odd || t4 >= 2, c2ok = odd || t4 < 2, lo2 = t4 < 2;
     const uint32_t pq = p.pq, pc = p.pc, pv = p.pv;
-    const uint32_t r15q = (lane & 15) * pq, r7q = (lane & 7) * pq;
     const uint32_t hi = (lane >> 4) * 16u, mid = ((lane >> 3) & 1) * 16u;
     const float sc = p.sc;
 
@@ -474,20 +508,25 @@
         const int s = it % kIn, o = it % kOut;
         const uint32_t Q = in_base + s * p.in_stage, K = Q + p.sec2, V = K + p.sec2, VL = Q + p.qkv_tile;
         const uint32_t ob = out_base + o * p.out_stage;
-        const long long row_base = static_cast<long long>(static_cast<int>(blockIdx.x) + it * static_cast<int>(gridDim.x)) * kT;
+        const int title = static_cast<int>(blockIdx.x) + it * static_cast<int>(gridDim.x);
+        const long long row_base = static_cast<long long>(title) * kT;
+        uint32_t ro[3], rv[3];
+        row_offsets(p.mask, title, pq, base + bias_q - Q, lane, ro);
+        if (HILO) row_offsets(p.mask, title, pv, base + bias_v - VL, lane, rv);
+        const uint32_t r15 = (lane & 8) ? ro[1] : ro[0];
         f_wait(&full[s], (it / kIn) & 1, 82);
         uint32_t kb16[3][2], kb8[3], vt16[3][2], vt8[3], vl16[HILO ? 3 : 1][2], vl8[HILO ? 3 : 1];
 #pragma unroll
         for (int nt = 0; nt < 3; ++nt) {
-            lds_x2(kb16[nt], K + k16b + nt * 8 * pq + r7q + mid);
-            lds_x1(&kb8[nt], K + k8b + nt * 8 * pq + r7q);
+            lds_x2(kb16[nt], K + k16b + ro[nt] + mid);
+            lds_x1(&kb8[nt], K + k8b + ro[nt]);
             kb8[nt] = sel(v8, kb8[nt]);
-            lds_x2_t(vt16[nt], V + gb + 16 * nt + r15q);
-            lds_x1_t(&vt8[nt], V + gb + 16 * nt + 16 * pq + r7q);
+            lds_x2_t(vt16[nt], V + gb + 16 * nt + r15);
+            lds_x1_t(&vt8[nt], V + gb + 16 * nt + ro[2]);
             vt8[nt] = sel(lo2, vt8[nt]);
             if (HILO) {
-                lds_x2_t(vl16[nt], VL + gb + 16 * nt + (lane & 15) * pv);
-                lds_x1_t(&vl8[nt], VL + gb + 16 * nt + 16 * pv + (lane & 7) * pv);
+                lds_x2_t(vl16[nt], VL + gb + 16 * nt + ((lane & 8) ? rv[1] : rv[0]));
+                lds_x1_t(&vl8[nt], VL + gb + 16 * nt + rv[2]);
                 vl8[nt] = sel(lo2, vl8[nt]);
             }
         }
@@ -495,13 +534,13 @@
         for (int mt = 0; mt < 2; ++mt) {
             uint32_t aq[4], aq8[2];
             if (mt == 0) {
-                lds_x4(aq, Q + k16b + r15q + hi);
-                lds_x2(aq8, Q + k8b + r15q);
+                lds_x4(aq, Q + k16b + r15 + hi);
+                lds_x2(aq8, Q + k8b + r15);
             } else {
                 uint32_t t[2];
-                lds_x2(t, Q + k16b + 16 * pq + r7q + mid);
+                lds_x2(t, Q + k16b + ro[2] + mid);
                 aq[0] = t[0], aq[1] = 0u, aq[2] = t[1], aq[3] = 0u;
-                lds_x1(&aq8[0], Q + k8b + 16 * pq + r7q);
+                lds_x1(&aq8[0], Q + k8b + ro[2]);
                 aq8[1] = 0u;
             }
             aq8[0] = sel(v8, aq8[0]), aq8[1] = sel(v8, aq8[1]);
@@ -681,8 +720,10 @@
     p.row_bytes = qkv_row;
     p.dbias = live != nullptr ? live->dbias : nullptr;
     p.ld_dbias = live != nullptr ? live->ld_dbias : 0;
+    p.compact = live != nullptr && live->compact_qkv ? 1 : 0;
+    p.bias = lt != nullptr ? lt->qkv : nullptr;
     const size_t smem = 128 + static_cast<size_t>(kIn) * p.in_stage + static_cast<size_t>(kOut) * p.out_stage +
-                       static_cast<size_t>(heads) * kScrWarp + (2 * kIn + 2 * kOut) * sizeof(uint64_t) + 64;
+                       static_cast<size_t>(heads) * kScrWarp + 128 + p.pq + 64;
     NR_REQUIRE(smem <= 227 * 1024, "mhsa_title_bwd: %zu bytes of shared memory", smem);
     const long long rows = n_seq * kT;
     CUtensorMap tq, tc, to, tp;
@@ -713,7 +754,7 @@
 }
 
 int mhsa_title_fwd(const void* qkv, int ld_qkv, int sec, long long n_seq, int heads, void* ctx, int ld_ctx, DropoutCfg drop,
-                   cudaStream_t stream, const void* v_lo, int ld_vlo, void* ctx_lo, const PaddingTitles* pad) {
+                   cudaStream_t stream, const void* v_lo, int ld_vlo, void* ctx_lo, const PaddingTitles* pad, const LiveTokens* live) {
     using namespace title;
     NR_REQUIRE(mhsa_title_fwd_supported(kT, kDk, heads, sec, ld_qkv, ld_ctx), "mhsa_title_fwd: unsupported layout");
     NR_REQUIRE(n_seq * kT < (1ll << 31), "mhsa_title_fwd: too many rows");
@@ -739,10 +780,16 @@
     p.drop = Dropout::make(drop.p, drop.seed);
     NR_REQUIRE(pad == nullptr || (pad->pad != nullptr && pad->qkv != nullptr && (!hilo || (pad->v_lo != nullptr && ld_vlo == sec))),
                "mhsa_title_fwd: padding titles without their Q|K|V tile (or its V low plane at pitch sec)");
+    NR_REQUIRE(live == nullptr || (pad == nullptr && live->pad && live->mask && live->offset && live->qkv && (!hilo || (live->v_lo && ld_vlo == sec))),
+               "mhsa_title_fwd: live tokens without their flags, offsets or bias rows (or with padding titles as well)");
     p.pad = pad != nullptr ? pad->pad : nullptr;
+    p.mask = live != nullptr ? live->mask : nullptr;
+    p.offset = live != nullptr ? live->offset : nullptr;
+    p.bias_q = live != nullptr ? live->qkv : nullptr;
+    p.bias_v = live != nullptr ? live->v_lo : nullptr;
     const int n_in = hilo ? kInHilo : kIn;
     const size_t smem = 128 + static_cast<size_t>(n_in) * p.in_stage + static_cast<size_t>(kOut) * p.out_stage +
-                       (2 * n_in + 2 * kOut) * sizeof(uint64_t) + 64;
+                       128 + p.pq + p.pv + 64;
     const size_t cap = hilo ? 227 * 1024 : 113 * 1024;
     NR_REQUIRE(smem <= cap, "mhsa_title_fwd: %zu bytes of shared memory", smem);
     const long long rows = n_seq * kT;
diff --git a/news-recommendation_b200/csrc/aux.cu b/news-recommendation_b200/csrc/aux.cu
--- a/news-recommendation_b200/csrc/aux.cu
+++ b/news-recommendation_b200/csrc/aux.cu
@@ -94,31 +94,42 @@
 __global__ void __launch_bounds__(kGatherThreads) gather_rows_kernel(const long long* __restrict__ ids, long long n_tok, int T,
                                                                    const uint4* __restrict__ table, int V, int D, int ld,
                                                                    uint4* __restrict__ X, int ld_x, int padded, Dropout drop,
-                                                                   int* bad_flag) {
+                                                                   int* bad_flag, const int* __restrict__ index,
+                                                                   const int* __restrict__ n_live) {
     const int chunks = ld >> 3;
     const int x_chunks = ld_x >> 3;
     const int rows_per_it = kGatherThreads / chunks;
     const int rl = threadIdx.x / chunks, c = threadIdx.x - rl * chunks;
     if (rl >= rows_per_it) return;
     const long long stride = static_cast<long long>(gridDim.x) * rows_per_it;
-    long long tok = static_cast<long long>(blockIdx.x) * rows_per_it + rl;
-    long long n_id = tok < n_tok ? __ldg(ids + tok) : 0;
-    if (tok < n_tok && (n_id < 0 || n_id >= V)) { atomicExch(bad_flag, 1); n_id = 0; }
-    uint4 n_u = tok < n_tok ? __ldg(table + n_id * chunks + c) : make_uint4(0, 0, 0, 0);
+    long long n_rows = n_tok;
+    if (index != nullptr) {
+        n_rows = __ldg(n_live);
+        const long long tail_end = min(n_tok, (n_rows + 63) / 64 * 64);
+        for (long long r = static_cast<long long>(blockIdx.x) * rows_per_it + rl + n_rows; r < tail_end; r += stride)
+            X[r * x_chunks + c] = make_uint4(0, 0, 0, 0);
+    }
+    const auto token = [&](long long i) -> long long { return index != nullptr ? __ldg(index + i) : i; };
+    long long i = static_cast<long long>(blockIdx.x) * rows_per_it + rl;
+    long long tok = i < n_rows ? token(i) : 0;
+    long long n_id = i < n_rows ? __ldg(ids + tok) : 0;
+    if (i < n_rows && (n_id < 0 || n_id >= V)) { atomicExch(bad_flag, 1); n_id = 0; }
+    uint4 n_u = i < n_rows ? __ldg(table + n_id * chunks + c) : make_uint4(0, 0, 0, 0);
     const int col = c * 8;
-    for (; tok < n_tok; tok += stride) {
+    for (; i < n_rows; i += stride) {
         uint4 u = n_u;
-        const long long tok2 = tok + stride;
-        if (tok2 < n_tok) {
-            n_id = __ldg(ids + tok2);
+        const long long cur = tok, i2 = i + stride;
+        if (i2 < n_rows) {
+            tok = token(i2);
+            n_id = __ldg(ids + tok);
             if (n_id < 0 || n_id >= V) { atomicExch(bad_flag, 1); n_id = 0; }
             n_u = __ldg(table + n_id * chunks + c);
         }
-        long long xr = tok;
+        long long xr = cur;
         int t = 0;
         if (padded) {
-            const long long seg = tok / T;
-            t = static_cast<int>(tok - seg * T);
+            const long long seg = cur / T;
+            t = static_cast<int>(cur - seg * T);
             xr = seg * (T + 2) + 1 + t;
         }
         uint32_t w[4] = {u.x, u.y, u.z, u.w};
@@ -136,7 +147,7 @@
             __nv_bfloat16* e = reinterpret_cast<__nv_bfloat16*>(w);
             for (int j = D - col; j < 8; ++j) e[j] = __float2bfloat16_rn(j == D - col ? 1.0f : 0.f);
         }
-        X[xr * x_chunks + c] = make_uint4(w[0], w[1], w[2], w[3]);
+        X[(index != nullptr ? i : xr) * x_chunks + c] = make_uint4(w[0], w[1], w[2], w[3]);
         if (padded) {
             if (t == 0) X[(xr - 1) * x_chunks + c] = make_uint4(0, 0, 0, 0);
             if (t == T - 1) X[(xr + 1) * x_chunks + c] = make_uint4(0, 0, 0, 0);
@@ -144,16 +155,19 @@
     }
 }
 int gather_rows(const long long* ids, long long n_tok, int T, const void* table, int V, int D, int ld_table, void* X,
-                int ld_x, int padded, DropoutCfg drop, int* bad_id_flag, cudaStream_t stream) {
+                int ld_x, int padded, DropoutCfg drop, int* bad_id_flag, cudaStream_t stream, const LiveTokens* live) {
     if (n_tok == 0) return 0;
     NR_REQUIRE(ld_table % 8 == 0 && ld_x % 8 == 0 && ld_x >= ld_table && ld_table >= D + 1 && ld_table / 8 <= kGatherThreads,
                "gather_rows: pitch %d/%d for D=%d", ld_table, ld_x, D);
+    NR_REQUIRE(live == nullptr || (!padded && ld_x == ld_table && live->index && live->offset),
+               "gather_rows: compact rows need the unpadded layout, ld_x == ld_table and the live tokens' index");
     const int rows_per_it = kGatherThreads / (ld_table / 8);
     const int blocks = static_cast<int>(std::min<long long>((n_tok + rows_per_it - 1) / rows_per_it, 148 * 6));
     ProfScope ps("gather_rows", static_cast<int>(n_tok), D, ld_x, stream);
     gather_rows_kernel<<<blocks, kGatherThreads, 0, stream>>>(ids, n_tok, T, static_cast<const uint4*>(table), V, D, ld_table,
                                                    static_cast<uint4*>(X), ld_x, padded, Dropout::make(drop.p, drop.seed),
-                                                   bad_id_flag);
+                                                   bad_id_flag, live != nullptr ? live->index : nullptr,
+                                                   live != nullptr ? live->offset + n_tok / T : nullptr);
     ++g_launches;
     NR_CHECK_CUDA(cudaGetLastError());
     return 0;
diff --git a/news-recommendation_b200/csrc/gemm.cu b/news-recommendation_b200/csrc/gemm.cu
--- a/news-recommendation_b200/csrc/gemm.cu
+++ b/news-recommendation_b200/csrc/gemm.cu
@@ -877,13 +877,14 @@
     int* counts;
     int* block_base;
     unsigned* ticket;
+    int* bad_id_flag;
     LiveTokens out;
 };
 
 __global__ void __launch_bounds__(kLiveTilesThreads) live_classify_kernel(const LiveJob j) {
     const int lane = threadIdx.x & 31, warp = threadIdx.x >> 5, warps = kLiveTilesThreads / 32;
     const bool all_live = j.row0 != nullptr && block_row_nonzero(j.row0, j.d);
-    write_padding_qkv(j.bqkv, j.T, j.sec, j.ld3, j.out.qkv, nullptr);
+    write_padding_qkv(j.bqkv, j.T, j.sec, j.ld3, j.out.qkv, j.out.v_lo);
     const int gtid = blockIdx.x * blockDim.x + threadIdx.x, nthreads = gridDim.x * blockDim.x;
     for (int i = gtid; i < (j.M + kTileM - 1) / kTileM; i += nthreads) j.out.tiles[1 + i] = i;
     const int px = j.ldx / 8;
@@ -892,6 +893,7 @@
     for (int s = s0 + warp; s < s1; s += warps) {
         const long long id = lane < j.T ? j.ids[static_cast<long long>(s) * j.T + lane] : 0;
         uint32_t mask = __ballot_sync(0xffffffffu, lane < j.T && (all_live || (id >= 1 && id < j.V)));
+        if (j.bad_id_flag != nullptr && __any_sync(0xffffffffu, lane < j.T && (id < 0 || id >= j.V)) && lane == 0) atomicExch(j.bad_id_flag, 1);
         if (j.row0 == nullptr) {
             for (uint32_t cand = ((j.T == 32 ? 0u : 1u << j.T) - 1u) & ~mask; cand != 0; cand &= cand - 1) {
                 const int r = __ffs(cand) - 1;
@@ -977,9 +979,9 @@
         const int m_live = j.out.offset[j.n_seq];
         const int tail_end = min(j.M, (m_live + kTileM - 1) / kTileM * kTileM);
         for (int r = m_live + threadIdx.x; r < tail_end; r += blockDim.x) j.out.index[r] = -1;
-        for (int i = threadIdx.x; i < (tail_end - m_live) * px; i += blockDim.x)
+        for (int i = threadIdx.x; j.Xc != nullptr && i < (tail_end - m_live) * px; i += blockDim.x)
             j.Xc[static_cast<long long>(m_live) * px + i] = make_uint4(0, 0, 0, 0);
-        for (int i = threadIdx.x; i < (tail_end - m_live) * p3; i += blockDim.x)
+        for (int i = threadIdx.x; j.dqkv_c != nullptr && i < (tail_end - m_live) * p3; i += blockDim.x)
             j.dqkv_c[static_cast<long long>(m_live) * p3 + i] = make_uint4(0, 0, 0, 0);
     }
     __shared__ int src_row[kLiveTilesThreads / 32][32];
@@ -992,6 +994,7 @@
             src_row[warp][rank] = s * j.T + lane;
         }
         __syncwarp();
+        if (j.Xc == nullptr) continue;
         const uint4* X = j.X;
         uint4* Xc = j.Xc + static_cast<long long>(dst) * px;
 #pragma unroll 4
@@ -1003,50 +1006,69 @@
     }
 }
 
-long long live_tokens_bytes(long long n_seq, int T, int ld3) {
-    const long long n = n_seq, M = n_seq * T, nb = (n + kLiveTitlesPerBlock - 1) / kLiveTitlesPerBlock;
-    WorkspaceLayout l{nullptr};
-    l.take<unsigned char>(n);
-    l.take<uint32_t>(n);
-    l.take<int>(n);
-    l.take<int>(n + 1);
-    l.take<int>(M);
-    l.take<int>(M / kTileM + 2);
-    l.take<int>(nb + 1);
-    l.take<__nv_bfloat16>(static_cast<long long>(T) * ld3);
-    return l.bytes();
-}
+struct LiveLayout : WorkspaceLayout {
+    LiveTokens out;
+    int *counts, *block_base;
+    LiveLayout(void* buf, long long n_seq, int T, int sec, int ld3) : WorkspaceLayout{static_cast<char*>(buf)} {
+        const long long n = n_seq, M = n_seq * T, nb = (n + kLiveTitlesPerBlock - 1) / kLiveTitlesPerBlock;
+        out.pad = take<unsigned char>(n);
+        out.mask = take<uint32_t>(n);
+        counts = take<int>(n);
+        out.offset = take<int>(n + 1);
+        out.index = take<int>(M);
+        out.tiles = take<int>(M / kTileM + 2);
+        block_base = take<int>(nb + 1);
+        out.qkv = take<__nv_bfloat16>(static_cast<long long>(T) * ld3);
+        out.v_lo = take<__nv_bfloat16>(static_cast<long long>(T) * sec);
+    }
+};
+
+long long live_tokens_bytes(long long n_seq, int T, int sec, int ld3) { return LiveLayout(nullptr, n_seq, T, sec, ld3).bytes(); }
+LiveTokens live_tokens_view(void* buf, long long n_seq, int T, int sec, int ld3) { return LiveLayout(buf, n_seq, T, sec, ld3).out; }
 
 int live_tokens(const long long* ids, long long n_seq, int T, int d, const void* table, int ld_table, int V, const float* bqkv,
                 int sec, int ld3, const void* X, int ldx, void* Xc, void* dqkv_c, void* buf, long long buf_bytes, LiveTokens* out,
-                cudaStream_t stream) {
-    NR_REQUIRE(ids && bqkv && X && Xc && dqkv_c && buf, "live_tokens: null operand");
+                cudaStream_t stream, int* bad_id_flag) {
+    NR_REQUIRE(ids && bqkv && buf && (table || X) && (!Xc || X), "live_tokens: null operand");
     NR_REQUIRE(T >= 1 && T <= 32 && d % 2 == 0 && ld_table % 8 == 0 && ldx % 8 == 0 && ld3 % 8 == 0 && V >= 1 && n_seq * T < (1ll << 31),
                "live_tokens: T=%d d=%d ld_table=%d ldx=%d ld3=%d V=%d", T, d, ld_table, ldx, ld3, V);
     const auto a16 = [](const void* p) { return (reinterpret_cast<uintptr_t>(p) & 15) == 0; };
     NR_REQUIRE(a16(X) && a16(Xc) && a16(dqkv_c) && a16(buf), "live_tokens: rows not 16-byte aligned");
-    NR_REQUIRE(buf_bytes >= live_tokens_bytes(n_seq, T, ld3), "live_tokens: buffer too small (%lld bytes)", buf_bytes);
+    NR_REQUIRE(buf_bytes >= live_tokens_bytes(n_seq, T, sec, ld3), "live_tokens: buffer too small (%lld bytes)", buf_bytes);
     const int n = static_cast<int>(n_seq), M = n * T, nb = ceil_div(n, kLiveTitlesPerBlock);
-    WorkspaceLayout l{static_cast<char*>(buf)};
-    out->pad = l.take<unsigned char>(n);
-    out->mask = l.take<uint32_t>(n);
-    int* counts = l.take<int>(n);
-    out->offset = l.take<int>(n + 1);
-    out->index = l.take<int>(M);
-    out->tiles = l.take<int>(M / kTileM + 2);
-    int* block_base = l.take<int>(nb + 1);
-    out->qkv = l.take<__nv_bfloat16>(static_cast<long long>(T) * ld3);
+    const LiveLayout l(buf, n_seq, T, sec, ld3);
+    *out = l.out;
+    int* counts = l.counts;
+    int* block_base = l.block_base;
     if (n == 0) return 0;
     unsigned* ticket = reinterpret_cast<unsigned*>(block_base + nb);
     NR_CHECK_CUDA(cudaMemsetAsync(ticket, 0, sizeof(unsigned), stream));
     const LiveJob j{.ids = ids, .n_seq = n, .T = T, .d = d, .M = M, .V = V, .n_blocks = nb, .row0 = static_cast<const uint32_t*>(table),
                     .bqkv = bqkv, .sec = sec, .ld3 = ld3, .ldx = ldx, .X = static_cast<const uint4*>(X), .Xc = static_cast<uint4*>(Xc),
-                    .dqkv_c = static_cast<uint4*>(dqkv_c), .counts = counts, .block_base = block_base, .ticket = ticket, .out = *out};
+                    .dqkv_c = static_cast<uint4*>(dqkv_c), .counts = counts, .block_base = block_base, .ticket = ticket,
+                    .bad_id_flag = bad_id_flag, .out = *out};
     ProfScope ps("live_tokens", M, n, 0, stream);
     live_classify_kernel<<<nb, kLiveTilesThreads, 0, stream>>>(j);
     ++g_launches;
     NR_CHECK_CUDA(cudaGetLastError());
     live_compact_kernel<<<nb, kLiveTilesThreads, 0, stream>>>(j);
+    ++g_launches;
+    NR_CHECK_CUDA(cudaGetLastError());
+    return 0;
+}
+
+__global__ void __launch_bounds__(kLiveTilesThreads) live_zero_tail_kernel(const int* m_live_p, int M, uint4* rows, int p16) {
+    const int m_live = *m_live_p, tail_end = min(M, (m_live + kTileM - 1) / kTileM * kTileM);
+    for (int i = blockIdx.x * blockDim.x + threadIdx.x; i < (tail_end - m_live) * p16; i += gridDim.x * blockDim.x)
+        rows[static_cast<long long>(m_live) * p16 + i] = make_uint4(0, 0, 0, 0);
+}
+
+int live_zero_tail(const LiveTokens& live, long long n_seq, int T, void* rows, int ld, cudaStream_t stream) {
+    NR_REQUIRE(live.offset && rows && ld % 8 == 0 && (reinterpret_cast<uintptr_t>(rows) & 15) == 0, "live_zero_tail: bad operand");
+    if (n_seq == 0) return 0;
+    ProfScope ps("live_zero_tail", static_cast<int>(n_seq * T), ld, 0, stream);
+    live_zero_tail_kernel<<<8, kLiveTilesThreads, 0, stream>>>(live.offset + n_seq, static_cast<int>(n_seq * T), static_cast<uint4*>(rows),
+                                                               ld / 8);
     ++g_launches;
     NR_CHECK_CUDA(cudaGetLastError());
     return 0;
diff --git a/news-recommendation_b200/csrc/nr_ops.h b/news-recommendation_b200/csrc/nr_ops.h
--- a/news-recommendation_b200/csrc/nr_ops.h
+++ b/news-recommendation_b200/csrc/nr_ops.h
@@ -99,11 +99,14 @@
     int* index = nullptr;
     int* tiles = nullptr;
     void* qkv = nullptr;
-};
-long long live_tokens_bytes(long long n_seq, int T, int ld3);
+    void* v_lo = nullptr;
+};
+long long live_tokens_bytes(long long n_seq, int T, int sec, int ld3);
 int live_tokens(const long long* ids, long long n_seq, int T, int d, const void* table, int ld_table, int V, const float* bqkv,
                 int sec, int ld3, const void* X, int ldx, void* Xc, void* dqkv_c, void* buf, long long buf_bytes, LiveTokens* out,
-                cudaStream_t stream);
+                cudaStream_t stream, int* bad_id_flag = nullptr);
+LiveTokens live_tokens_view(void* buf, long long n_seq, int T, int sec, int ld3);
+int live_zero_tail(const LiveTokens& live, long long n_seq, int T, void* rows, int ld, cudaStream_t stream);
 
 struct Bf16Rows {
     const float* src;
@@ -128,11 +131,12 @@
 inline int rows_to_bf16(const Bf16Rows& job, Bf16Op op, cudaStream_t stream) { return rows_to_bf16(&job, 1, op, stream); }
 int sum_over_seq(const float* src, long long n_seq, long long L, float* dst, cudaStream_t stream);
 int gather_rows(const long long* ids, long long n_tok, int T, const void* table, int V, int D, int ld_table, void* X,
-                int ld_x, int padded, DropoutCfg drop, int* bad_id_flag, cudaStream_t stream);
+                int ld_x, int padded, DropoutCfg drop, int* bad_id_flag, cudaStream_t stream, const LiveTokens* live = nullptr);
 struct TitleBwdLive {
     const LiveTokens* tokens;
     float* dbias;
     int ld_dbias;
+    int compact_qkv = 0;
 };
 int mhsa_core_fwd(const void* qkv, int ld_qkv, int sec, long long n_seq, int T, int heads, int dk, void* ctx, int ld_ctx,
                   DropoutCfg drop, cudaStream_t stream);
@@ -141,7 +145,7 @@
 bool mhsa_title_fwd_supported(int T, int dk, int heads, int sec, int ld_qkv, int ld_ctx);
 int mhsa_title_fwd(const void* qkv, int ld_qkv, int sec, long long n_seq, int heads, void* ctx, int ld_ctx, DropoutCfg drop,
                    cudaStream_t stream, const void* v_lo = nullptr, int ld_vlo = 0, void* ctx_lo = nullptr,
-                   const PaddingTitles* pad = nullptr);
+                   const PaddingTitles* pad = nullptr, const LiveTokens* live = nullptr);
 bool mhsa_title_bwd_supported(int T, int dk, int heads, int sec, int ld_qkv, int ld_dctx, int ld_dqkv);
 int mhsa_title_bwd(const void* qkv, int ld_qkv, int sec, const void* dctx, int ld_dctx, long long n_seq, int heads, void* dqkv,
                    int ld_dqkv, cudaStream_t stream, const TitleBwdLive* live = nullptr);
diff --git a/news-recommendation_b200/src/newsrec_b200/__init__.py b/news-recommendation_b200/src/newsrec_b200/__init__.py
--- a/news-recommendation_b200/src/newsrec_b200/__init__.py
+++ b/news-recommendation_b200/src/newsrec_b200/__init__.py
@@ -21,6 +21,7 @@
         ("wqkv_kcat_bf16", _vp), ("X_kcat_bf16", _vp), ("QKV_f32", _vp),
         ("V_lo_bf16", _vp),
         ("dense_pos", _vp),
+        ("live", _vp), ("live_bytes", _ll),
     ]
 
 
@@ -35,6 +36,7 @@
         ("workspace", _vp), ("workspace_bytes", _ll),
         ("wqkv_bf16", _vp), ("bqkv", _vp), ("emb_grad_ready_event", _vp),
         ("dpos", _vp), ("table_bf16", _vp),
+        ("live", _vp), ("live_bytes", _ll),
     ]
 
 
@@ -186,6 +188,7 @@
     "nr_dot_score_bwd": (_i, [_vp, _vp, _vp, _i, _i, _i, _vp, _vp, _vp]),
     "nr_mhsa_accurate_supported": (_i, [_i, _i, _i]),
     "nr_mhsa_encoder_fwd": (_i, [C.POINTER(MhsaEncoderFwdArgs), _vp]),
+    "nr_mhsa_encoder_live_bytes": (_ll, [_ll, _i, _i]),
     "nr_mhsa_encoder_bwd_workspace": (_ll, [_ll, _i, _i, _i]),
     "nr_mhsa_encoder_bwd": (_i, [C.POINTER(MhsaEncoderBwdArgs), _vp]),
     "nr_cnn_encoder_fwd": (_i, [C.POINTER(CnnEncoderFwdArgs), _vp]),
diff --git a/news-recommendation_b200/src/newsrec_b200/ops.py b/news-recommendation_b200/src/newsrec_b200/ops.py
--- a/news-recommendation_b200/src/newsrec_b200/ops.py
+++ b/news-recommendation_b200/src/newsrec_b200/ops.py
@@ -213,10 +213,16 @@
             a.wqkv_kcat_bf16, a.X_kcat_bf16, a.QKV_f32, a.C_lo_bf16 = _p(kcat), _p(keep[0]), _p(keep[1]), _p(C_lo)
         a.X_bf16, a.QKV_bf16, a.C_bf16, a.w, a.out = _p(X), _p(QKV), _p(Cx), _p(w), _p(out)
         a.bad_id_flag = _p(bad_flag)
+        live = None
+        if ids is not None and bool(lib.nr_mhsa_accurate_supported(T, d, heads)):
+            live_bytes = int(lib.nr_mhsa_encoder_live_bytes(n_seq, T, d))
+            live = torch.empty((live_bytes,), dtype=torch.uint8, device=dev)
+            a.live, a.live_bytes = _p(live), live_bytes
         check(lib.nr_mhsa_encoder_fwd(C.byref(a), _stream()), "nr_mhsa_encoder_fwd")
         if need_bwd:
             ctx.save_for_backward(X, QKV if QKV is not None else torch.empty(0, device=dev), Cx, w,
-                                  ids if ids is not None else torch.empty(0, device=dev))
+                                  ids if ids is not None else torch.empty(0, device=dev),
+                                  live if live is not None else torch.empty(0, dtype=torch.uint8, device=dev))
         ctx.meta = dict(n_seq=n_seq, T=T, d=d, q=q, heads=heads, p_drop=float(p_drop), seed=seed, ops=ops,
                         has_ids=ids is not None, V=emb_w.shape[0] if ids is not None else 0,
                         dense_shape=None if dense is None else tuple(dense.shape),
@@ -227,7 +233,7 @@
     @staticmethod
     def backward(ctx, dout):
         lib = load_library()
-        X, QKV, Cx, w, ids = ctx.saved_tensors
+        X, QKV, Cx, w, ids, live = ctx.saved_tensors
         m = ctx.meta
         dev = X.device
         d, q, T, n_seq = m["d"], m["q"], m["T"], m["n_seq"]
@@ -280,6 +286,8 @@
         a.dWqkv_ext, a.dWa_ext, a.dqv = _p(dWqkv), _p(dWa), _p(dqv)
         a.demb, a.ddense, a.dpos = _p(demb), _p(ddense), _p(dpos)
         a.workspace, a.workspace_bytes = _p(ws), ws_bytes
+        if live.numel():
+            a.live, a.live_bytes = _p(live), live.numel()
         check(lib.nr_mhsa_encoder_bwd(C.byref(a), _stream()), "nr_mhsa_encoder_bwd")
         g_dense = ddense.view(m["dense_shape"]) if ddense is not None else None
         g_emb = None if emb_direct else demb
```

After: 98950 (median of 6 runs). 11.4% higher.
